# fxxJuses/MICFormer

Measured on AMD Instinct MI355X. Metric: train volumes/sec (128^3 CT+MRI pair), higher is better.
Workload: dtype bf16; 1 GPU; MicFormer base Head(embed_dim=48, depths 2-2-6-2, heads 3-6-12-24, window 2^3, 8 classes) full train step (fwd + MDiceLoss + bwd + Adam/cosine) on 128^3 CT+MR pairs, DropPath on; local_batch=2, global_batch=2, parallelism=dp1, launch=hipGraph replay (one graph)

## Files before the change

### include/micformer_hip.h

```cpp
#ifndef MICFORMER_HIP_H
#define MICFORMER_HIP_H

#include <stddef.h>
#include <stdint.h>

#ifdef __cplusplus
extern "C" {
#endif

typedef void* micf_stream_t;

#define MICF_OK 0
#define MICF_EINVAL (-1)
#define MICF_EUNSUPPORTED (-2)
#define MICF_ELAUNCH (-3)

#define MICF_ABI_VERSION 1

#define MICF_DTYPE_F32 0
#define MICF_DTYPE_BF16 1
#define MICF_DTYPE_BF16_ATTN_FP8 2

int micf_abi_version(void);
const char* micf_strerror(int code);
// ... 137 lines not shown
                            micf_stream_t stream);
int micf_conv_down_bwd_weight(const float* dy, const float* x, float* dw, float* dbias, int B, int D, int H, int W,
                              int C, int N, micf_stream_t stream);
int micf_space_to_depth(const float* x, float* a, int B, int D, int H, int W, int C, int k, int64_t batch_stride,
                        micf_stream_t stream);
int micf_depth_to_space(const float* a, const float* bias, float* y, int B, int D, int H, int W, int C, int k,
                        micf_stream_t stream);
int micf_depth_to_space_add(const float* a, const float* bias, const float* add, float* y, int B, int D, int H, int W, int C,
                            int k, micf_stream_t stream);
int micf_colsum(const float* x, float* out, int64_t M, int N, micf_stream_t stream);
int micf_conv_up_fwd(const float* x, const float* w, const float* bias, float* y, int B, int D, int H, int W, int C,
                     int N, int k, micf_stream_t stream);
int micf_conv_up_bwd_data(const float* dy, const float* w, float* dx, int B, int D, int H, int W, int C, int N, int k,
                          micf_stream_t stream);
int micf_conv_up_bwd_weight(const float* dy, const float* x, float* dw, float* dbias, int B, int D, int H, int W,
                            int C, int N, int k, micf_stream_t stream);

int micf_sw_window(const float* vol, float* win, int C, int D, int H, int W, int rd, int rh, int rw, int z0, int y0, int x0,
                   micf_stream_t stream);
int micf_sw_accumulate(const float* pred, float* out, float* count, int K, int D, int H, int W, int rd, int rh, int rw, int z0,
                       int y0, int x0, micf_stream_t stream);
int micf_sw_normalize(float* out, const float* count, int K, int64_t V, micf_stream_t stream);
int micf_sw_window_batch(const float* vol, float* win, const int32_t* coords, int n, int B, int C, int D, int H, int W, int rd,
                         int rh, int rw, micf_stream_t stream);
int micf_sw_accumulate_batch(const float* pred, float* out, float* count, const int32_t* coords, int n, int B, int K, int D, int H,
                             int W, int rd, int rh, int rw, micf_stream_t stream);

int micf_intensity_stats(const void* vol, int is_half, double* sums, int B, int Cm, int64_t V, micf_stream_t stream);
int micf_patch_rows_prepared(const void* vol, int is_half, const double* sums, const float* params, float* rows0, float* rows1, int B,
                             int Cm, int D, int H, int W, int k, micf_stream_t stream);
int micf_input_prepare(const void* vol, int is_half, const double* sums, const float* params, float* out, const uint8_t* label_in,
                       uint8_t* label_out, int B, int Cm, int D, int H, int W, micf_stream_t stream);

int micf_pad3d(const float* src, float* dst, int B, int D, int H, int W, int Dp, int Hp, int Wp, int C,
               micf_stream_t stream);
int micf_crop3d(const float* src, float* dst, int B, int D, int H, int W, int Dp, int Hp, int Wp, int C,
                int accumulate, micf_stream_t stream);
int micf_resize_trilinear_fwd(const float* src, float* dst, int B, int D, int H, int W, int Do, int Ho, int Wo, int C,
                              micf_stream_t stream);
int micf_resize_trilinear_bwd(const float* ddst, float* dsrc, int B, int D, int H, int W, int Do, int Ho, int Wo,
                              int C, micf_stream_t stream);

int micf_dice_bce_fwd(const float* logits, const float* target, double* sums, float* loss, int B, int K, int64_t V,
                      micf_stream_t stream);
int micf_dice_bce_bwd(const float* logits, const float* target, const double* sums, const float* grad_out,
                      float* dlogits, int B, int K, int64_t V, micf_stream_t stream);
int micf_dice_bce_label_fwd(const float* logits, const uint8_t* label, double* sums, float* loss, int B, int K, int64_t V,
                            micf_stream_t stream);
int micf_dice_bce_label_bwd(const float* logits, const uint8_t* label, const double* sums, const float* grad_out,
                            float* dlogits, int B, int K, int64_t V, micf_stream_t stream);
int micf_argmax_meandice(const float* logits, const uint8_t* label, uint8_t* mask_out, int64_t* counts, double* out,
                         int B, int K, int64_t V, micf_stream_t stream);

int micf_dice_metric(const float* logits, const void* target, int target_is_label, double* sums, float* out, int B, int K,
                     int64_t V, micf_stream_t stream);

int micf_adam_tick(void* state, double base_lr, double eta_min, int64_t t_max, micf_stream_t stream);
int micf_adam_step(float* p, const float* g, float* m, float* v, int64_t n, const void* state, float beta1,
                   float beta2, float eps, float grad_scale, void* p_bf16, micf_stream_t stream);


typedef struct micf_ln_pair_item {
  const float *x, *gamma, *beta;
  float *y, *mean, *rstd;
} micf_ln_pair_item;
typedef struct micf_ln_bwd_pair_item {
  const float *dy, *x, *mean, *rstd, *gamma;
  float *dx, *dgamma, *dbeta;
  const float* add;
  float* partials;
} micf_ln_bwd_pair_item;
int micf_layernorm_fwd_pair(const micf_ln_pair_item* items, int n, int64_t rows, int C, float eps, float* zero,
                            int64_t zero_floats, micf_stream_t stream);
int micf_layernorm_bwd_pair(const micf_ln_bwd_pair_item* items, int n, int64_t rows, int C, micf_stream_t stream);

typedef struct micf_offset_head_group {
  const float* xn;
  const float* xa;
  const float *conv_w, *conv_b;
  float* conv_ws;
  const float *ln_g, *ln_b, *w1;
  float *hid, *flow, *xs;
} micf_offset_head_group;
typedef struct micf_offset_head_bwd_group {
  const float* dxs;
  const float *hid, *flow, *xa, *ln_g, *ln_b, *w1, *conv_w;
  float* conv_ws;
  float* dxa;
  float* dxn;
  float* dhid;
  float *dln_g, *dln_b, *dw1;
} micf_offset_head_bwd_group;
int micf_offset_head_needs_zero(int B, int D, int H, int W, int C);
int micf_offset_head_fwd(const micf_offset_head_group* groups, int ngroups, int B, int D, int H, int W, int C, float eps,
                         int prepared, int hid_zeroed, int dtype, micf_stream_t stream);
int64_t micf_offset_head_bwd_workspace(int ngroups, int B, int D, int H, int W);
int micf_offset_head_bwd(const micf_offset_head_bwd_group* groups, int ngroups, int B, int D, int H, int W, int C, float eps,
                         int prepared, float* workspace, int64_t workspace_floats, int dtype, int defer_finish, micf_stream_t stream);
int micf_offset_head_finish_deferrable(int B, int D, int H, int W);
int micf_offset_head_bwd_finish(const micf_offset_head_bwd_group* groups, int ngroups, int B, int D, int H, int W, int C,
                                float* workspace, int64_t workspace_floats, micf_stream_t stream);
typedef struct micf_offset_head_finish_call {
  const micf_offset_head_bwd_group* groups;
  int32_t ngroups, B, D, H, W, C;
  float* workspace;
  int64_t workspace_floats;
} micf_offset_head_finish_call;
int micf_offset_head_bwd_finish_grouped(const micf_offset_head_finish_call* calls, int ncalls, micf_stream_t stream);

typedef struct micf_block_fwd_group {
  const float* x;
  const float* kvsrc;
  const float *ln1_g, *ln1_b, *bq, *bkv, *bp, *ln2_g, *ln2_b, *b1, *b2;
  const void *wq, *wkv, *wp, *w1, *w2;
  const float *s1, *s2;
  float* y;
  float *xn, *q, *kv, *o, *x1, *xn2;
  void* h;
  float* g;
  float* stats;
  void* kvs16;
  const float* hid;
  const float* samp_src;
  const float *ln16_g, *ln16_b, *w1c;
  float* flow;
  float* xs32;
  const float *nln_g, *nln_b;
  float *nln_y, *nln_mean, *nln_rstd;
  float* zero16;
} micf_block_fwd_group;
int micf_block_fuses_sampler(int C, int heads);
int micf_block_saves_bf16(int C, int heads, int dtype);
typedef struct micf_block_bwd_group {
  const float* dy;
  const float *x, *x1, *stats, *q, *kv;
  const void* h;
  const float *ln1_g, *ln2_g;
  const void *wqt, *wkvt, *wpt, *w1t, *w2t;
  const float *s1, *s2;
  float* dx;
  float* dxs;
  float *dx1, *dh, *dq, *dkv;
  float *ln1_part, *ln2_part;
  float* dx1_copy;
  void* dy16;
  const float* xn2;
  const void* w1;
  const float* b1;
  const float* pre_d;
  const float* pre_x;
  const float *pre_mean, *pre_rstd;
  const float* pre_g;
  float* pre_part;
} micf_block_bwd_group;
int micf_block_recomputes_h(int C, int heads);
int micf_block_tile_tokens(int B, int D, int H, int W, int C, int heads, int hidden, int backward);
int micf_block_fwd_persistent_probe(const micf_block_fwd_group* groups, int ngroups, int B, int D, int H, int W, int C, int heads,
                                    int hidden, float eps, float scale, int dtype, int repeats, int* sync_ws, micf_stream_t stream);
int micf_probe_mfma_chain(const void* a, const void* b, const void* c, const void* d, float* out, int form, micf_stream_t stream);
typedef struct micf_weight_prep_item {
  const float* src;
  void* dst;
  void* dst_t;
  int32_t rows, cols, bf16 , reserved;
} micf_weight_prep_item;
int micf_weight_prep_grouped(const micf_weight_prep_item* items, int n, micf_stream_t stream);
int micf_block_fwd(const micf_block_fwd_group* groups, int ngroups, int B, int D, int H, int W, int C, int heads,
                   int hidden, float eps, float scale, int dtype, micf_stream_t stream);
int micf_block_bwd(const micf_block_bwd_group* groups, int ngroups, int B, int D, int H, int W, int C, int heads,
                   int hidden, float scale, int dtype, micf_stream_t stream);

int micf_zero(void* p, int64_t bytes, micf_stream_t stream);
int micf_drop_path_draw(void* rng, const float* keep, float* out, int n, int B, micf_stream_t stream);


int micf_grad_wire_pack(const float* src, int64_t n, void* dst, int64_t padded, micf_stream_t stream);
int micf_grad_wire_sum(const void* recv, int ranks, int64_t shard, void* out, micf_stream_t stream);
int micf_grad_wire_unpack(const void* src, float* dst, int64_t n, micf_stream_t stream);

#ifdef __cplusplus
}
#endif
#endif
```

### micformer_amd/_lib.py

```python
import ctypes
import os

_PKT = "DEBUG_CLR_GRAPH_PACKET_CAPTURE"
_pkt_before = os.environ.get(_PKT)
if os.environ.get("MICF_SEGMENTED", "0") == "1":
    os.environ.setdefault(_PKT, "0")

import torch

GRAPH_SEGMENTS_OK = os.environ.get(_PKT) == "0" and (_pkt_before == "0" or not torch.cuda.is_initialized())

_HERE = os.path.dirname(os.path.abspath(__file__))
LIB_PATH = os.environ.get("MICF_LIB") or os.path.join(_HERE, "libmicformer_hip.so")

_P, _I, _L, _F, _D = ctypes.c_void_p, ctypes.c_int, ctypes.c_int64, ctypes.c_float, ctypes.c_double
_T = {"p": _P, "i": _I, "l": _L, "f": _F, "d": _D}

SIGNATURES = {
    "micf_layernorm_fwd": "ppippppplifp",
    "micf_layernorm_bwd": "pppippppppplippp",
    "micf_layernorm_bwd_partial_rows": "lii",
    "micf_layernorm_bwd_finish": "pip",
    "micf_linear_fwd": "ppipppplppliiiip",
    "micf_linear_bwd_data": "pplppppiiliiip",
    "micf_linear_bwd_weight": "pplppiippliiplip",
    "micf_linear_bwd_weight_workspace": "lii",
    "micf_linear_bwd_weight_grouped": "piplip",
    "micf_linear_bwd_weight_grouped_workspace": "pi",
    "micf_head_tail_compose": "pppppiiiipp",
    "micf_head_tail_col2im": "pppiiiiiip",
    "micf_head_tail_im2col": "ppiiiiiip",
    "micf_head_tail_col2im_sw": "pppppiiiiiiiiiip",
    "micf_head_tail_decompose": "pppppppppiiiipp",
    "micf_head_tail_fused_supported": "iiiiiii",
    "micf_head_tail_pack_bytes": "ii",
    "micf_head_tail_pack": "pppppiiip",
    "micf_head_tail_fwd_fused": "pppiiiiiiip",
    "micf_head_tail_fwd_fused_sw": "pppppiiiiiiiiiiip",
    "micf_head_tail_loss_parts": "iiii",
    "micf_head_tail_fwd_loss_fused": "ppppipppiiiiiiip",
    "micf_head_tail_bwd_data_fused": "pppiiiiiiip",
    "micf_head_tail_bwd_weight_fused": "pppppliiiiiiip",
    "micf_head_tail_bwd_weight_fused_workspace": "iiiii",
    "micf_sw_window": "ppiiiiiiiiiip",
    "micf_sw_accumulate": "pppiiiiiiiiiip",
    "micf_sw_normalize": "ppilp",
    "micf_window_attn_fwd": "pippipiiiiiiiiiifp",
    "micf_window_attn_fwd_fp8": "pippipiiiiiiiiiifp",
    "micf_window_attn_bwd": "pippipipippiiiiiiiiiifp",
    "micf_conv3_fwd": "pipipppiiiiiipliip",
    "micf_conv3_fwd_workspace": "iii",
    "micf_conv3_bwd_data": "pippiipiiiiiiipliip",
    "micf_conv3_weight_prep_grouped": "pip",
    "micf_layernorm_fwd_pair": "pilifplp",
    "micf_layernorm_bwd_pair": "pilip",
    "micf_offset_head_needs_zero": "iiiii",
    "micf_offset_head_fwd": "piiiiiifiiip",
    "micf_offset_head_bwd_workspace": "iiiii",
    "micf_offset_head_bwd": "piiiiiifipliip",
    "micf_offset_head_finish_deferrable": "iiii",
    "micf_offset_head_bwd_finish": "piiiiiiplp",
    "micf_offset_head_bwd_finish_grouped": "pip",
    "micf_conv3_bwd_data_workspace": "iii",
    "micf_conv3_bwd_weight": "pipipippiiiiiplip",
    "micf_conv3_bwd_weight_workspace": "iiiiiii",
    "micf_conv3_bwd_weight_grouped": "piiiiiiiiplip",
    "micf_conv3_bwd_weight_grouped_workspace": "iiiiiiii",
    "micf_offset_sample_fwd": "pppppppiiiiifp",
    "micf_offset_sample_bwd": "ppppppppppppiiiiifplp",
    "micf_offset_sample_bwd_workspace": "iiii",
    "micf_stn_fwd": "pppiiiiip",
    "micf_stn_bwd": "pppppiiiiip",
    "micf_patch_embed_fwd": "piipppiiiiiip",
    "micf_patch_embed_bwd_weight": "ppiippiiiiiip",
    "micf_conv_down_fwd": "ppppiiiiiip",
    "micf_conv_down_bwd_data": "pppiiiiiip",
    "micf_conv_down_bwd_weight": "ppppiiiiiip",
    "micf_conv_up_fwd": "ppppiiiiiiip",
    "micf_conv_up_bwd_data": "pppiiiiiiip",
    "micf_conv_up_bwd_weight": "ppppiiiiiiip",
    "micf_space_to_depth": "ppiiiiiilp",
    "micf_depth_to_space": "pppiiiiiip",
    "micf_depth_to_space_add": "ppppiiiiiip",
    "micf_colsum": "pplip",
    "micf_pad3d": "ppiiiiiiiip",
    "micf_crop3d": "ppiiiiiiiiip",
    "micf_resize_trilinear_fwd": "ppiiiiiiiip",
    "micf_resize_trilinear_bwd": "ppiiiiiiiip",
    "micf_dice_bce_fwd": "ppppiilp",
    "micf_dice_bce_bwd": "pppppiilp",
    "micf_dice_bce_label_fwd": "ppppiilp",
    "micf_dice_bce_label_bwd": "pppppiilp",
    "micf_argmax_meandice": "pppppiilp",
    "micf_adam_tick": "pddlp",
    "micf_adam_step": "pppplpffffpp",
    "micf_block_tile_tokens": "iiiiiiii",
    "micf_block_saves_bf16": "iii",
    "micf_block_fuses_sampler": "ii",
    "micf_block_recomputes_h": "ii",
    "micf_weight_prep_grouped": "pip",
    "micf_grad_wire_pack": "plplp",
    "micf_grad_wire_sum": "pilpp",
    "micf_grad_wire_unpack": "pplp",
    "micf_block_fwd": "piiiiiiiiffip",
    "micf_block_bwd": "piiiiiiiifip",
    "micf_block_fwd_persistent_probe": "piiiiiiiiffiipp",
    "micf_probe_mfma_chain": "pppppip",
    "micf_dice_metric": "ppippiilp",
    "micf_sw_window_batch": "pppiiiiiiiiip",
    "micf_sw_accumulate_batch": "ppppiiiiiiiiip",
    "micf_intensity_stats": "pipiilp",
    "micf_input_prepare": "pipppppiiiiip",
    "micf_patch_rows_prepared": "pippppiiiiiip",
    "micf_zero": "plp",
    "micf_drop_path_draw": "pppiip",
}


class WgradItem(ctypes.Structure):
    _fields_ = [("a", ctypes.c_void_p), ("dy", ctypes.c_void_p), ("dp_scale", ctypes.c_void_p), ("dw", ctypes.c_void_p),
                ("dbias", ctypes.c_void_p), ("M", ctypes.c_int64), ("rows_per_sample", ctypes.c_int64),
                ("N", ctypes.c_int32), ("K", ctypes.c_int32), ("operand_dtype", ctypes.c_int32), ("ldw", ctypes.c_int32)]


class Conv3WgradItem(ctypes.Structure):
    _fields_ = [("dy", ctypes.c_void_p), ("x1", ctypes.c_void_p), ("x2", ctypes.c_void_p), ("dw", ctypes.c_void_p),
                ("dbias", ctypes.c_void_p)]


class LnFinishItem(ctypes.Structure):
    _fields_ = [("partials", ctypes.c_void_p), ("dgamma", ctypes.c_void_p), ("dbeta", ctypes.c_void_p),
                ("blocks", ctypes.c_int32), ("C", ctypes.c_int32)]


_VP = ctypes.c_void_p


class BlockFwdGroup(ctypes.Structure):
    FIELDS = ("x", "kvsrc", "ln1_g", "ln1_b", "bq", "bkv", "bp", "ln2_g", "ln2_b", "b1", "b2", "wq", "wkv", "wp", "w1", "w2",
              "s1", "s2", "y", "xn", "q", "kv", "o", "x1", "xn2", "h", "g", "stats", "kvs16", "hid", "samp_src", "ln16_g", "ln16_b", "w1c", "flow", "xs32",
              "nln_g", "nln_b", "nln_y", "nln_mean", "nln_rstd", "zero16")
    _fields_ = [(n, _VP) for n in FIELDS]


class BlockBwdGroup(ctypes.Structure):
    FIELDS = ("dy", "x", "x1", "stats", "q", "kv", "h", "ln1_g", "ln2_g", "wqt", "wkvt", "wpt", "w1t", "w2t", "s1", "s2",
              "dx", "dxs", "dx1", "dh", "dq", "dkv", "ln1_part", "ln2_part", "dx1_copy", "dy16", "xn2", "w1", "b1",
              "pre_d", "pre_x", "pre_mean", "pre_rstd", "pre_g", "pre_part")
    _fields_ = [(n, _VP) for n in FIELDS]


class WeightPrepItem(ctypes.Structure):
    _fields_ = [("src", _VP), ("dst", _VP), ("dst_t", _VP), ("rows", ctypes.c_int32), ("cols", ctypes.c_int32),
                ("bf16", ctypes.c_int32), ("reserved", ctypes.c_int32)]


class LnPairItem(ctypes.Structure):
    FIELDS = ("x", "gamma", "beta", "y", "mean", "rstd")
    _fields_ = [(n, _VP) for n in FIELDS]


class LnBwdPairItem(ctypes.Structure):
    FIELDS = ("dy", "x", "mean", "rstd", "gamma", "dx", "dgamma", "dbeta", "add", "partials")
    _fields_ = [(n, _VP) for n in FIELDS]


class OffsetHeadGroup(ctypes.Structure):
    FIELDS = ("xn", "xa", "conv_w", "conv_b", "conv_ws", "ln_g", "ln_b", "w1", "hid", "flow", "xs")
    _fields_ = [(n, _VP) for n in FIELDS]


class OffsetHeadBwdGroup(ctypes.Structure):
    FIELDS = ("dxs", "hid", "flow", "xa", "ln_g", "ln_b", "w1", "conv_w", "conv_ws", "dxa", "dxn", "dhid", "dln_g", "dln_b", "dw1")
    _fields_ = [(n, _VP) for n in FIELDS]


class OffsetHeadFinishCall(ctypes.Structure):
    _fields_ = [("groups", _VP), ("ngroups", ctypes.c_int32), ("B", ctypes.c_int32), ("D", ctypes.c_int32), ("H", ctypes.c_int32),
                ("W", ctypes.c_int32), ("C", ctypes.c_int32), ("workspace", _VP), ("workspace_floats", ctypes.c_int64)]


class Conv3PrepItem(ctypes.Structure):
    _fields_ = [("w", _VP), ("fwd", _VP), ("bwd", _VP), ("N", ctypes.c_int32), ("Cin", ctypes.c_int32)]


class MicfError(RuntimeError):
    pass


INT64_RETURNS = frozenset((
    "micf_linear_bwd_weight_workspace", "micf_linear_bwd_weight_grouped_workspace", "micf_conv3_bwd_data_workspace",
    "micf_offset_sample_bwd_workspace", "micf_conv3_bwd_weight_workspace", "micf_conv3_bwd_weight_grouped_workspace",
    "micf_head_tail_pack_bytes", "micf_head_tail_loss_parts", "micf_head_tail_bwd_weight_fused_workspace",
    "micf_conv3_fwd_workspace", "micf_offset_head_bwd_workspace"))


def bind(signatures, int64=(), feature=None, library=None):
    library = lib if library is None else library
    for name, sig in signatures.items():
        try:
            fn = getattr(library, name)
        except AttributeError:
            what = f"predates the {feature} ({name} is missing)" if feature else f"does not export {name}"
            raise ImportError(f"{LIB_PATH} {what}: rebuild it with "
                              "`python -c \"import __graft_entry__ as g; g.build()\"`") from None
        fn.argtypes = [_T[c] for c in sig]
        fn.restype = _L if name in int64 else _I
    return library


def _load():
    if not os.path.exists(LIB_PATH):
        raise ImportError(
            f"{LIB_PATH} not found: build it with `python micformer_amd/build.py` (hipcc, gfx950). "
            "micformer_amd has no CPU / PyTorch fallback path.")
    lib = bind(SIGNATURES, INT64_RETURNS, library=ctypes.CDLL(LIB_PATH))
    lib.micf_strerror.argtypes = [_I]
    lib.micf_strerror.restype = ctypes.c_char_p
    lib.micf_set_option.argtypes = [ctypes.c_char_p, _I]
    lib.micf_set_option.restype = _I
    lib.micf_get_option.argtypes = [ctypes.c_char_p, ctypes.POINTER(_I)]
    lib.micf_get_option.restype = _I
    lib.micf_abi_version.argtypes = []
    lib.micf_abi_version.restype = _I
    if lib.micf_abi_version() != 1:
        raise ImportError("libmicformer_hip.so ABI version mismatch")
    return lib


lib = _load()


def get_option(name):
    v = _I(0)
    if lib.micf_get_option(name.encode(), ctypes.byref(v)) != 0:
        raise KeyError(f"unknown micformer option {name!r}")
    return v.value


def set_option(name, value):
    prev = get_option(name)
    if lib.micf_set_option(name.encode(), int(value)) != 0:
        raise KeyError(f"unknown micformer option {name!r}")
    return prev


class option:

    def __init__(self, name, value):
        self.name, self.value = name, value

    def __enter__(self):
        self.prev = set_option(self.name, self.value)

    def __exit__(self, *exc):
        set_option(self.name, self.prev)
        return False


def ptr(t):
    if t is None:
        return None
    if not t.is_cuda:
        raise MicfError("micformer_amd ops need CUDA (ROCm) tensors: there is no CPU path")
    if not t.is_contiguous():
        raise MicfError("micformer_amd ops need contiguous tensors")
    return t.data_ptr()


_raw_stream = getattr(torch._C, "_cuda_getCurrentRawStream", None)
_cur_device = getattr(torch._C, "_cuda_getDevice", None)


def stream():
    if _raw_stream is not None and _cur_device is not None:
        return _raw_stream(_cur_device())
    return torch.cuda.current_stream().cuda_stream


PROFILE = None
BLOCK_DEPTH = 0
UNIT = None


def set_unit(kind, groups, tokens, channels):
    global UNIT
    if PROFILE is not None:
        UNIT = f"{kind}|{groups}x{tokens}x{channels}"


class block_region:

    def __enter__(self):
        global BLOCK_DEPTH
        BLOCK_DEPTH += 1

    def __exit__(self, *exc):
        global BLOCK_DEPTH, UNIT
        BLOCK_DEPTH -= 1
        if BLOCK_DEPTH == 0:
            UNIT = None
# ... 79 lines not shown
```

### micformer_amd/csrc/block_bwd.hip

```cpp
#include "block_fused.h"
#include "attn_fp8.h"

namespace micf {

struct BlkBwdArgs {
  micf_block_bwd_group g[2];
  TileGeo geo;
  int G, tiles, C, heads, hidden;
  float scale;
  int attn_mfma;
};

template <int TM, int NW, int X4>
struct RowRegs {
  static constexpr int RPP = 4 * NW, NPASS = (TM + RPP - 1) / RPP, K = (X4 + 15) / 16;
  float4 v[NPASS][K];
  template <class Addr>
  __device__ __forceinline__ void load(const int* tok, int tk0, const Addr addr) {
    const int lane = threadIdx.x & 63, wave = threadIdx.x >> 6, l16 = lane & 15, rg = lane >> 4;
#pragma unroll
    for (int pass = 0; pass < NPASS; ++pass) {
      const int row = pass * RPP + wave * 4 + rg;
      const int tk = row < TM ? tok[row] : -1;
#pragma unroll
// ... 417 lines not shown
          float sacc = 0.f, dacc = 0.f;
#pragma unroll
          for (int d = 0; d < HP; d += 4) {
            const float4 t = *reinterpret_cast<const float4*>(kp + d);
            sacc += qr[d] * t.x; sacc += qr[d + 1] * t.y; sacc += qr[d + 2] * t.z; sacc += qr[d + 3] * t.w;
            const float4 u = *reinterpret_cast<const float4*>(vp + d);
            dacc += dor[d] * u.x; dacc += dor[d + 1] * u.y; dacc += dor[d + 2] * u.z; dacc += dor[d + 3] * u.w;
          }
          if (SP >= 2) { sacc += __shfl_xor(sacc, 1, 64); dacc += __shfl_xor(dacc, 1, 64); }
          if (SP == 4) { sacc += __shfl_xor(sacc, 2, 64); dacc += __shfl_xor(dacc, 2, 64); }
          p[j] = sacc; dp[j] = dacc;
          mx = fmaxf(mx, sacc);
        }
        float den = 0.f;
#pragma unroll
        for (int j = 0; j < 8; ++j) { p[j] = expf(p[j] - mx); den += p[j]; }
        const float inv = 1.0f / den;
        float dot = 0.f;
#pragma unroll
        for (int j = 0; j < 8; ++j) { p[j] *= inv; dot += p[j] * dp[j]; }
#pragma unroll
        for (int d = 0; d < HP; ++d) dq[d] = 0.f;
#pragma unroll
        for (int j = 0; j < 8; ++j) {
          const float ds = p[j] * (dp[j] - dot);
          if (j / (8 / SP) == sub) {
            PS[pair * 16 + j] = p[j];
            PS[pair * 16 + 8 + j] = ds;
          }
          const float* kp = U + (r0 + j) * SU + C + hoff;
          const float dss = ds * a.scale;
#pragma unroll
          for (int d = 0; d < HP; d += 4) {
            const float4 t = *reinterpret_cast<const float4*>(kp + d);
            dq[d] += dss * t.x; dq[d + 1] += dss * t.y; dq[d + 2] += dss * t.z; dq[d + 3] += dss * t.w;
          }
        }
      }
      lds_barrier();
      if (active) {
#pragma unroll
        for (int d = 0; d < HP; ++d) { dk[d] = 0.f; dv[d] = 0.f; }
        const int base = pair - i * heads;
#pragma unroll
        for (int m = 0; m < 8; ++m) {
          const float pm = PS[(base + m * heads) * 16 + i];
          const float dsm = PS[(base + m * heads) * 16 + 8 + i] * a.scale;
          const float* qp = U + (r0 + m) * SU + hoff;
          const float* dop = A2 + (r0 + m) * S + hoff;
#pragma unroll
          for (int d = 0; d < HP; d += 4) {
            const float4 t = *reinterpret_cast<const float4*>(qp + d);
            dk[d] += dsm * t.x; dk[d + 1] += dsm * t.y; dk[d + 2] += dsm * t.z; dk[d + 3] += dsm * t.w;
            const float4 u = *reinterpret_cast<const float4*>(dop + d);
            dv[d] += pm * u.x; dv[d + 1] += pm * u.y; dv[d + 2] += pm * u.z; dv[d + 3] += pm * u.w;
          }
        }
      }
      lds_barrier();
      if (active) {
#pragma unroll
        for (int d = 0; d < HP; d += 4) {
          *reinterpret_cast<float4*>(U + row * SU + hoff + d) = make_float4(dq[d], dq[d + 1], dq[d + 2], dq[d + 3]);
          *reinterpret_cast<float4*>(U + row * SU + C + hoff + d) = make_float4(dk[d], dk[d + 1], dk[d + 2], dk[d + 3]);
          *reinterpret_cast<float4*>(U + row * SU + 2 * C + hoff + d) = make_float4(dv[d], dv[d + 1], dv[d + 2], dv[d + 3]);
        }
      }
      lds_barrier();
    }
  }

#pragma unroll 1
  for (int pass = 0; pass < NPASS; ++pass) {
    const int row = pass * RPP + wave * 4 + rg;
    if (row >= TM) continue;
    const int tk = tok[row];
    if (tk < 0) continue;
    const uint32_t rel = (uint32_t)(tk - tk0);
    for (int c4 = l16; c4 < 3 * C4; c4 += 16) {
      const float4 v = *reinterpret_cast<const float4*>(U + row * SU + 4 * c4);
      if (c4 < C4) st_h4_32<BF16>(dq0, rel * C + 4 * c4, v);
      else st_h4_32<BF16>(dkv0, rel * 2 * C + 4 * (c4 - C4), v);
    }
  }

  if (!g.dxs) {
    if (PARK) r_ln1.unpark(stash, g.ln1_g);
    gemm_phase<TJ, NSLK, NKK, C, NW, BF16>(wqt, C, U, nullptr, 0, nullptr, SU, A2, S, EpiStore{});
    gemm_phase<TJ, NSLK, 2 * NKK, 2 * C, NW, BF16>(wkvt, C, U + C, nullptr, 0, nullptr, SU, A2, S, EpiAcc{});
    ln_bwd_tile<TJ, VPL, NW, C>(A2, A1, S, r_ln1, tok, tk0, dx0, nullptr, U, g.ln1_part ? g.ln1_part + (int64_t)tile * 2 * C : nullptr);
  } else {
    gemm_phase<TJ, NSLK, NKK, C, NW, BF16>(wqt, C, U, nullptr, 0, nullptr, SU, A2, S, EpiStore{});
#pragma unroll 1
    for (int pass = 0; pass < NPASS; ++pass) {
      const int row = pass * RPP + wave * 4 + rg;
      if (row >= TM) continue;
      const int tk = tok[row];
      if (tk < 0) continue;
      for (int c4 = l16; c4 < C4; c4 += 16)
        st4g(at32(dx0, ((uint32_t)(tk - tk0) * C + 4 * c4) * 4u), *reinterpret_cast<const float4*>(A2 + row * S + 4 * c4));
    }
    lds_barrier();
    gemm_phase<TJ, NSLK, 2 * NKK, 2 * C, NW, BF16>(wkvt, C, U + C, nullptr, 0, nullptr, SU, A2, S, EpiStore{});
#pragma unroll 1
    for (int pass = 0; pass < NPASS; ++pass) {
      const int row = pass * RPP + wave * 4 + rg;
      if (row >= TM) continue;
      const int tk = tok[row];
      if (tk < 0) continue;
      for (int c4 = l16; c4 < C4; c4 += 16)
        st4g(at32(g.dxs + (int64_t)tk0 * C, ((uint32_t)(tk - tk0) * C + 4 * c4) * 4u), *reinterpret_cast<const float4*>(A2 + row * S + 4 * c4));
    }
  }
}

template <int C, int HD, int TJ>
static int launch_bwd(const BlkBwdArgs& a, int dtype, hipStream_t s) {
  constexpr int TM = 16 * TJ, NW = C >= 192 ? 8 : 4;
  const bool recomp = a.g[0].h == nullptr;
  const size_t lds = block_lds_floats(TM, C, block_bwd_scratch_floats(TM, C / HD, 64 * NW),
                                      block_bwd_park_floats(TM, C, 64 * NW) + (recomp ? 4 * C : 0)) * sizeof(float);
  if (lds > 160 * 1024) return MICF_EUNSUPPORTED;
  const unsigned grid = a.G == 2 ? (unsigned)((a.tiles + 3) / 4 * 8) : (unsigned)a.tiles;
  static std::once_flag once;
  std::call_once(once, [] {
    (void)hipFuncSetAttribute(reinterpret_cast<const void*>(&block_bwd_kernel<C, HD, TJ, NW, true, false>), hipFuncAttributeMaxDynamicSharedMemorySize, 160 * 1024);
    (void)hipFuncSetAttribute(reinterpret_cast<const void*>(&block_bwd_kernel<C, HD, TJ, NW, false, false>), hipFuncAttributeMaxDynamicSharedMemorySize, 160 * 1024);
    (void)hipFuncSetAttribute(reinterpret_cast<const void*>(&block_bwd_kernel<C, HD, TJ, NW, true, true>), hipFuncAttributeMaxDynamicSharedMemorySize, 160 * 1024);
    (void)hipFuncSetAttribute(reinterpret_cast<const void*>(&block_bwd_kernel<C, HD, TJ, NW, false, true>), hipFuncAttributeMaxDynamicSharedMemorySize, 160 * 1024);
  });
  if (dtype == MICF_DTYPE_BF16) {
    if (recomp) hipLaunchKernelGGL((block_bwd_kernel<C, HD, TJ, NW, true, true>), dim3(grid), dim3(64 * NW), lds, s, a);
    else hipLaunchKernelGGL((block_bwd_kernel<C, HD, TJ, NW, true, false>), dim3(grid), dim3(64 * NW), lds, s, a);
  } else {
    if (recomp) hipLaunchKernelGGL((block_bwd_kernel<C, HD, TJ, NW, false, true>), dim3(grid), dim3(64 * NW), lds, s, a);
    else hipLaunchKernelGGL((block_bwd_kernel<C, HD, TJ, NW, false, false>), dim3(grid), dim3(64 * NW), lds, s, a);
  }
  MICF_RETURN_LAUNCH();
}

}

#include "block_wave_bwd.h"

using namespace micf;

extern "C" int micf_block_bwd(const micf_block_bwd_group* groups, int ngroups, int B, int D, int H, int W, int C, int heads,
                              int hidden, float scale, int dtype, micf_stream_t stream) {
  if (!groups || ngroups < 1 || ngroups > 2) return MICF_EINVAL;
  const int TM = micf_block_tile_tokens(B, D, H, W, C, heads, hidden, 1);
  if (TM == 0) return MICF_EUNSUPPORTED;
  if (dtype != MICF_DTYPE_F32 && dtype != MICF_DTYPE_BF16) return MICF_EINVAL;
  BlkBwdArgs a;
  for (int i = 0; i < ngroups; ++i) {
    const micf_block_bwd_group& g = groups[i];
    const void* need[] = {g.dy, g.x1, g.stats, g.q, g.kv, g.ln2_g, g.wqt, g.wkvt, g.wpt, g.w1t, g.w2t, g.dx, g.dx1, g.dh, g.dq, g.dkv};
    for (const void* p : need)
      if (!p || (reinterpret_cast<uintptr_t>(p) & 15)) return MICF_EINVAL;
    if (g.h) {
      if (reinterpret_cast<uintptr_t>(g.h) & 15) return MICF_EINVAL;
    } else {
      const void* re[] = {g.xn2, g.w1, g.b1};
      for (const void* p : re)
        if (!p || (reinterpret_cast<uintptr_t>(p) & 15)) return MICF_EINVAL;
      if (!micf_block_recomputes_h(C, heads)) return MICF_EINVAL;
    }
    if (i > 0 && (g.h == nullptr) != (groups[0].h == nullptr)) return MICF_EINVAL;
    if (g.pre_d) {
      const void* pr[] = {g.pre_d, g.pre_x, g.pre_mean, g.pre_rstd, g.pre_g, g.pre_part, g.dy16};
      for (const void* p : pr)
        if (!p || (reinterpret_cast<uintptr_t>(p) & 15)) return MICF_EINVAL;
      if (g.dxs || dtype != MICF_DTYPE_BF16 || block_wide_tile_tokens(C, C / heads)) return MICF_EINVAL;
    }
    if (!g.dxs && (!g.x || !g.ln1_g)) return MICF_EINVAL;
    const void* opt[] = {g.x, g.ln1_g, g.dxs, g.ln1_part, g.ln2_part, g.dx1_copy, g.dy16};
    for (const void* p : opt)
      if (p && (reinterpret_cast<uintptr_t>(p) & 15)) return MICF_EINVAL;
    a.g[i] = g;
  }
  if (ngroups == 1) a.g[1] = a.g[0];
  a.geo = make_tile_geo(B, D, H, W);
  a.G = ngroups; a.C = C; a.heads = heads; a.hidden = hidden; a.scale = scale;
  a.tiles = (a.geo.nwin + TM / 8 - 1) / (TM / 8);
  a.attn_mfma = dtype == MICF_DTYPE_BF16 ? 1 : 0;
  hipStream_t s = (hipStream_t)stream;
  const int hd = C / heads, tj = TM / 16;
  if ((int64_t)2 * H * W * (TM / 8 + 1) * hidden * (int64_t)sizeof(float) >= (int64_t)1 << 32) return MICF_EUNSUPPORTED;
  if (block_wide_tile_tokens(C, hd)) return block_bwd_wide(groups, ngroups, B, D, H, W, C, heads, scale, dtype, s);
  {
    if (options().block_wave != 0 && C == 48 && hd == 16 && tj == 2 && dtype == MICF_DTYPE_BF16 && a.attn_mfma && a.g[0].h && a.g[1].h && (a.g[0].dxs != nullptr) == (a.g[1].dxs != nullptr) &&
        (a.g[0].pre_d != nullptr) == (a.g[1].pre_d != nullptr) && !(a.g[0].dxs && a.g[0].pre_d) &&
        a.geo.T * (int64_t)hidden * 2 < ((int64_t)1 << 31))
    {
      if (options().block_debug & 1) a.attn_mfma |= 2;
      return wave48::launch_bwd_wave48(a, s);
    }
  }
#define MICF_BB(C_, HD_, TJ_) if (C == C_ && hd == HD_ && tj == TJ_) return launch_bwd<C_, HD_, TJ_>(a, dtype, s)
  MICF_BB(48, 16, 2); MICF_BB(96, 16, 2); MICF_BB(192, 16, 1);
  MICF_BB(96, 32, 1); MICF_BB(192, 32, 1); MICF_BB(384, 32, 1);
#undef MICF_BB
  return MICF_EUNSUPPORTED;
}
```

### micformer_amd/csrc/block_fwd.hip

```cpp
#include <cstdlib>

#include "block_fused.h"
#include "attn_fp8.h"

namespace micf {

struct BlkFwdArgs {
  micf_block_fwd_group g[2];
  TileGeo geo;
  int G, tiles, C, heads, hidden, debug;
  int att8;
  float eps, scale;
};

template <int C, int HD, int TJ, int NW, bool BF16, bool SAMP>
__device__ __forceinline__ void block_fwd_tile(const BlkFwdArgs& a, const unsigned bid) {
  constexpr int TM = 16 * TJ, VPL = (C + 63) / 64, NSL = C / 16, NTHR = 64 * NW, RPP = 4 * NW, NPASS = (TM + RPP - 1) / RPP;
  constexpr int NSLK = C >= 384 ? NSL / 2 : NSL, NKK = C >= 384 ? 2 : 1;
  extern __shared__ __attribute__((aligned(1024))) float lds[];
  constexpr int C4 = C >> 2, S = C + 4, SU = block_u_cols(C, true, TM) + 4, Hd = 4 * C;
  float* A1 = lds;
  float* A2 = A1 + TM * S;
  float* U = A2 + TM * S;
  float* sc1 = U + TM * SU;
// ... 317 lines not shown
      const int row = pass * RPP + wave * 4 + rg;
      if (row >= TM) continue;
      const int tk = tok[row];
      for (int c4 = l16; c4 < X4; c4 += 16) {
        float* up = U + row * SU + 4 * c4;
        const float4 v = *reinterpret_cast<const float4*>(up);
        const float4 ge = do_gelu ? make_float4(gelu_t<BF16>(v.x), gelu_t<BF16>(v.y), gelu_t<BF16>(v.z), gelu_t<BF16>(v.w)) : v;
        *reinterpret_cast<float4*>(up) = ge;
        if (tk >= 0 && save) {
          if (g.h) st_h4<BF16>(g.h, (int64_t)tk * Hd + c0 + 4 * c4, v);
          st_h4<BF16>(g.g, (int64_t)tk * Hd + c0 + 4 * c4, ge);
        }
      }
    }
    lds_barrier();
    if (!(a.debug & 4)) gemm_phase<TJ, NSLK, NKK * HC / C, Hd, NW, BF16>(w2 + 16 * c0, C, U, nullptr, 0, nullptr, SU, A2, S, EpiAccScale{sc2});
  }

  const bool nln = g.nln_g != nullptr;
#pragma unroll 1
  for (int pass = 0; pass < NPASS; ++pass) {
    const int row = pass * RPP + wave * 4 + rg;
    if (row >= TM) continue;
    const int tk = tok[row];
    if (tk < 0) continue;
    const float s2v = sc2[row];
    float4 v[VPL];
#pragma unroll
    for (int k = 0; k < VPL; ++k) {
      const int c4 = l16 + 16 * k;
      v[k] = make_float4(0.f, 0.f, 0.f, 0.f);
      if (c4 < C4) {
        v[k] = *reinterpret_cast<const float4*>(A2 + row * S + 4 * c4);
        const float4 b = *reinterpret_cast<const float4*>(p_b2 + 4 * c4);
        v[k].x += s2v * b.x; v[k].y += s2v * b.y; v[k].z += s2v * b.z; v[k].w += s2v * b.w;
        st4g(g.y + (int64_t)tk * C + 4 * c4, v[k]);
      }
    }
    if (nln) {
      float s = 0.f;
#pragma unroll
      for (int k = 0; k < VPL; ++k) s += (v[k].x + v[k].y) + (v[k].z + v[k].w);
      const float mu = sum16(s) * invC;
      float qd = 0.f;
#pragma unroll
      for (int k = 0; k < VPL; ++k) {
        if (l16 + 16 * k < C4) {
          const float d0 = v[k].x - mu, d1 = v[k].y - mu, d2 = v[k].z - mu, d3 = v[k].w - mu;
          qd += (d0 * d0 + d1 * d1) + (d2 * d2 + d3 * d3);
        }
      }
      const float rs = 1.0f / sqrtf(sum16(qd) * invC + a.eps);
#pragma unroll
      for (int k = 0; k < VPL; ++k) {
        const int c4 = l16 + 16 * k;
        if (c4 < C4) {
          const float4 gm = *reinterpret_cast<const float4*>(p_ln1g + 4 * c4), bt = *reinterpret_cast<const float4*>(p_ln1b + 4 * c4);
          st4g(g.nln_y + (int64_t)tk * C + 4 * c4, make_float4((v[k].x - mu) * rs * gm.x + bt.x, (v[k].y - mu) * rs * gm.y + bt.y,
                                                                (v[k].z - mu) * rs * gm.z + bt.z, (v[k].w - mu) * rs * gm.w + bt.w));
        }
      }
      if (l16 == 0) { g.nln_mean[tk] = mu; g.nln_rstd[tk] = rs; }
      if (g.zero16) g.zero16[(int64_t)tk * 16 + l16] = 0.f;
    }
  }
}

template <int C, int HD, int TJ, int NW, bool BF16, bool SAMP>
__global__ void __launch_bounds__(64 * NW) block_fwd_kernel(const BlkFwdArgs a) {
  block_fwd_tile<C, HD, TJ, NW, BF16, SAMP>(a, blockIdx.x);
}

__device__ __forceinline__ void probe_grid_barrier(unsigned* bar, unsigned target, int* err) {
  __syncthreads();
  if (threadIdx.x == 0) {
    __threadfence();
    atomicAdd(bar, 1u);
    long spins = 0;
    while (__atomic_load_n(bar, __ATOMIC_ACQUIRE) < target) {
      if (++spins > 40000000) { *err = 1; break; }
    }
    __threadfence();
  }
  __syncthreads();
}
template <int C, int HD, int TJ, int NW, bool BF16, bool SAMP>
__global__ void __launch_bounds__(64 * NW) block_fwd_persist_probe_kernel(const BlkFwdArgs a, int repeats, unsigned* bar, int* err) {
  for (int k = 0; k < repeats; ++k) {
    block_fwd_tile<C, HD, TJ, NW, BF16, SAMP>(a, blockIdx.x);
    if (k + 1 < repeats) probe_grid_barrier(bar, (unsigned)(k + 1) * gridDim.x, err);
  }
}

template <int C, int HD, int TJ>
static int launch_fwd(const BlkFwdArgs& a, int dtype, hipStream_t s) {
  constexpr int TM = 16 * TJ, NW = C >= 192 ? (HD <= 16 ? 16 : 8) : 4;
  const size_t lds = block_lds_floats(TM, C, 0, 9 * C + 4 * C, true) * sizeof(float);
  if (lds > 160 * 1024) return MICF_EUNSUPPORTED;
  const unsigned grid = a.G == 2 ? (unsigned)((a.tiles + 3) / 4 * 8) : (unsigned)a.tiles;
  static std::once_flag once;
  std::call_once(once, [] {
    (void)hipFuncSetAttribute(reinterpret_cast<const void*>(&block_fwd_kernel<C, HD, TJ, NW, true, false>), hipFuncAttributeMaxDynamicSharedMemorySize, 160 * 1024);
    (void)hipFuncSetAttribute(reinterpret_cast<const void*>(&block_fwd_kernel<C, HD, TJ, NW, false, false>), hipFuncAttributeMaxDynamicSharedMemorySize, 160 * 1024);
    (void)hipFuncSetAttribute(reinterpret_cast<const void*>(&block_fwd_kernel<C, HD, TJ, NW, true, true>), hipFuncAttributeMaxDynamicSharedMemorySize, 160 * 1024);
    (void)hipFuncSetAttribute(reinterpret_cast<const void*>(&block_fwd_kernel<C, HD, TJ, NW, false, true>), hipFuncAttributeMaxDynamicSharedMemorySize, 160 * 1024);
  });
  const bool samp = a.g[0].hid != nullptr || a.g[1].hid != nullptr;
  if (dtype == MICF_DTYPE_BF16) {
    if (samp) hipLaunchKernelGGL((block_fwd_kernel<C, HD, TJ, NW, true, true>), dim3(grid), dim3(64 * NW), lds, s, a);
    else hipLaunchKernelGGL((block_fwd_kernel<C, HD, TJ, NW, true, false>), dim3(grid), dim3(64 * NW), lds, s, a);
  } else {
    if (samp) hipLaunchKernelGGL((block_fwd_kernel<C, HD, TJ, NW, false, true>), dim3(grid), dim3(64 * NW), lds, s, a);
    else hipLaunchKernelGGL((block_fwd_kernel<C, HD, TJ, NW, false, false>), dim3(grid), dim3(64 * NW), lds, s, a);
  }
  MICF_RETURN_LAUNCH();
}

}

#include "block_wave_fwd.h"

using namespace micf;

extern "C" int micf_block_tile_tokens(int B, int D, int H, int W, int C, int heads, int hidden, int backward) {
  if (B <= 0 || D <= 0 || H <= 0 || W <= 0 || C <= 0 || heads <= 0 || hidden <= 0) return 0;
  if ((D | H | W) & 1) return 0;
  if (C % heads || hidden != 4 * C) return 0;
  if ((int64_t)B * D * H * W >= (1LL << 31)) return 0;
  const int hd = C / heads;
  if (const int wt = block_wide_tile_tokens(C, hd)) return wt;
  int tj = 0;
  if (C == 48 && hd == 16) tj = 2;
  else if (C == 96 && hd == 16) tj = backward ? 2 : 1;
  else if ((C == 96 || C == 192) && (hd == 16 || hd == 32)) tj = 1;
  else if (C == 384 && hd == 32) tj = 1;
  return 16 * tj;
}

extern "C" int micf_block_fuses_sampler(int C, int heads) {
  if (C <= 0 || heads <= 0 || C % heads) return 0;
  return block_wide_tile_tokens(C, C / heads) ? 0 : 1;
}

extern "C" int micf_block_recomputes_h(int C, int heads) {
  if (C <= 0 || heads <= 0 || C % heads || block_wide_tile_tokens(C, C / heads)) return 0;
  return options().block_recompute_h != 0 ? 1 : 0;
}

extern "C" int micf_block_saves_bf16(int C, int heads, int dtype) {
  if (C <= 0 || heads <= 0 || C % heads) return 0;
  return block_saves_bf16(C, C / heads, dtype) ? 1 : 0;
}

extern "C" int micf_block_fwd(const micf_block_fwd_group* groups, int ngroups, int B, int D, int H, int W, int C, int heads,
                              int hidden, float eps, float scale, int dtype, micf_stream_t stream) {
  if (!groups || ngroups < 1 || ngroups > 2) return MICF_EINVAL;
  const int TM = micf_block_tile_tokens(B, D, H, W, C, heads, hidden, 0);
  if (TM == 0) return MICF_EUNSUPPORTED;
  const int att8 = dtype == MICF_DTYPE_BF16_ATTN_FP8;
  if (att8) dtype = MICF_DTYPE_BF16;
  if (dtype != MICF_DTYPE_F32 && dtype != MICF_DTYPE_BF16) return MICF_EINVAL;
  BlkFwdArgs a;
  a.att8 = att8 ? 2 : (dtype == MICF_DTYPE_BF16 ? 1 : 0);
  int nosave = -1;
  for (int i = 0; i < ngroups; ++i) {
    const micf_block_fwd_group& g = groups[i];
    const void* must[] = {g.x, g.ln1_g, g.ln1_b, g.wq, g.bq, g.wkv, g.bkv, g.wp, g.bp, g.ln2_g, g.ln2_b, g.w1, g.b1, g.w2, g.b2, g.y};
    for (const void* p : must)
      if (!p || (reinterpret_cast<uintptr_t>(p) & 15)) return MICF_EINVAL;
    const void* saves[] = {g.q, g.kv, g.o, g.x1, g.xn2, g.g, g.stats};
    int nnull = 0;
    for (const void* p : saves) nnull += p == nullptr;
    const bool ns = nnull == 7 && !g.h && !g.xn && !g.kvs16 && !g.flow && !g.xs32;
    if (nosave >= 0 && nosave != (int)ns) return MICF_EINVAL;
    nosave = ns;
    if (ns) {
      if (block_wide_tile_tokens(C, C / heads)) return MICF_EUNSUPPORTED;
    } else {
      for (const void* p : saves)
        if (!p || (reinterpret_cast<uintptr_t>(p) & 15)) return MICF_EINVAL;
      if (g.h ? (reinterpret_cast<uintptr_t>(g.h) & 15) != 0 : !micf_block_recomputes_h(C, heads)) return MICF_EINVAL;
    }
    if ((g.kvsrc && (reinterpret_cast<uintptr_t>(g.kvsrc) & 15)) || (g.xn && (reinterpret_cast<uintptr_t>(g.xn) & 15)) ||
        (g.kvs16 && (reinterpret_cast<uintptr_t>(g.kvs16) & 15))) return MICF_EINVAL;
    if (g.hid) {
      if (g.kvsrc || !g.samp_src || !g.ln16_g || !g.ln16_b || !g.w1c || (!g.flow && !ns) || (reinterpret_cast<uintptr_t>(g.samp_src) & 15) ||
          (g.xs32 && (reinterpret_cast<uintptr_t>(g.xs32) & 15)) || block_wide_tile_tokens(C, C / heads))
        return MICF_EINVAL;
    }
    if (g.nln_g) {
      const void* need[] = {g.nln_g, g.nln_b, g.nln_y, g.nln_mean, g.nln_rstd};
      for (const void* p : need)
        if (!p || (reinterpret_cast<uintptr_t>(p) & 15)) return MICF_EINVAL;
      if (g.zero16 && (reinterpret_cast<uintptr_t>(g.zero16) & 15)) return MICF_EINVAL;
      if (block_wide_tile_tokens(C, C / heads)) return MICF_EUNSUPPORTED;
    } else if (g.nln_b || g.nln_y || g.nln_mean || g.nln_rstd || g.zero16) {
      return MICF_EINVAL;
    }
    a.g[i] = g;
  }
  if (ngroups == 1) a.g[1] = a.g[0];
  a.geo = make_tile_geo(B, D, H, W);
  a.G = ngroups; a.C = C; a.heads = heads; a.hidden = hidden; a.eps = eps; a.scale = scale;
  a.tiles = (a.geo.nwin + TM / 8 - 1) / (TM / 8);
  a.debug = options().block_debug;
  if (nosave == 1) a.debug |= 1;
  hipStream_t s = (hipStream_t)stream;
  const int hd = C / heads, tj = TM / 16;
  if (block_wide_tile_tokens(C, hd)) return block_fwd_wide(groups, ngroups, B, D, H, W, C, heads, eps, scale, att8 ? MICF_DTYPE_BF16_ATTN_FP8 : dtype, s);
  if (options().block_wave != 0 && C == 48 && hd == 16 && dtype == MICF_DTYPE_BF16 && a.att8 == 1 && !(a.debug & ~17) &&
      a.geo.T * (int64_t)C * 4 < ((int64_t)1 << 32))
    return wave48::launch_fwd_wave48(a, s);
#define MICF_BF(C_, HD_, TJ_) if (C == C_ && hd == HD_ && tj == TJ_) return launch_fwd<C_, HD_, TJ_>(a, dtype, s)
  MICF_BF(48, 16, 2); MICF_BF(96, 16, 1); MICF_BF(192, 16, 1);
  MICF_BF(96, 32, 1); MICF_BF(192, 32, 1); MICF_BF(384, 32, 1);
#undef MICF_BF
  return MICF_EUNSUPPORTED;
}

namespace micf {
namespace wave48 {
__global__ void __launch_bounds__(64) mfma_chain_probe_kernel0(const bf16x8* a, const bf16x8* b, const bf16x4_t* c, const bf16x4_t* d, f32x4* out) {
  const int l = threadIdx.x;
  const f32x4 z = {0.f, 0.f, 0.f, 0.f};
  out[l] = mfma16(c[l], d[l], mfma32(a[l], b[l], z));
}
__global__ void __launch_bounds__(64) mfma_chain_probe_kernel1(const bf16x8* a, const bf16x8* b, const bf16x4_t* c, const bf16x4_t* d, f32x4* out) {
  const int l = threadIdx.x;
  out[l] = mfma48(a[l], c[l], b[l], d[l]);
}
template <int NOPS>
__global__ void __launch_bounds__(64) mfma_chain_probe_kernel2(const bf16x8* a, const bf16x8* b, const bf16x4_t* c, const bf16x4_t* d, f32x4* out) {
  const int l = threadIdx.x;
  const bf16x8 av = a[l], bv = b[l];
  const bf16x4_t cv = c[l], dv = d[l];
  f32x4 acc;
  if (NOPS == 0)
    asm volatile("s_nop 7\n\tv_mfma_f32_16x16x32_bf16 %0, %1, %2, 0\n\tv_mfma_f32_16x16x16_bf16 %0, %3, %4, %0\n\ts_nop 15\n\ts_nop 15"
                 : "=&v"(acc) : "v"(av), "v"(bv), "v"(cv), "v"(dv));
  else
    asm volatile("s_nop 7\n\tv_mfma_f32_16x16x32_bf16 %0, %1, %2, 0\n\ts_nop 15\n\tv_mfma_f32_16x16x16_bf16 %0, %3, %4, %0\n\ts_nop 15\n\ts_nop 15"
                 : "=&v"(acc) : "v"(av), "v"(bv), "v"(cv), "v"(dv));
  out[l] = acc;
}
}
}
extern "C" int micf_probe_mfma_chain(const void* a, const void* b, const void* c, const void* d, float* out, int form, micf_stream_t stream) {
  if (!a || !b || !c || !d || !out || form < 0 || form > 3) return MICF_EINVAL;
  hipStream_t s = (hipStream_t)stream;
  using namespace micf::wave48;
  if (form == 0) hipLaunchKernelGGL(mfma_chain_probe_kernel0, dim3(1), dim3(64), 0, s, static_cast<const bf16x8*>(a), static_cast<const bf16x8*>(b), static_cast<const bf16x4_t*>(c), static_cast<const bf16x4_t*>(d), reinterpret_cast<f32x4*>(out));
  else if (form == 3) hipLaunchKernelGGL(mfma_chain_probe_kernel2<16>, dim3(1), dim3(64), 0, s, static_cast<const bf16x8*>(a), static_cast<const bf16x8*>(b), static_cast<const bf16x4_t*>(c), static_cast<const bf16x4_t*>(d), reinterpret_cast<f32x4*>(out));
  else if (form == 2) hipLaunchKernelGGL(mfma_chain_probe_kernel2<0>, dim3(1), dim3(64), 0, s, static_cast<const bf16x8*>(a), static_cast<const bf16x8*>(b), static_cast<const bf16x4_t*>(c), static_cast<const bf16x4_t*>(d), reinterpret_cast<f32x4*>(out));
  else hipLaunchKernelGGL(mfma_chain_probe_kernel1, dim3(1), dim3(64), 0, s, static_cast<const bf16x8*>(a), static_cast<const bf16x8*>(b), static_cast<const bf16x4_t*>(c), static_cast<const bf16x4_t*>(d), reinterpret_cast<f32x4*>(out));
  MICF_RETURN_LAUNCH();
}

extern "C" int micf_block_fwd_persistent_probe(const micf_block_fwd_group* groups, int ngroups, int B, int D, int H, int W, int C,
                                               int heads, int hidden, float eps, float scale, int dtype, int repeats, int* sync_ws,
                                               micf_stream_t stream) {
  if (!groups || ngroups < 1 || ngroups > 2 || !sync_ws || repeats < 1 || repeats > 64) return MICF_EINVAL;
  if (C != 192 || heads != 12 || hidden != 4 * C || dtype != MICF_DTYPE_BF16) return MICF_EUNSUPPORTED;
  const int TM = micf_block_tile_tokens(B, D, H, W, C, heads, hidden, 0);
  if (TM != 16) return MICF_EUNSUPPORTED;
  BlkFwdArgs a;
  a.att8 = 1;
  for (int i = 0; i < 2; ++i) a.g[i] = groups[i < ngroups ? i : 0];
  a.geo = make_tile_geo(B, D, H, W);
  a.G = ngroups; a.C = C; a.heads = heads; a.hidden = hidden; a.eps = eps; a.scale = scale;
  a.tiles = (a.geo.nwin + TM / 8 - 1) / (TM / 8);
  a.debug = 0;
  const unsigned grid = a.G == 2 ? (unsigned)((a.tiles + 3) / 4 * 8) : (unsigned)a.tiles;
  if (grid > 256) return MICF_EUNSUPPORTED;
  constexpr int NW = 16;
  const size_t lds = block_lds_floats(TM, C, 0, 9 * C + 4 * C, true) * sizeof(float);
  hipStream_t s = (hipStream_t)stream;
  if (hipMemsetAsync(sync_ws, 0, 2 * sizeof(int), s) != hipSuccess) return MICF_ELAUNCH;
  const bool samp = a.g[0].hid != nullptr;
  static std::once_flag once;
  std::call_once(once, [] {
    (void)hipFuncSetAttribute(reinterpret_cast<const void*>(&block_fwd_persist_probe_kernel<192, 16, 1, NW, true, false>), hipFuncAttributeMaxDynamicSharedMemorySize, 160 * 1024);
    (void)hipFuncSetAttribute(reinterpret_cast<const void*>(&block_fwd_persist_probe_kernel<192, 16, 1, NW, true, true>), hipFuncAttributeMaxDynamicSharedMemorySize, 160 * 1024);
  });
  unsigned* bar = reinterpret_cast<unsigned*>(sync_ws);
  if (samp) hipLaunchKernelGGL((block_fwd_persist_probe_kernel<192, 16, 1, NW, true, true>), dim3(grid), dim3(64 * NW), lds, s, a, repeats, bar, sync_ws + 1);
  else hipLaunchKernelGGL((block_fwd_persist_probe_kernel<192, 16, 1, NW, true, false>), dim3(grid), dim3(64 * NW), lds, s, a, repeats, bar, sync_ws + 1);
  MICF_RETURN_LAUNCH();
}
```

### micformer_amd/csrc/block_wave.h

```cpp
#pragma once

namespace micf {
namespace wave48 {

constexpr int C = 48, HID = 192, NWAVE = 8, NTHR = 64 * NWAVE;

typedef unsigned u32x4v __attribute__((ext_vector_type(4)));
typedef unsigned u32x2v __attribute__((ext_vector_type(2)));

__device__ __forceinline__ int row_p48(int j, int r) { return j < 2 ? 8 * (r >> 2) + 4 * j + (r & 3) : 32 + r; }
__device__ __forceinline__ int row_p192(int j, int r) { return 32 * (j >> 1) + 8 * (r >> 2) + 4 * (j & 1) + (r & 3); }
__device__ __forceinline__ int k16(int row, int k, int KB) { return ((row >> 4) * KB + (k >> 4)) * 256 + (row & 15) * 16 + (k & 15); }

__device__ __forceinline__ bf16x8 frag32(const char* lds, int base, int f, int lane) {
  return *reinterpret_cast<const bf16x8*>(lds + base + (f * 64 + lane) * 16);
}
__device__ __forceinline__ bf16x4_t frag16(const char* lds, int base, int f, int lane) {
  return *reinterpret_cast<const bf16x4_t*>(lds + base + (f * 64 + lane) * 8);
}
__device__ __forceinline__ f32x4 mfma32(const bf16x8& a, const bf16x8& b, const f32x4& c) { return __builtin_amdgcn_mfma_f32_16x16x32_bf16(a, b, c, 0, 0, 0); }
__device__ __forceinline__ f32x4 mfma16(const bf16x4_t& a, const bf16x4_t& b, const f32x4& c) { return __builtin_amdgcn_mfma_f32_16x16x16bf16_1k(a, b, c, 0, 0, 0); }
__device__ __forceinline__ f32x4 mfma48(const bf16x8& a32, const bf16x4_t& a16, const bf16x8& b32, const bf16x4_t& b16) {
  const f32x4 z = {0.f, 0.f, 0.f, 0.f};
  const f32x4 p = mfma32(a32, b32, z), q = mfma16(a16, b16, z);
  return f32x4{p[0] + q[0], p[1] + q[1], p[2] + q[2], p[3] + q[3]};
}
__device__ __forceinline__ float sum4(float v) {
  v += __shfl_xor(v, 16, 64);
  return v + __shfl_xor(v, 32, 64);
}
__device__ __forceinline__ void st4u(void* p, const bf16x8& v) { *reinterpret_cast<u32x4v*>(p) = __builtin_bit_cast(u32x4v, v); }
__device__ __forceinline__ void st2u(void* p, const bf16x4_t& v) { *reinterpret_cast<u32x2v*>(p) = __builtin_bit_cast(u32x2v, v); }
__device__ __forceinline__ bf16x4_t pack4q(const f32x4& v) { return pack4_bf16v(v[0], v[1], v[2], v[3]); }

struct Row12 {
  float v[12];
  __device__ __forceinline__ void load(const float* row, int lr) {
    const float4 a = ld4g(row + 8 * lr), b = ld4g(row + 8 * lr + 4), c = ld4g(row + 32 + 4 * lr);
    v[0] = a.x; v[1] = a.y; v[2] = a.z; v[3] = a.w; v[4] = b.x; v[5] = b.y; v[6] = b.z; v[7] = b.w; v[8] = c.x; v[9] = c.y; v[10] = c.z; v[11] = c.w;
  }
  __device__ __forceinline__ void zero() {
#pragma unroll
    for (int e = 0; e < 12; ++e) v[e] = 0.f;
  }
  __device__ __forceinline__ void store(float* row, int lr) const {
    *reinterpret_cast<float4*>(row + 8 * lr) = make_float4(v[0], v[1], v[2], v[3]);
    *reinterpret_cast<float4*>(row + 8 * lr + 4) = make_float4(v[4], v[5], v[6], v[7]);
    *reinterpret_cast<float4*>(row + 32 + 4 * lr) = make_float4(v[8], v[9], v[10], v[11]);
  }
  __device__ __forceinline__ bf16x8 lo() const { return to_bf16x8(make_float4(v[0], v[1], v[2], v[3]), make_float4(v[4], v[5], v[6], v[7])); }
  __device__ __forceinline__ bf16x4_t hi() const { return pack4_bf16v(v[8], v[9], v[10], v[11]); }
};
__device__ __forceinline__ void vec12(const float* p, int lr, float (&o)[12]) {
  const float4 a = *reinterpret_cast<const float4*>(p + 8 * lr), b = *reinterpret_cast<const float4*>(p + 8 * lr + 4),
               c = *reinterpret_cast<const float4*>(p + 32 + 4 * lr);
  o[0] = a.x; o[1] = a.y; o[2] = a.z; o[3] = a.w; o[4] = b.x; o[5] = b.y; o[6] = b.z; o[7] = b.w; o[8] = c.x; o[9] = c.y; o[10] = c.z; o[11] = c.w;
}
__device__ __forceinline__ void layernorm12(const Row12& x, const float* gam, const float* bet, int lr, float eps, Row12& y, float& mu, float& rs) {
  float s = 0.f;
#pragma unroll
  for (int e = 0; e < 12; e += 4) s += (x.v[e] + x.v[e + 1]) + (x.v[e + 2] + x.v[e + 3]);
  mu = sum4(s) * (1.0f / C);
  float qd = 0.f;
#pragma unroll
  for (int e = 0; e < 12; e += 4) {
    const float d0 = x.v[e] - mu, d1 = x.v[e + 1] - mu, d2 = x.v[e + 2] - mu, d3 = x.v[e + 3] - mu;
    qd += (d0 * d0 + d1 * d1) + (d2 * d2 + d3 * d3);
  }
  rs = 1.0f / sqrtf(sum4(qd) * (1.0f / C) + eps);
  float gm[12], bt[12];
  vec12(gam, lr, gm);
  vec12(bet, lr, bt);
#pragma unroll
  for (int e = 0; e < 12; ++e) y.v[e] = (x.v[e] - mu) * rs * gm[e] + bt[e];
}

}
}
```

### micformer_amd/csrc/block_wave_bwd.h

```cpp
#pragma once

#include "block_wave.h"

namespace micf {
namespace wave48 {

constexpr int kB2 = 0;
constexpr int kB2h = kB2 + 12 * 1024;
constexpr int kB1 = kB2h + 12 * 512;
constexpr int kBP = kB1 + 18 * 1024;
constexpr int kBPh = kBP + 3 * 1024;
constexpr int kBQ = kBPh + 3 * 512;
constexpr int kBKV = kBQ + 9 * 512;
constexpr int kBVec = kBKV + 18 * 512;
constexpr int kBPark = kBVec + 3 * C * 4;
constexpr int kParkFloats = 4 * (16 * 12 + 8);
constexpr int kBwdLdsBytes = kBPark + NWAVE * kParkFloats * 4;

__device__ __forceinline__ void stage_weights_bwd(char* lds, const micf_block_bwd_group& g) {
  const uint16_t* wqt = static_cast<const uint16_t*>(g.wqt), *wkvt = static_cast<const uint16_t*>(g.wkvt), *wpt = static_cast<const uint16_t*>(g.wpt),
                 *w1t = static_cast<const uint16_t*>(g.w1t), *w2t = static_cast<const uint16_t*>(g.w2t);
  const int tid = threadIdx.x;
  for (int s = tid; s < 12 * 64; s += NTHR) {
    const int j = s >> 6, li = s & 15, lr = (s >> 4) & 3, row = row_p192(j, li);
    *reinterpret_cast<u32x4v*>(lds + kB2 + s * 16) = *reinterpret_cast<const u32x4v*>(w2t + k16(row, 8 * lr, 3));
    *reinterpret_cast<u32x2v*>(lds + kB2h + s * 8) = *reinterpret_cast<const u32x2v*>(w2t + k16(row, 32 + 4 * lr, 3));
  }
  for (int s = tid; s < 18 * 64; s += NTHR) {
    const int f = s >> 6, j = f / 6, kc = f - 6 * j, li = s & 15, lr = (s >> 4) & 3;
    *reinterpret_cast<u32x4v*>(lds + kB1 + s * 16) = *reinterpret_cast<const u32x4v*>(w1t + k16(row_p48(j, li), 32 * kc + 8 * lr, 12));
  }
  for (int s = tid; s < 3 * 64; s += NTHR) {
    const int j = s >> 6, li = s & 15, lr = (s >> 4) & 3, row = 16 * j + li;
    *reinterpret_cast<u32x4v*>(lds + kBP + s * 16) = *reinterpret_cast<const u32x4v*>(wpt + k16(row, 8 * lr, 3));
    *reinterpret_cast<u32x2v*>(lds + kBPh + s * 8) = *reinterpret_cast<const u32x2v*>(wpt + k16(row, 32 + 4 * lr, 3));
  }
  for (int s = tid; s < 9 * 64; s += NTHR) {
    const int f = s >> 6, j = f / 3, h = f - 3 * j, li = s & 15, lr = (s >> 4) & 3;
    *reinterpret_cast<u32x2v*>(lds + kBQ + s * 8) = *reinterpret_cast<const u32x2v*>(wqt + k16(row_p48(j, li), 16 * h + 4 * lr, 3));
  }
  for (int s = tid; s < 18 * 64; s += NTHR) {
    const int f = s >> 6, j = f / 6, h = f - 6 * j, li = s & 15, lr = (s >> 4) & 3;
    *reinterpret_cast<u32x2v*>(lds + kBKV + s * 8) = *reinterpret_cast<const u32x2v*>(wkvt + k16(row_p48(j, li), 16 * h + 4 * lr, 6));
  }
  float* PV = reinterpret_cast<float*>(lds + kBVec);
  for (int e = tid; e < 3 * C; e += NTHR) {
    const float* src = e < C ? g.ln1_g : (e < 2 * C ? g.ln2_g : g.pre_g);
    PV[e] = src ? src[e % C] : 0.f;
  }
}

__device__ __forceinline__ void park12(float* tile, int lr, int li, const float (&v)[12]) {
  float* p = tile + lr * 200 + li * 12;
  *reinterpret_cast<float4*>(p) = make_float4(v[0], v[1], v[2], v[3]);
  *reinterpret_cast<float4*>(p + 4) = make_float4(v[4], v[5], v[6], v[7]);
  *reinterpret_cast<float4*>(p + 8) = make_float4(v[8], v[9], v[10], v[11]);
}
__device__ __forceinline__ void unpark12(const float* tile, int lr, int li, float (&v)[12]) {
  const float* p = tile + lr * 200 + li * 12;
  const float4 a = *reinterpret_cast<const float4*>(p), b = *reinterpret_cast<const float4*>(p + 4), c = *reinterpret_cast<const float4*>(p + 8);
  v[0] = a.x; v[1] = a.y; v[2] = a.z; v[3] = a.w; v[4] = b.x; v[5] = b.y; v[6] = b.z; v[7] = b.w; v[8] = c.x; v[9] = c.y; v[10] = c.z; v[11] = c.w;
}
__device__ __forceinline__ float colsum16(const float* tile, int lane) {
  const int c = lane < 48 ? lane : 0;
  const float* p = tile + (c < 32 ? (c >> 3) * 200 + (c & 7) : ((c - 32) >> 2) * 200 + 8 + (c & 3));
  float s0 = 0.f, s1 = 0.f;
#pragma unroll
  for (int t = 0; t < 16; t += 2) { s0 += p[12 * t]; s1 += p[12 * t + 12]; }
  return s0 + s1;
}

__device__ __forceinline__ void ln_bwd12(const float (&d)[12], const Row12& xin, float mu, float rs, const float* gam, int lr, int li,
                                         int lane, float* tile, const Row12& add, Row12& out, float& pg, float& pb) {
  float gm[12], dxh[12];
  vec12(gam, lr, gm);
  float sa = 0.f, sb = 0.f;
#pragma unroll
  for (int e = 0; e < 12; e += 4) {
    float g4[4], xh[4];
#pragma unroll
    for (int r = 0; r < 4; ++r) { xh[r] = (xin.v[e + r] - mu) * rs; g4[r] = gm[e + r] * d[e + r]; dxh[e + r] = d[e + r] * xh[r]; }
    sa += (g4[0] + g4[1]) + (g4[2] + g4[3]);
    sb += (g4[0] * xh[0] + g4[1] * xh[1]) + (g4[2] * xh[2] + g4[3] * xh[3]);
  }
  const float Am = sum4(sa) * (1.0f / C), Bm = sum4(sb) * (1.0f / C);
  park12(tile, lr, li, dxh);
#pragma unroll
  for (int e = 0; e < 12; ++e) out.v[e] = add.v[e] + rs * (gm[e] * d[e] - Am - ((xin.v[e] - mu) * rs) * Bm);
  pg += colsum16(tile, lane);
  asm volatile("" : "+v"(pg));
  park12(tile, lr, li, d);
  pb += colsum16(tile, lane);
  asm volatile("" : "+v"(pb));
}

__device__ __forceinline__ void unpack8(const u32x4v& u, float (&o)[8]) {
#pragma unroll
  for (int w = 0; w < 4; ++w) { o[2 * w] = __uint_as_float(u[w] << 16); o[2 * w + 1] = __uint_as_float(u[w] & 0xFFFF0000u); }
}

template <bool CROSS, bool PRE>
__global__ void __launch_bounds__(NTHR) __attribute__((amdgpu_waves_per_eu(4, 4))) block_bwd_wave48_kernel(const BlkBwdArgs a) {
  extern __shared__ __attribute__((aligned(1024))) char wlds[];
  const unsigned bid = blockIdx.x;
  int grp, wg, nwg;
  if (a.G == 2) { const int xcd = bid & 7; grp = xcd >> 2; wg = (int)(bid >> 3) * 4 + (xcd & 3); nwg = (int)(gridDim.x >> 3) * 4; }
  else { grp = 0; wg = bid; nwg = gridDim.x; }
  const micf_block_bwd_group& g = a.g[grp];
  stage_weights_bwd(wlds, g);
  const int tid = threadIdx.x, lane0 = tid & 63, wave = __builtin_amdgcn_readfirstlane(tid >> 6);
  const float* PV = reinterpret_cast<const float*>(wlds + kBVec);
  const float *p_ln1g = PV, *p_ln2g = PV + C, *p_preg = PV + 2 * C;
  const uint32_t T = (uint32_t)a.geo.T;
  const int ngroup16 = (a.geo.nwin + 1) >> 1;
  constexpr bool cross = CROSS, pre = PRE;
  const f32x4 z4 = {0.f, 0.f, 0.f, 0.f};
  lds_barrier();

  for (int unit = wg * NWAVE + wave; unit < a.tiles; unit += nwg * NWAVE) {
    float pg_pre = 0.f, pb_pre = 0.f, pg2 = 0.f, pb2 = 0.f, pg1 = 0.f, pb1 = 0.f;
#pragma unroll 1
    for (int sub = 0; sub < 2; ++sub) {
      const int gt = 2 * unit + sub;
      if (gt >= ngroup16) break;
      asm volatile("" ::: "memory");
      int lane = lane0;
      asm volatile("" : "+v"(lane));
      const int li = lane & 15, lr = lane >> 4;
      const bf16x4_t ident = pack4_bf16v(4 * lr == li ? 1.f : 0.f, 4 * lr + 1 == li ? 1.f : 0.f, 4 * lr + 2 == li ? 1.f : 0.f, 4 * lr + 3 == li ? 1.f : 0.f);
      const bool valid = (lr >> 1) == (li >> 3);
      float* tile = reinterpret_cast<float*>(wlds + kBPark) + wave * kParkFloats;
      const int win = 2 * gt + (li >> 3);
      const bool live0 = win < a.geo.nwin, live = live0 && !(a.attn_mfma & 2);
      int b = 0, d_ = 0, hh = 0, w = 0;
      a.geo.coords(live0 ? win : 0, li & 7, b, d_, hh, w);
      const uint32_t tk = (uint32_t)(((b * a.geo.D + d_) * a.geo.H + hh) * a.geo.W + w);
      const float s1v = g.s1 ? g.s1[b] : 1.f, s2v = g.s2 ? g.s2[b] : 1.f;
      const uint32_t rowC = tk * C;

      Row12 dy;
      dy.load(at32(g.dy, rowC * 4u), lr);
      if (!live) dy.zero();
      if (pre) {
        Row12 pd, px;
        pd.load(at32(g.pre_d, rowC * 4u), lr);
        px.load(at32(g.pre_x, rowC * 4u), lr);
        float pm = *at32(g.pre_mean, tk * 4u), pr = *at32(g.pre_rstd, tk * 4u);
        if (!live) { pd.zero(); px.zero(); pm = 0.f; pr = 0.f; }
        Row12 t;
        ln_bwd12(pd.v, px, pm, pr, p_preg, lr, li, lane, tile, dy, t, pg_pre, pb_pre);
        dy = t;
        if (!live) dy.zero();
      }
      const bf16x8 dyA = dy.lo();
      const bf16x4_t dyB = dy.hi();
      park12(tile, lr, li, dy.v);
      u32x4v hreg[6];
      {
        const uint16_t* hp = static_cast<const uint16_t*>(g.h);
#pragma unroll
        for (int c = 0; c < 6; ++c) {
          hreg[c] = *reinterpret_cast<const u32x4v*>(at32(hp, (tk * HID + 32 * c + 8 * lr) * 2u));
          if (!live) hreg[c] = u32x4v{0u, 0u, 0u, 0u};
        }
      }

      f32x4 dn2[3] = {z4, z4, z4};
      bf16x8 dhs[6];
      {
#pragma unroll
        for (int c = 0; c < 6; ++c) {
          float h8[8];
          unpack8(hreg[c], h8);
          float4 dv[2];
#pragma unroll
          for (int u = 0; u < 2; ++u) {
            const int j = 2 * c + u;
            const f32x4 acc = mfma48(frag32(wlds, kB2, j, lane), frag16(wlds, kB2h, j, lane), dyA, dyB);
            dv[u] = make_float4(s2v * acc[0] * gelu_grad_t<true>(h8[4 * u]), s2v * acc[1] * gelu_grad_t<true>(h8[4 * u + 1]),
                                s2v * acc[2] * gelu_grad_t<true>(h8[4 * u + 2]), s2v * acc[3] * gelu_grad_t<true>(h8[4 * u + 3]));
          }
          dhs[c] = to_bf16x8(dv[0], dv[1]);
#pragma unroll
          for (int j = 0; j < 3; ++j) dn2[j] = mfma32(frag32(wlds, kB1, 6 * j + c, lane), dhs[c], dn2[j]);
          __builtin_amdgcn_sched_barrier(0);
        }
      }
      const uint16_t* qp = reinterpret_cast<const uint16_t*>(g.q);
      const uint16_t* kp = reinterpret_cast<const uint16_t*>(g.kv);
      bf16x4_t qn, kn, vn;
      auto load_head = [&](int h) {
        qn = *reinterpret_cast<const bf16x4_t*>(at32(qp, (rowC + 16 * h + 4 * lr) * 2u));
        kn = *reinterpret_cast<const bf16x4_t*>(at32(kp, (2 * rowC + 16 * h + 4 * lr) * 2u));
        vn = *reinterpret_cast<const bf16x4_t*>(at32(kp, (2 * rowC + C + 16 * h + 4 * lr) * 2u));
        if (!live) { qn = bf16x4_t{0, 0, 0, 0}; kn = qn; vn = qn; }
      };
      load_head(0);
      Row12 x1;
      x1.load(at32(g.x1, rowC * 4u), lr);
      float mu2 = *at32(g.stats, (2 * T + tk) * 4u), rs2 = *at32(g.stats, (3 * T + tk) * 4u);
      if (!live) { x1.zero(); mu2 = 0.f; rs2 = 0.f; }
      Row12 x;
      float mu1 = 0.f, rs1 = 0.f;

      asm volatile("" ::: "memory");
      if (live) {
        if (g.dy16) {
          uint16_t* o = static_cast<uint16_t*>(g.dy16);
          st4u(at32(o, (rowC + 8 * lr) * 2u), dyA); st2u(at32(o, (rowC + 32 + 4 * lr) * 2u), dyB);
        }
        uint16_t* dho = reinterpret_cast<uint16_t*>(g.dh);
#pragma unroll
        for (int c = 0; c < 6; ++c) st4u(at32(dho, (tk * HID + 32 * c + 8 * lr) * 2u), dhs[c]);
      }

      __builtin_amdgcn_sched_barrier(0);
      Row12 dx1;
      {
        float d[12];
#pragma unroll
        for (int j = 0; j < 3; ++j)
#pragma unroll
          for (int r = 0; r < 4; ++r) d[4 * j + r] = dn2[j][r];
        Row12 dyp;
        unpark12(tile, lr, li, dyp.v);
        ln_bwd12(d, x1, mu2, rs2, p_ln2g, lr, li, lane, tile, dyp, dx1, pg2, pb2);
        if (!live) dx1.zero();
      }
      const bf16x8 d1A = dx1.lo();
      const bf16x4_t d1B = dx1.hi();
      if (live) {
        uint16_t* o = reinterpret_cast<uint16_t*>(g.dx1);
        st4u(at32(o, (rowC + 8 * lr) * 2u), d1A); st2u(at32(o, (rowC + 32 + 4 * lr) * 2u), d1B);
        if (g.dx1_copy) dx1.store(at32(g.dx1_copy, rowC * 4u), lr);
      }

      bf16x4_t dqf[3], dkf[3], dvf[3];
      {
        uint16_t* dqo = reinterpret_cast<uint16_t*>(g.dq);
        uint16_t* dko = reinterpret_cast<uint16_t*>(g.dkv);
#pragma unroll
        for (int h = 0; h < 3; ++h) {
          const bf16x4_t qcur = qn, kf = kn, vf = vn;
          if (h < 2) load_head(h + 1);
          else if (!cross) {
            x.load(at32(g.x, rowC * 4u), lr);
            mu1 = *at32(g.stats, tk * 4u); rs1 = *at32(g.stats, (T + tk) * 4u);
            if (!live) { x.zero(); mu1 = 0.f; rs1 = 0.f; }
          }
          const f32x4 dacc = mfma48(frag32(wlds, kBP, h, lane), frag16(wlds, kBPh, h, lane), d1A, d1B);
          const bf16x4_t of = pack4_bf16v(s1v * dacc[0], s1v * dacc[1], s1v * dacc[2], s1v * dacc[3]);
          const uint2 qu = __builtin_bit_cast(uint2, qcur);
          const bf16x4_t qf = pack4_bf16v(__uint_as_float(qu.x << 16) * a.scale, __uint_as_float(qu.x & 0xFFFF0000u) * a.scale,
                                          __uint_as_float(qu.y << 16) * a.scale, __uint_as_float(qu.y & 0xFFFF0000u) * a.scale);
          const f32x4 s1 = mfma16(kf, qf, z4);
          const f32x4 p1 = mfma16(vf, of, z4);
          const f32x4 s2 = mfma16(qf, kf, z4);
          const f32x4 p2 = mfma16(of, vf, z4);
          float m = valid ? fmaxf(fmaxf(s1[0], s1[1]), fmaxf(s1[2], s1[3])) : -INFINITY;
          m = fmaxf(m, __shfl_xor(m, 16, 64));
          float e[4];
#pragma unroll
          for (int r = 0; r < 4; ++r) e[r] = valid ? expf(s1[r] - m) : 0.f;
          float sum = (e[0] + e[1]) + (e[2] + e[3]);
          sum += __shfl_xor(sum, 16, 64);
          const float inv = valid ? 1.0f / sum : 0.f;
          float dot = 0.f;
#pragma unroll
          for (int r = 0; r < 4; ++r) { e[r] *= inv; dot += valid ? e[r] * p1[r] : 0.f; }
          dot += __shfl_xor(dot, 16, 64);
          float ds1[4];
#pragma unroll
          for (int r = 0; r < 4; ++r) ds1[r] = valid ? e[r] * (p1[r] - dot) : 0.f;
          const bf16x4_t dsf1 = pack4_bf16v(ds1[0], ds1[1], ds1[2], ds1[3]);
          float e2[4], ds2[4];
#pragma unroll
          for (int r = 0; r < 4; ++r) {
            const int qi = 4 * lr + r, src = qi + 16 * (2 * (qi >> 3));
            const float mq = __shfl(m, src, 64), iq = __shfl(inv, src, 64), dq_ = __shfl(dot, src, 64);
            e2[r] = valid ? expf(s2[r] - mq) * iq : 0.f;
            ds2[r] = valid ? e2[r] * (p2[r] - dq_) : 0.f;
          }
          const bf16x4_t pf2 = pack4_bf16v(e2[0], e2[1], e2[2], e2[3]);
          const bf16x4_t dsf2 = pack4_bf16v(ds2[0], ds2[1], ds2[2], ds2[3]);
          const bf16x4_t kt = pack4q(mfma16(kf, ident, z4)), qt = pack4q(mfma16(qf, ident, z4)), ot = pack4q(mfma16(of, ident, z4));
          const f32x4 ga = mfma16(kt, dsf1, z4);
          const f32x4 gb = mfma16(qt, dsf2, z4);
          const f32x4 gc = mfma16(ot, pf2, z4);
          dqf[h] = pack4_bf16v(ga[0] * a.scale, ga[1] * a.scale, ga[2] * a.scale, ga[3] * a.scale);
          dkf[h] = pack4q(gb);
          dvf[h] = pack4q(gc);
          if (live) {
            st2u(at32(dqo, (rowC + 16 * h + 4 * lr) * 2u), dqf[h]);
            st2u(at32(dko, (2 * rowC + 16 * h + 4 * lr) * 2u), dkf[h]);
            st2u(at32(dko, (2 * rowC + C + 16 * h + 4 * lr) * 2u), dvf[h]);
          }
          __builtin_amdgcn_sched_barrier(0);
        }
      }

      __builtin_amdgcn_sched_barrier(0);
      if (!cross) {
        float d[12];
#pragma unroll
        for (int j = 0; j < 3; ++j) {
          f32x4 acc = z4;
#pragma unroll
          for (int h = 0; h < 3; ++h) acc = mfma16(frag16(wlds, kBQ, 3 * j + h, lane), dqf[h], acc);
#pragma unroll
          for (int h = 0; h < 6; ++h) acc = mfma16(frag16(wlds, kBKV, 6 * j + h, lane), h < 3 ? dkf[h] : dvf[h - 3], acc);
#pragma unroll
          for (int r = 0; r < 4; ++r) d[4 * j + r] = acc[r];
        }
        Row12 dx;
        ln_bwd12(d, x, mu1, rs1, p_ln1g, lr, li, lane, tile, dx1, dx, pg1, pb1);
        if (live) dx.store(at32(g.dx, rowC * 4u), lr);
      } else {
        Row12 dxq, dxs;
#pragma unroll
        for (int j = 0; j < 3; ++j) {
          f32x4 acc = z4, acs = z4;
#pragma unroll
          for (int h = 0; h < 3; ++h) acc = mfma16(frag16(wlds, kBQ, 3 * j + h, lane), dqf[h], acc);
#pragma unroll
          for (int h = 0; h < 6; ++h) acs = mfma16(frag16(wlds, kBKV, 6 * j + h, lane), h < 3 ? dkf[h] : dvf[h - 3], acs);
#pragma unroll
          for (int r = 0; r < 4; ++r) { dxq.v[4 * j + r] = acc[r]; dxs.v[4 * j + r] = acs[r]; }
        }
        if (live) {
          dxq.store(at32(g.dx, rowC * 4u), lr);
          dxs.store(at32(g.dxs, rowC * 4u), lr);
        }
      }
    }
    if (lane0 < C) {
      const int64_t row = (int64_t)unit * 2 * C;
      if (g.ln2_part) { g.ln2_part[row + lane0] = pg2; g.ln2_part[row + C + lane0] = pb2; }
      if (!cross && g.ln1_part) { g.ln1_part[row + lane0] = pg1; g.ln1_part[row + C + lane0] = pb1; }
      if (pre) { g.pre_part[row + lane0] = pg_pre; g.pre_part[row + C + lane0] = pb_pre; }
    }
  }
}

static int launch_bwd_wave48(const BlkBwdArgs& a, hipStream_t s) {
  int nwg = (a.tiles + NWAVE - 1) / NWAVE;
  if (nwg > 256) nwg = 256;
  const unsigned grid = a.G == 2 ? (unsigned)((nwg + 3) / 4 * 8) : (unsigned)nwg;
  static std::once_flag once;
  std::call_once(once, [] {
    (void)hipFuncSetAttribute(reinterpret_cast<const void*>(&block_bwd_wave48_kernel<true, false>), hipFuncAttributeMaxDynamicSharedMemorySize, 160 * 1024);
    (void)hipFuncSetAttribute(reinterpret_cast<const void*>(&block_bwd_wave48_kernel<false, true>), hipFuncAttributeMaxDynamicSharedMemorySize, 160 * 1024);
    (void)hipFuncSetAttribute(reinterpret_cast<const void*>(&block_bwd_wave48_kernel<false, false>), hipFuncAttributeMaxDynamicSharedMemorySize, 160 * 1024);
  });
  const bool cross = a.g[0].dxs != nullptr, pre = a.g[0].pre_d != nullptr;
  if (cross) hipLaunchKernelGGL((block_bwd_wave48_kernel<true, false>), dim3(grid), dim3(NTHR), kBwdLdsBytes, s, a);
  else if (pre) hipLaunchKernelGGL((block_bwd_wave48_kernel<false, true>), dim3(grid), dim3(NTHR), kBwdLdsBytes, s, a);
  else hipLaunchKernelGGL((block_bwd_wave48_kernel<false, false>), dim3(grid), dim3(NTHR), kBwdLdsBytes, s, a);
  MICF_RETURN_LAUNCH();
}

}
}
```

### micformer_amd/csrc/block_wave_fwd.h

```cpp
#pragma once

#include "block_wave.h"

namespace micf {
namespace wave48 {

constexpr int kTapBatch = 8;

constexpr int kQ32 = 0;
constexpr int kQ16 = kQ32 + 9 * 1024;
constexpr int kP16 = kQ16 + 9 * 512;
constexpr int kF32 = kP16 + 9 * 512;
constexpr int kF16 = kF32 + 12 * 1024;
constexpr int kG32 = kF16 + 12 * 512;
constexpr int kVec = kG32 + 18 * 1024;
constexpr int kLdsBytes = kVec + (9 * C + HID + 2 * C) * 4;


__device__ __forceinline__ void stage_weights(char* lds, const micf_block_fwd_group& g) {
  const uint16_t* wq = static_cast<const uint16_t*>(g.wq), *wkv = static_cast<const uint16_t*>(g.wkv), *wp = static_cast<const uint16_t*>(g.wp),
                 *w1 = static_cast<const uint16_t*>(g.w1), *w2 = static_cast<const uint16_t*>(g.w2);
  const int tid = threadIdx.x;
  for (int s = tid; s < 9 * 64; s += NTHR) {
    const int j = s >> 6, li = s & 15, lr = (s >> 4) & 3;
    const uint16_t* W = j < 3 ? wq : wkv;
    const int row = 16 * (j < 3 ? j : j - 3) + li;
    *reinterpret_cast<u32x4v*>(lds + kQ32 + s * 16) = *reinterpret_cast<const u32x4v*>(W + k16(row, 8 * lr, 3));
    *reinterpret_cast<u32x2v*>(lds + kQ16 + s * 8) = *reinterpret_cast<const u32x2v*>(W + k16(row, 32 + 4 * lr, 3));
  }
  for (int s = tid; s < 9 * 64; s += NTHR) {
    const int f = s >> 6, j = f / 3, h = f - 3 * j, li = s & 15, lr = (s >> 4) & 3;
    *reinterpret_cast<u32x2v*>(lds + kP16 + s * 8) = *reinterpret_cast<const u32x2v*>(wp + k16(row_p48(j, li), 16 * h + 4 * lr, 3));
  }
  for (int s = tid; s < 12 * 64; s += NTHR) {
    const int j = s >> 6, li = s & 15, lr = (s >> 4) & 3, row = row_p192(j, li);
    *reinterpret_cast<u32x4v*>(lds + kF32 + s * 16) = *reinterpret_cast<const u32x4v*>(w1 + k16(row, 8 * lr, 3));
    *reinterpret_cast<u32x2v*>(lds + kF16 + s * 8) = *reinterpret_cast<const u32x2v*>(w1 + k16(row, 32 + 4 * lr, 3));
  }
  for (int s = tid; s < 18 * 64; s += NTHR) {
    const int f = s >> 6, j = f / 6, kc = f - 6 * j, li = s & 15, lr = (s >> 4) & 3;
    *reinterpret_cast<u32x4v*>(lds + kG32 + s * 16) = *reinterpret_cast<const u32x4v*>(w2 + k16(row_p48(j, li), 32 * kc + 8 * lr, 12));
  }
  float* PV = reinterpret_cast<float*>(lds + kVec);
  const float* const srcs[9] = {g.ln1_g, g.ln1_b, g.bq, g.bkv, g.bp, g.ln2_g, g.ln2_b, g.b2, g.b1};
  const int offs[10] = {0, C, 2 * C, 3 * C, 5 * C, 6 * C, 7 * C, 8 * C, 9 * C, 9 * C + HID};
  for (int e4 = tid; e4 < (9 * C + HID) >> 2; e4 += NTHR) {
    const int e = e4 << 2;
    int k = 0;
#pragma unroll
    for (int j = 1; j < 9; ++j) k += (e >= offs[j]) ? 1 : 0;
    const float* sp = srcs[0];
    int so = offs[0];
#pragma unroll
    for (int j = 1; j < 9; ++j) if (k == j) { sp = srcs[j]; so = offs[j]; }
    *reinterpret_cast<float4*>(PV + e) = ld4g(sp + (e - so));
  }
  if (g.nln_g && tid < 2 * C / 4)
    *reinterpret_cast<float4*>(PV + 9 * C + HID + 4 * tid) = tid < C / 4 ? ld4g(g.nln_g + 4 * tid) : ld4g(g.nln_b + 4 * (tid - C / 4));
}


template <bool SAMP>
__global__ void __launch_bounds__(NTHR) __attribute__((amdgpu_waves_per_eu(4, 4))) block_fwd_wave48_kernel(const BlkFwdArgs a) {
  extern __shared__ __attribute__((aligned(1024))) char wlds[];
  const unsigned bid = blockIdx.x;
  int grp, wg, nwg;
  if (a.G == 2) { const int xcd = bid & 7; grp = xcd >> 2; wg = (int)(bid >> 3) * 4 + (xcd & 3); nwg = (int)(gridDim.x >> 3) * 4; }
  else { grp = 0; wg = bid; nwg = gridDim.x; }
  const micf_block_fwd_group& g = a.g[grp];
  stage_weights(wlds, g);
  const int tid = threadIdx.x, lane = tid & 63, wave = __builtin_amdgcn_readfirstlane(tid >> 6), li = lane & 15, lr = lane >> 4;
  const float* PV = reinterpret_cast<const float*>(wlds + kVec);
  const float *p_ln1g = PV, *p_ln1b = PV + C, *p_bq = PV + 2 * C, *p_bkv = PV + 3 * C, *p_bp = PV + 5 * C, *p_ln2g = PV + 6 * C,
              *p_ln2b = PV + 7 * C, *p_b2 = PV + 8 * C, *p_b1 = PV + 9 * C;
  const int64_t T = a.geo.T;
  const int ngroup16 = (a.geo.nwin + 1) >> 1;
  const bool cross = g.kvsrc != nullptr || (SAMP && g.hid != nullptr);
  const bool save = !(a.debug & 1), save_hg = !(a.debug & 17);
  lds_barrier();

  struct In { Row12 x, kvr; int64_t tk; float s1v, s2v; bool live0; };
  auto fetch = [&](int gt, In& in) {
    const int win = 2 * gt + (li >> 3);
    const bool live0 = win < a.geo.nwin, live = live0 && save;
    int b = 0, d = 0, hh = 0, w = 0;
    a.geo.coords(live0 ? win : 0, li & 7, b, d, hh, w);
    const int64_t tk = ((int64_t)(b * a.geo.D + d) * a.geo.H + hh) * a.geo.W + w;
    in.tk = tk; in.live0 = live0;
    in.s1v = g.s1 ? g.s1[b] : 1.f; in.s2v = g.s2 ? g.s2[b] : 1.f;
    Row12& x = in.x; Row12& kvr = in.kvr;
    x.load(g.x + tk * C, lr);
    if (!live0) x.zero();
    if (g.kvsrc) {
      kvr.load(g.kvsrc + tk * C, lr);
      if (!live0) kvr.zero();
    }
    if (SAMP && g.hid) {
      const float4 hv = ld4g(g.hid + tk * kHid + 4 * lr);
      const float mu = sum4((hv.x + hv.y) + (hv.z + hv.w)) * (1.f / kHid);
      const float d0 = hv.x - mu, d1 = hv.y - mu, d2 = hv.z - mu, d3 = hv.w - mu;
      const float rs = 1.0f / sqrtf(sum4((d0 * d0 + d1 * d1) + (d2 * d2 + d3 * d3)) * (1.f / kHid) + a.eps);
      const float4 lg = ld4g(g.ln16_g + 4 * lr), lb = ld4g(g.ln16_b + 4 * lr);
      const float g0 = gelu_f(d0 * rs * lg.x + lb.x), g1 = gelu_f(d1 * rs * lg.y + lb.y), g2 = gelu_f(d2 * rs * lg.z + lb.z),
                  g3 = gelu_f(d3 * rs * lg.w + lb.w);
      float fl[3];
#pragma unroll
      for (int ax = 0; ax < 3; ++ax) {
        const float4 wv = ld4g(g.w1c + ax * kHid + 4 * lr);
        fl[ax] = sum4((wv.x * g0 + wv.y * g1) + (wv.z * g2 + wv.w * g3));
      }
      fl[0] += ((float)d + 0.5f) / (float)a.geo.H * 2.f - 1.f;
      fl[1] += ((float)hh + 0.5f) / (float)a.geo.W * 2.f - 1.f;
      fl[2] += ((float)w + 0.5f) / (float)a.geo.D * 2.f - 1.f;
      if (live && lr < 3) g.flow[tk * 3 + lr] = lr == 0 ? fl[0] : (lr == 1 ? fl[1] : fl[2]);
      const Taps tp = make_taps(d, hh, w, fl, a.geo.D, a.geo.H, a.geo.W);
      uint32_t row0 = (uint32_t)b * (uint32_t)(a.geo.D * a.geo.H * a.geo.W);
      int lin[8]; float wgt[8]; bool okq[8];
#pragma unroll
      for (int q = 0; q < 8; ++q) {
        const int dz = q >> 2, dy = (q >> 1) & 1, dx = q & 1;
        lin[q] = 0;
        okq[q] = live0 && tp.finite && corner(tp, dz, dy, dx, a.geo.D, a.geo.H, a.geo.W, lin[q]);
        const float wx = dx ? tp.cx - tp.x0 : (tp.x0 + 1.f) - tp.cx;
        const float wy = dy ? tp.cy - tp.y0 : (tp.y0 + 1.f) - tp.cy;
        const float wz = dz ? tp.cz - tp.z0 : (tp.z0 + 1.f) - tp.cz;
        wgt[q] = okq[q] ? wx * wy * wz : 0.f;
      }
#pragma unroll
      for (int pc = 0; pc < 3; ++pc) {
        const int co = pc < 2 ? 8 * lr + 4 * pc : 32 + 4 * lr;
        float4 acc = make_float4(0.f, 0.f, 0.f, 0.f);
#pragma unroll
        for (int q0 = 0; q0 < 8; q0 += kTapBatch) {
          float4 tv[kTapBatch];
#pragma unroll
          for (int q = 0; q < kTapBatch; ++q) tv[q] = ld4g(at32(g.samp_src, ((row0 + (uint32_t)lin[q0 + q]) * C + co) * 4u));
#pragma unroll
          for (int q = 0; q < kTapBatch; ++q) {
            const bool ok = okq[q0 + q];
            const float wq = wgt[q0 + q];
            acc.x += (ok ? tv[q].x : 0.f) * wq; acc.y += (ok ? tv[q].y : 0.f) * wq; acc.z += (ok ? tv[q].z : 0.f) * wq; acc.w += (ok ? tv[q].w : 0.f) * wq;
          }
          asm volatile("" : "+v"(row0), "+v"(acc.x), "+v"(acc.y), "+v"(acc.z), "+v"(acc.w));
        }
        kvr.v[4 * pc] = acc.x; kvr.v[4 * pc + 1] = acc.y; kvr.v[4 * pc + 2] = acc.z; kvr.v[4 * pc + 3] = acc.w;
      }
    }
  };
  const int gstride = nwg * NWAVE;
  In cur, nxt;
  int gt = wg * NWAVE + wave;
  if (gt < ngroup16) fetch(gt, cur);
  for (; gt < ngroup16; gt += gstride) {
    asm volatile("" ::: "memory");
    if (gt + gstride < ngroup16) fetch(gt + gstride, nxt);
    asm volatile("" ::: "memory");
    const Row12& x = cur.x; const Row12& kvr = cur.kvr;
    const int64_t tk = cur.tk;
    const float s1v = cur.s1v, s2v = cur.s2v;
    const bool live0 = cur.live0, live = live0 && save;
    bf16x8 xnA, kvA; bf16x4_t xnB, kvB;
    {
      Row12 xn;
      float mu, rs;
      layernorm12(x, p_ln1g, p_ln1b, lr, a.eps, xn, mu, rs);
      xnA = xn.lo(); xnB = xn.hi();
      if (live) {
        if (g.xn) {
          uint16_t* o = reinterpret_cast<uint16_t*>(g.xn) + tk * C;
          st4u(o + 8 * lr, xnA); st2u(o + 32 + 4 * lr, xnB);
        }
        if (lr == 0) { g.stats[tk] = mu; g.stats[T + tk] = rs; }
      }
    }
    if (cross) {
      kvA = kvr.lo(); kvB = kvr.hi();
      if (live && g.kvs16) {
        uint16_t* o = static_cast<uint16_t*>(g.kvs16) + tk * C;
        st4u(o + 8 * lr, kvA); st2u(o + 32 + 4 * lr, kvB);
      }
    } else { kvA = xnA; kvB = xnB; }

    const f32x4 z4 = {0.f, 0.f, 0.f, 0.f};
    bf16x4_t of[3];
    {
      const bool valid = (lr >> 1) == (li >> 3);
      uint16_t* qo = reinterpret_cast<uint16_t*>(g.q) + tk * C + 4 * lr;
      uint16_t* ko = reinterpret_cast<uint16_t*>(g.kv) + tk * 2 * C + 4 * lr;
      uint16_t* oo = reinterpret_cast<uint16_t*>(g.o) + tk * C + 4 * lr;
#pragma unroll
      for (int h = 0; h < 3; ++h) {
        f32x4 qkv[3], vsw;
#pragma unroll
        for (int t = 0; t < 3; ++t) {
          const int j = 3 * t + h;
          const bf16x8 wa = frag32(wlds, kQ32, j, lane);
          const bf16x4_t wb = frag16(wlds, kQ16, j, lane);
          const f32x4 acc = mfma48(wa, wb, t == 0 ? xnA : kvA, t == 0 ? xnB : kvB);
          const float4 bs = *reinterpret_cast<const float4*>(p_bq + 16 * j + 4 * lr);
          qkv[t] = f32x4{acc[0] + bs.x, acc[1] + bs.y, acc[2] + bs.z, acc[3] + bs.w};
          if (t == 2) {
            const f32x4 u = mfma48(kvA, kvB, wa, wb);
            const float bv = p_bkv[C + 16 * h + li];
            vsw = f32x4{u[0] + bv, u[1] + bv, u[2] + bv, u[3] + bv};
          }
        }
        const bf16x4_t kf = pack4q(qkv[1]);
        if (live) {
          st2u(qo + 16 * h, pack4q(qkv[0]));
          st2u(ko + 16 * h, kf);
          st2u(ko + C + 16 * h, pack4q(qkv[2]));
        }
        const bf16x4_t qf = pack4_bf16v(qkv[0][0] * a.scale, qkv[0][1] * a.scale, qkv[0][2] * a.scale, qkv[0][3] * a.scale);
        const f32x4 st = mfma16(kf, qf, z4);
        float m = valid ? fmaxf(fmaxf(st[0], st[1]), fmaxf(st[2], st[3])) : -INFINITY;
        m = fmaxf(m, __shfl_xor(m, 16, 64));
        float e[4];
#pragma unroll
        for (int r = 0; r < 4; ++r) e[r] = valid ? expf(st[r] - m) : 0.f;
        float sum = (e[0] + e[1]) + (e[2] + e[3]);
        sum += __shfl_xor(sum, 16, 64);
        const float inv = valid ? 1.0f / sum : 0.f;
        const bf16x4_t pf = pack4_bf16v(e[0] * inv, e[1] * inv, e[2] * inv, e[3] * inv);
        of[h] = pack4q(mfma16(pack4q(vsw), pf, z4));
        if (live) st2u(oo + 16 * h, of[h]);
      }
    }

    Row12 x1;
    {
      float bp[12];
      vec12(p_bp, lr, bp);
#pragma unroll
      for (int j = 0; j < 3; ++j) {
        f32x4 acc = z4;
#pragma unroll
        for (int h = 0; h < 3; ++h) acc = mfma16(frag16(wlds, kP16, 3 * j + h, lane), of[h], acc);
#pragma unroll
        for (int r = 0; r < 4; ++r) x1.v[4 * j + r] = x.v[4 * j + r] + s1v * (acc[r] + bp[4 * j + r]);
      }
      if (!live0) x1.zero();
    }
    bf16x8 n2A; bf16x4_t n2B;
    {
      Row12 xn2;
      float mu, rs;
      layernorm12(x1, p_ln2g, p_ln2b, lr, a.eps, xn2, mu, rs);
      n2A = xn2.lo(); n2B = xn2.hi();
      if (live) {
        x1.store(g.x1 + tk * C, lr);
        uint16_t* o = reinterpret_cast<uint16_t*>(g.xn2) + tk * C;
        st4u(o + 8 * lr, n2A); st2u(o + 32 + 4 * lr, n2B);
        if (lr == 0) { g.stats[2 * T + tk] = mu; g.stats[3 * T + tk] = rs; }
      }
    }

    {
      uint16_t* ho = g.h ? static_cast<uint16_t*>(g.h) + tk * HID + 8 * lr : nullptr;
      uint16_t* go = reinterpret_cast<uint16_t*>(g.g) + tk * HID + 8 * lr;
      f32x4 y3[3] = {z4, z4, z4};
#pragma unroll
      for (int c = 0; c < 6; ++c) {
        float4 hv[2], gv[2];
#pragma unroll
        for (int u = 0; u < 2; ++u) {
          const int j = 2 * c + u;
          const f32x4 acc = mfma48(frag32(wlds, kF32, j, lane), frag16(wlds, kF16, j, lane), n2A, n2B);
          const float4 bs = *reinterpret_cast<const float4*>(p_b1 + 32 * c + 8 * lr + 4 * u);
          hv[u] = make_float4(acc[0] + bs.x, acc[1] + bs.y, acc[2] + bs.z, acc[3] + bs.w);
          gv[u] = make_float4(gelu_t<true>(hv[u].x), gelu_t<true>(hv[u].y), gelu_t<true>(hv[u].z), gelu_t<true>(hv[u].w));
        }
        const bf16x8 gf = to_bf16x8(gv[0], gv[1]);
        if (live && save_hg) {
          if (ho) st4u(ho + 32 * c, to_bf16x8(hv[0], hv[1]));
          st4u(go + 32 * c, gf);
        }
#pragma unroll
        for (int j = 0; j < 3; ++j) y3[j] = mfma32(frag32(wlds, kG32, 6 * j + c, lane), gf, y3[j]);
      }
      float b2[12];
      vec12(p_b2, lr, b2);
      Row12 y;
#pragma unroll
      for (int j = 0; j < 3; ++j)
#pragma unroll
        for (int r = 0; r < 4; ++r) y.v[4 * j + r] = x1.v[4 * j + r] + s2v * (y3[j][r] + b2[4 * j + r]);
      if (live0) y.store(g.y + tk * C, lr);
      if (g.nln_g) {
        Row12 z;
        float mu, rs;
        layernorm12(y, PV + 9 * C + HID, PV + 10 * C + HID, lr, a.eps, z, mu, rs);
        if (live0) {
          z.store(g.nln_y + tk * C, lr);
          if (lr == 0) { g.nln_mean[tk] = mu; g.nln_rstd[tk] = rs; }
          if (g.zero16) *reinterpret_cast<float4*>(g.zero16 + tk * 16 + 4 * lr) = make_float4(0.f, 0.f, 0.f, 0.f);
        }
      }
    }
    cur = nxt;
  }
}

static int launch_fwd_wave48(const BlkFwdArgs& a, hipStream_t s) {
  const int ngroup16 = (a.geo.nwin + 1) / 2;
  int nwg = (ngroup16 + NWAVE - 1) / NWAVE;
  if (nwg > 256) nwg = 256;
  const unsigned grid = a.G == 2 ? (unsigned)((nwg + 3) / 4 * 8) : (unsigned)nwg;
  static std::once_flag once;
  std::call_once(once, [] {
    (void)hipFuncSetAttribute(reinterpret_cast<const void*>(&block_fwd_wave48_kernel<false>), hipFuncAttributeMaxDynamicSharedMemorySize, 160 * 1024);
    (void)hipFuncSetAttribute(reinterpret_cast<const void*>(&block_fwd_wave48_kernel<true>), hipFuncAttributeMaxDynamicSharedMemorySize, 160 * 1024);
  });
  const bool samp = a.g[0].hid != nullptr || a.g[1].hid != nullptr;
  if (samp) hipLaunchKernelGGL((block_fwd_wave48_kernel<true>), dim3(grid), dim3(NTHR), kLdsBytes, s, a);
  else hipLaunchKernelGGL((block_fwd_wave48_kernel<false>), dim3(grid), dim3(NTHR), kLdsBytes, s, a);
  MICF_RETURN_LAUNCH();
}

}
}
```

### micformer_amd/functional.py

```python
import torch

from . import ops
from . import _lib
from ._lib import block_region

_zl = torch.zeros_like


def _in_block(fn):
    import functools

    @functools.wraps(fn)
    def wrapped(*a, **k):
        with block_region():
            return fn(*a, **k)
    return wrapped


def effective_window(dims, window):
    return tuple(d if d <= w else w for d, w in zip(dims, window))


def _padded(dims, ws):
    return tuple(d + (-d) % w for d, w in zip(dims, ws))
# ... 755 lines not shown
            dxn = ops.linear_bwd_data(dq, P["self_attn.q.weight"])
            ops.linear_bwd_data(dkv, P["self_attn.kv.weight"], out=dxn, accumulate=True)
        if padded:
            dxn = ops.crop3d(dxn, dims, pd)
        dx = ops.layernorm_bwd(dxn, xf, m1, r1, P["norm1.weight"], G["norm1.weight"], G["norm1.bias"], add=dx1, defer=_ln_defer(side))
        return (dx.reshape(B, D, H, W, C), None, None, None, None, None) + \
            tuple(_ret(t, G[k]) for k, t in zip(SELF_KEYS, ctx.tg))


class CrossBlockFn(torch.autograd.Function):
    @staticmethod
    @_in_block
    def forward(ctx, x, xa, s1, s2, heads, window, eps, *params):
        P = dict(zip(CROSS_KEYS, params))
        x, xa = _c(x), _c(xa)
        B, D, H, W, C = x.shape
        dims = (B, D, H, W)
        ws = effective_window((D, H, W), window)
        pd = _padded((D, H, W), ws)
        padded = pd != (D, H, W)
        pdims = (B,) + pd
        rps = D * H * W
        scale = (C // heads) ** -0.5
        xf, xaf = x.reshape(-1, C), xa.reshape(-1, C)
        if not padded and _fusable(dims, C, heads, ws, P):
            hd = _cross_head_fwd(xf, xaf, P, dims, eps)
            sv = ops.block_fwd([{"x": xf, "kvsrc": hd[5], "P": P, "attn": "cross_attn", "s1": s1, "s2": s2, "want_xn": False}], dims, C,
                               heads, eps, scale)[0]
            ctx.save_for_backward(xf, xaf, *hd, *[sv[k] for k in _CSV_KEYS], s1, s2, *params)
            ctx.meta = (dims, heads, eps)
            ctx.tg = _targets(params)
            ctx.fused = True
            return sv["y"].reshape(x.shape)
        ctx.fused = False
        xn, m1, r1 = ops.layernorm_fwd(xf, P["norm1.weight"], P["norm1.bias"], eps)
        xnp = ops.pad3d(xn, dims, pd) if padded else xn
        xap = ops.pad3d(xaf, dims, pd) if padded else xaf
        hid = ops.conv3_fwd(xnp, P["conv_offset.0.weight"], P["conv_offset.0.bias"], pdims, x2=xap)
        w1 = P["conv_offset.3.weight"]
        flow, xs = ops.offset_sample_fwd(hid, P["conv_offset.1.norm.weight"], P["conv_offset.1.norm.bias"], w1, xap,
                                         pdims, eps)
        q = ops.linear_fwd(xnp, P["cross_attn.q.weight"], P["cross_attn.q.bias"])
        kv = ops.linear_fwd(xs, P["cross_attn.kv.weight"], P["cross_attn.kv.bias"])
        o = ops.window_attn_fwd(q, kv, pdims, heads, ws, scale)
        if padded:
            o = ops.crop3d(o, dims, pd)
        x1 = ops.linear_fwd(o, P["cross_attn.proj.weight"], P["cross_attn.proj.bias"], resid=xf, dp_scale=s1,
                            rows_per_sample=rps)
        y, mlp_saved = _mlp_fwd(x1, dims, P, s2, eps)
        ctx.save_for_backward(xf, m1, r1, xnp, xap, hid, flow, xs, q, kv, o, x1, s1, s2, *mlp_saved, *params)
        ctx.meta = (dims, ws, pd, padded, heads, scale, eps)
        ctx.tg = _targets(params)
        return y.reshape(x.shape)

    @staticmethod
    @_in_block
    def backward(ctx, dy):
        sv = ctx.saved_tensors
        if ctx.fused:
            m = len(_CSV_KEYS)
            xf, xaf, hd = sv[0], sv[1], sv[2:8]
            svd, (s1, s2), params = dict(zip(_CSV_KEYS, sv[8:8 + m])), sv[8 + m:10 + m], sv[10 + m:]
            P = dict(zip(CROSS_KEYS, params))
            G = {k: _grad_buf(t, v) for (k, v), t in zip(P.items(), ctx.tg)}
            dims, heads, eps = ctx.meta
            C = xf.shape[1]
            rps = dims[1] * dims[2] * dims[3]
            side = all(t is not None for t in ctx.tg)
            dyf = _c(dy).reshape(-1, C)
            bo = ops.block_bwd([{"dy": dyf, "x": None, "x1": svd["x1"], "stats": svd["stats"], "q": svd["q"], "kv": svd["kv"],
                                 "h": svd["h"], "xn2": svd["xn2"], "P": P, "attn": "cross_attn", "s1": s1, "s2": s2, "cross": True,
                                 "want_copy": True}], dims, C, heads, (C // heads) ** -0.5)[0]
            xn, m1, r1, hid, flow, xsamp = hd
            _queue_block_wgrads(side, P, G, "cross_attn", svd, bo, dyf, xn, xsamp, s1, s2, rps)
            _ln_partials(side, bo["ln2_part"], bo["tiles"], C, G["norm2.weight"], G["norm2.bias"])
            dxa = ops.zero_(torch.empty_like(xaf))
            dx = _cross_head_bwd(side, P, G, dims, eps, xf, xaf, xn, m1, r1, hid, flow, bo["dx"], bo["dxs"], dxa, bo["dx1_copy"])
            shape = dims + (C,)
            return (dx.reshape(shape), dxa.reshape(shape), None, None, None, None, None) + \
                tuple(_ret(t, G[k]) for k, t in zip(CROSS_KEYS, ctx.tg))
        xf, m1, r1, xnp, xap, hid, flow, xs, q, kv, o, x1, s1, s2 = sv[:14]
        mlp_saved = sv[14:19]
        params = sv[19:]
        P = dict(zip(CROSS_KEYS, params))
        G = {k: _grad_buf(t, v) for (k, v), t in zip(P.items(), ctx.tg)}
        dims, ws, pd, padded, heads, scale, eps = ctx.meta
        B, D, H, W = dims
        pdims = (B,) + pd
        rps = D * H * W
        C = xf.shape[1]
        dy = _c(dy).reshape(-1, C)
        side = all(t is not None for t in ctx.tg)
        dx1 = _mlp_bwd(dy, x1, mlp_saved, dims, P, G, s2, side)
        _lin_wgrad(side, dx1, o, G["cross_attn.proj.weight"], G["cross_attn.proj.bias"], s1, rps)
        do = ops.linear_bwd_data(dx1, P["cross_attn.proj.weight"], dp_scale=s1, rows_per_sample=rps)
        if padded:
            do = ops.pad3d(do, dims, pd)
        dq, dkv = ops.window_attn_bwd(q, kv, do, pdims, heads, ws, scale)
        _lin_wgrad(side, dq, xnp, G["cross_attn.q.weight"], G["cross_attn.q.bias"])
        _lin_wgrad(side, dkv, xs, G["cross_attn.kv.weight"], G["cross_attn.kv.bias"])
        dxnp = ops.linear_bwd_data(dq, P["cross_attn.q.weight"])
        dxs = ops.linear_bwd_data(dkv, P["cross_attn.kv.weight"])
        dxap = ops.zero_(torch.empty_like(xap))
        dhid = ops.offset_sample_bwd(dxs, hid, P["conv_offset.1.norm.weight"], P["conv_offset.1.norm.bias"],
                                     P["conv_offset.3.weight"], xap, flow, dxap, G["conv_offset.1.norm.weight"],
                                     G["conv_offset.1.norm.bias"], G["conv_offset.3.weight"], pdims, eps)
        _defer_conv_wgrad(side, dhid, xnp, xap, G["conv_offset.0.weight"], G["conv_offset.0.bias"], pdims)
        ops.conv3_bwd_data(dhid, P["conv_offset.0.weight"], pdims, C, C, dx1=dxnp, dx2=dxap, acc1=True, acc2=True)
        if padded:
            dxn = ops.crop3d(dxnp, dims, pd)
            dxa = ops.crop3d(dxap, dims, pd)
        else:
            dxn, dxa = dxnp, dxap
        dx = ops.layernorm_bwd(dxn, xf, m1, r1, P["norm1.weight"], G["norm1.weight"], G["norm1.bias"], add=dx1, defer=_ln_defer(side))
        return (dx.reshape(B, D, H, W, C), dxa.reshape(B, D, H, W, C), None, None, None, None, None) + \
            tuple(_ret(t, G[k]) for k, t in zip(CROSS_KEYS, ctx.tg))


def _fusable(dims, C, heads, window, P):
    if tuple(window) != (2, 2, 2) or not FUSE_BLOCKS:
        return 0
    return ops.block_tile_tokens(dims, C, heads, P["mlp.fc1.weight"].shape[0])


import os as _os
FUSE_BLOCKS = True


def _queue_block_wgrads(side, P, G, attn, sv, bo, dy, xn, kv_in, s1, s2, rps):
    if bo.get("dy16") is not None:
        dy, xn = bo["dy16"], sv["xn"]
        kv_in = sv["kvs16"] if sv.get("kvs16") is not None else sv["xn"]
    _lin_wgrad(side, dy, sv["g"], G["mlp.fc2.weight"], G["mlp.fc2.bias"], s2, rps)
    _lin_wgrad(side, bo["dh"], sv["xn2"], G["mlp.fc1.weight"], G["mlp.fc1.bias"])
    _lin_wgrad(side, bo["dx1"], sv["o"], G[f"{attn}.proj.weight"], G[f"{attn}.proj.bias"], s1, rps)
    _lin_wgrad(side, bo["dq"], xn, G[f"{attn}.q.weight"], G[f"{attn}.q.bias"])
    _lin_wgrad(side, bo["dkv"], kv_in, G[f"{attn}.kv.weight"], G[f"{attn}.kv.bias"])


def _ln_partials(side, part, tiles, C, dg, db):
    item = (part, tiles, C, dg, db)
    lst = _ln_defer(side)
    if lst is not None:
        lst.append(item)
    elif _LOCAL is not None:
        _LOCAL[1].append(item)
    else:
        ops.layernorm_bwd_finish([item])


FUSE_NEXT_LN = True


def _self_fwd_fused(xs, Ps, scales, dims, heads, eps, save=True, next_ln=None):
    C = xs[0].shape[1]
    groups = [{"x": x, "kvsrc": None, "P": P, "attn": "self_attn", "s1": s[0], "s2": s[1]} for x, P, s in zip(xs, Ps, scales)]
    if next_ln is None:
        return ops.block_fwd(groups, dims, C, heads, eps, (C // heads) ** -0.5, save=save)
    hid = None
    if ops.offset_head_needs_zero(dims, C):
        hid = torch.empty((len(xs), xs[0].shape[0], 16), dtype=torch.float32, device=xs[0].device)
    for i, gd in enumerate(groups):
        gd["next_ln"] = (next_ln[i][0], next_ln[i][1], hid[i] if hid is not None else None)
    return ops.block_fwd(groups, dims, C, heads, eps, (C // heads) ** -0.5, save=save), hid


LAZY_LN_DEFAULT = True


def lazy_ln_pending():
    return len(CTX.lazy_ln)


def _self_bwd_fused(dys, xs, svs, Ps, Gs, scales, dims, heads, sides):
    C = xs[0].shape[1]
    rps = dims[1] * dims[2] * dims[3]
    groups = [{"dy": dy, "x": x, "x1": sv["x1"], "stats": sv["stats"], "q": sv["q"], "kv": sv["kv"], "h": sv["h"], "xn2": sv["xn2"], "P": P,
               "attn": "self_attn", "s1": s[0], "s2": s[1], "cross": False} for dy, x, sv, P, s in zip(dys, xs, svs, Ps, scales)]
    pres = [CTX.lazy_ln.pop(dy.data_ptr(), None) for dy in dys]
    for gd, pre in zip(groups, pres):
        if pre is not None:
            if tuple(pre["d"].shape) != tuple(gd["dy"].shape):
                raise RuntimeError("parked LayerNorm backward does not match the gradient it was parked for")
            gd["pre"] = pre
    bos = ops.block_bwd(groups, dims, C, heads, (C // heads) ** -0.5)
    for bo, pre in zip(bos, pres):
        if pre is not None:
            _ln_partials(pre["side"], bo["pre_part"], bo["tiles"], C, pre["dgamma"], pre["dbeta"])
    for dy, sv, bo, P, G, s, side in zip(dys, svs, bos, Ps, Gs, scales, sides):
        _queue_block_wgrads(side, P, G, "self_attn", sv, bo, dy, sv["xn"], sv["xn"], s[0], s[1], rps)
        _ln_partials(side, bo["ln2_part"], bo["tiles"], C, G["norm2.weight"], G["norm2.bias"])
        _ln_partials(side, bo["ln1_part"], bo["tiles"], C, G["norm1.weight"], G["norm1.bias"])
    return [bo["dx"] for bo in bos]


_SV_KEYS = ("xn", "q", "kv", "o", "x1", "xn2", "h", "g", "stats")


class SelfPairFn(torch.autograd.Function):

    @staticmethod
    @_in_block
    def forward(ctx, x, xa, sa1, sa2, sb1, sb2, heads, eps, grad_mode, *params):
        n = len(SELF_KEYS)
        Ps = [dict(zip(SELF_KEYS, params[:n])), dict(zip(SELF_KEYS, params[n:]))]
        x, xa = _c(x), _c(xa)
        B, D, H, W, C = x.shape
        dims = (B, D, H, W)
        xs = [x.reshape(-1, C), xa.reshape(-1, C)]
        _lib.set_unit("self_fwd", 2, xs[0].shape[0], C)
        scales = [(sa1, sa2), (sb1, sb2)]
        save = bool(grad_mode) and any(ctx.needs_input_grad)
        nl, CTX.next_ln, CTX.next_ln_out = CTX.next_ln, None, None
        if nl is not None and FUSE_NEXT_LN and GROUP_CROSS_HEADS and ops.block_fuses_sampler(C, heads) \
                and all(t.numel() == C and t.device == x.device for pr in nl for t in pr):
            svs, hid = _self_fwd_fused(xs, Ps, scales, dims, heads, eps, save=save, next_ln=nl)
            CTX.next_ln_out = ((svs[0]["y"].data_ptr(), svs[1]["y"].data_ptr()), [svs[0]["nln"], svs[1]["nln"]], hid)
        else:
            svs = _self_fwd_fused(xs, Ps, scales, dims, heads, eps, save=save)
        if save:
            ctx.save_for_backward(*xs, *[sv[k] for sv in svs for k in _SV_KEYS], sa1, sa2, sb1, sb2, *params)
            ctx.meta = (dims, heads)
            ctx.tg = _targets(params)
        return svs[0]["y"].reshape(x.shape), svs[1]["y"].reshape(x.shape)

    @staticmethod
    @_in_block
    def backward(ctx, dy, dya):
        sv = ctx.saved_tensors
        dims, heads = ctx.meta
        n, m = len(SELF_KEYS), len(_SV_KEYS)
        xs = list(sv[:2])
        svs = [dict(zip(_SV_KEYS, sv[2:2 + m])), dict(zip(_SV_KEYS, sv[2 + m:2 + 2 * m]))]
        sa1, sa2, sb1, sb2 = sv[2 + 2 * m:6 + 2 * m]
        params = sv[6 + 2 * m:]
        Ps = [dict(zip(SELF_KEYS, params[:n])), dict(zip(SELF_KEYS, params[n:]))]
        tgs = [ctx.tg[:n], ctx.tg[n:]]
        Gs = [_grad_bufs(P, tg) for P, tg in zip(Ps, tgs)]
        sides = [all(t is not None for t in tg) for tg in tgs]
        C = xs[0].shape[1]
        _lib.set_unit("self_bwd", 2, xs[0].shape[0], C)
        dys = [_c(dy).reshape(-1, C), _c(dya).reshape(-1, C)]
        with _local_batch():
            dxs = _self_bwd_fused(dys, xs, svs, Ps, Gs, [(sa1, sa2), (sb1, sb2)], dims, heads, sides)
        shape = dims + (C,)
        grads = tuple(_ret(t, G[k]) for G, tg in zip(Gs, tgs) for k, t in zip(SELF_KEYS, tg))
        return (dxs[0].reshape(shape), dxs[1].reshape(shape), None, None, None, None, None, None, None) + grads


def _cross_head_fwd(xf, xaf, P, dims, eps):
    xn, m1, r1 = ops.layernorm_fwd(xf, P["norm1.weight"], P["norm1.bias"], eps)
    hid = ops.conv3_fwd(xn, P["conv_offset.0.weight"], P["conv_offset.0.bias"], dims, x2=xaf)
    flow, xs = ops.offset_sample_fwd(hid, P["conv_offset.1.norm.weight"], P["conv_offset.1.norm.bias"], P["conv_offset.3.weight"], xaf,
                                     dims, eps)
    return xn, m1, r1, hid, flow, xs


def _cross_head_bwd(side, P, G, dims, eps, xf, xaf, xn, m1, r1, hid, flow, dxq, dxs, dxa_acc, add, out=None):
    C = xf.shape[1]
    dhid = ops.offset_sample_bwd(dxs, hid, P["conv_offset.1.norm.weight"], P["conv_offset.1.norm.bias"], P["conv_offset.3.weight"],
                                 xaf, flow, dxa_acc, G["conv_offset.1.norm.weight"], G["conv_offset.1.norm.bias"],
                                 G["conv_offset.3.weight"], dims, eps)
    _defer_conv_wgrad(side, dhid, xn, xaf, G["conv_offset.0.weight"], G["conv_offset.0.bias"], dims)
    ops.conv3_bwd_data(dhid, P["conv_offset.0.weight"], dims, C, C, dx1=dxq, dx2=dxa_acc, acc1=True, acc2=True)
    return ops.layernorm_bwd(dxq, xf, m1, r1, P["norm1.weight"], G["norm1.weight"], G["norm1.bias"], add=add, defer=_ln_defer(side),
                             out=out)


_CSV_KEYS = ("q", "kv", "o", "x1", "xn2", "h", "g", "stats", "xn", "kvs16")

OVERLAP_CROSS_HEADS = True
GROUP_CROSS_HEADS = True
FUSE_SAMPLER = True


def _conv_offset_wgrad(side, dhid, xn, xa, G, dims):
    _defer_conv_wgrad(side, dhid, xn, xa, G["conv_offset.0.weight"], G["conv_offset.0.bias"], dims)
_SIDE = {}


def _side_stream(device):
    st = _SIDE.get(device)
    if st is None:
        st = _SIDE[device] = torch.cuda.Stream(device=device)
    return st


def _cross_head_adjoint(i, hds, bos, Ps, Gs, xs, acc, dims, eps, C, sides):
    xn, m1, r1, hid, flow, xsamp = hds[i]
    dhid = ops.offset_sample_bwd(bos[i]["dxs"], hid, Ps[i]["conv_offset.1.norm.weight"], Ps[i]["conv_offset.1.norm.bias"],
                                 Ps[i]["conv_offset.3.weight"], xs[1 - i], flow, acc[1 - i], Gs[i]["conv_offset.1.norm.weight"],
                                 Gs[i]["conv_offset.1.norm.bias"], Gs[i]["conv_offset.3.weight"], dims, eps)
    _defer_conv_wgrad(sides[i], dhid, xn, xs[1 - i], Gs[i]["conv_offset.0.weight"], Gs[i]["conv_offset.0.bias"], dims)
    ops.conv3_bwd_data(dhid, Ps[i]["conv_offset.0.weight"], dims, C, C, dx1=bos[i]["dx"], dx2=acc[1 - i], acc1=True, acc2=True)


class CrossPairFn(torch.autograd.Function):

    @staticmethod
    @_in_block
    def forward(ctx, x, xa, sa1, sa2, sb1, sb2, heads, eps, grad_mode, *params):
        n = len(CROSS_KEYS)
        Ps = [dict(zip(CROSS_KEYS, params[:n])), dict(zip(CROSS_KEYS, params[n:]))]
        x, xa = _c(x), _c(xa)
        ctx.lazy_ln = CTX.cross_after_self == (x.data_ptr(), xa.data_ptr())
        CTX.cross_after_self = None
        B, D, H, W, C = x.shape
        dims = (B, D, H, W)
        xs = [x.reshape(-1, C), xa.reshape(-1, C)]
        _lib.set_unit("cross_fwd", 2, xs[0].shape[0], C)
        fuse_sampler = GROUP_CROSS_HEADS and FUSE_SAMPLER and ops.block_fuses_sampler(C, heads)
        if GROUP_CROSS_HEADS:
            pre, CTX.next_ln_out = CTX.next_ln_out, None
            if pre is not None and pre[0] == (xs[0].data_ptr(), xs[1].data_ptr()):
                lns, hid = pre[1], pre[2]
            else:
                hid = None
                if ops.offset_head_needs_zero(dims, C):
                    hid = torch.empty((2, xs[0].shape[0], 16), dtype=torch.float32, device=x.device)
                lns = ops.layernorm_fwd_pair(xs, [P["norm1.weight"] for P in Ps], [P["norm1.bias"] for P in Ps], eps, zero=hid)
            outs = ops.offset_head_fwd([{"xn": lns[i][0], "xa": xs[1 - i], "P": Ps[i]} for i in (0, 1)], dims, eps, hid,
                                       sample=not fuse_sampler)
            heads_ = [lns[i] + outs[i] for i in (0, 1)]
        elif OVERLAP_CROSS_HEADS:
            main, side = torch.cuda.current_stream(), _side_stream(x.device)
            side.wait_stream(main)
            h0 = _cross_head_fwd(xs[0], xs[1], Ps[0], dims, eps)
            with torch.cuda.stream(side):
                h1 = _cross_head_fwd(xs[1], xs[0], Ps[1], dims, eps)
            main.wait_stream(side)
            for t in h1:
                t.record_stream(main)
            heads_ = [h0, h1]
        else:
            heads_ = [_cross_head_fwd(xs[i], xs[1 - i], Ps[i], dims, eps) for i in (0, 1)]
        scales = [(sa1, sa2), (sb1, sb2)]
        groups = [{"x": xs[i], "kvsrc": heads_[i][5], "P": Ps[i], "attn": "cross_attn", "s1": scales[i][0], "s2": scales[i][1],
                   "want_xn": False} for i in (0, 1)]
        if fuse_sampler:
            for i in (0, 1):
                groups[i].update(kvsrc=None, hid=heads_[i][3], samp_src=xs[1 - i])
        save = bool(grad_mode) and any(ctx.needs_input_grad)
        svs = ops.block_fwd(groups, dims, C, heads, eps, (C // heads) ** -0.5, save=save)
        if not save:
            return svs[0]["y"].reshape(x.shape), svs[1]["y"].reshape(x.shape)
        if fuse_sampler:
            heads_ = [heads_[i][:4] + (svs[i]["flow"], svs[i]["xs32"]) for i in (0, 1)]
        ctx.save_for_backward(*xs, *[t for hd in heads_ for t in hd], *[sv[k] for sv in svs for k in _CSV_KEYS], sa1, sa2, sb1, sb2,
                              *params)
        ctx.meta = (dims, heads, eps)
        ctx.tg = _targets(params)
        return svs[0]["y"].reshape(x.shape), svs[1]["y"].reshape(x.shape)

    @staticmethod
    @_in_block
    @_batched
    def backward(ctx, dy, dya):
        sv = ctx.saved_tensors
        dims, heads, eps = ctx.meta
        n, m = len(CROSS_KEYS), len(_CSV_KEYS)
        xs = list(sv[:2])
        hds = [sv[2:8], sv[8:14]]
        svs = [dict(zip(_CSV_KEYS, sv[14:14 + m])), dict(zip(_CSV_KEYS, sv[14 + m:14 + 2 * m]))]
        sa1, sa2, sb1, sb2 = sv[14 + 2 * m:18 + 2 * m]
        scales = [(sa1, sa2), (sb1, sb2)]
        params = sv[18 + 2 * m:]
        Ps = [dict(zip(CROSS_KEYS, params[:n])), dict(zip(CROSS_KEYS, params[n:]))]
        tgs = [ctx.tg[:n], ctx.tg[n:]]
        Gs = [_grad_bufs(P, tg) for P, tg in zip(Ps, tgs)]
        sides = [all(t is not None for t in tg) for tg in tgs]
        C = xs[0].shape[1]
        _lib.set_unit("cross_bwd", 2, xs[0].shape[0], C)
        rps = dims[1] * dims[2] * dims[3]
        dys = [_c(dy).reshape(-1, C), _c(dya).reshape(-1, C)]
        groups = [{"dy": dys[i], "x": None, "x1": svs[i]["x1"], "stats": svs[i]["stats"], "q": svs[i]["q"], "kv": svs[i]["kv"],
                   "h": svs[i]["h"], "xn2": svs[i]["xn2"], "P": Ps[i], "attn": "cross_attn", "s1": scales[i][0], "s2": scales[i][1], "cross": True,
                   "want_copy": True} for i in (0, 1)]
        bos = ops.block_bwd(groups, dims, C, heads, (C // heads) ** -0.5)
        acc = [bos[0]["dx1_copy"], bos[1]["dx1_copy"]]
        for i in (0, 1):
            xn, m1, r1, hid, flow, xsamp = hds[i]
            _queue_block_wgrads(sides[i], Ps[i], Gs[i], "cross_attn", svs[i], bos[i], dys[i], xn, xsamp, scales[i][0], scales[i][1], rps)
            _ln_partials(sides[i], bos[i]["ln2_part"], bos[i]["tiles"], C, Gs[i]["norm2.weight"], Gs[i]["norm2.bias"])
        if GROUP_CROSS_HEADS:
            hgroups = [{"dxs": bos[i]["dxs"], "hid": hds[i][3], "flow": hds[i][4], "xa": xs[1 - i], "P": Ps[i],
                        "G": Gs[i], "dxa": acc[1 - i], "dxn": bos[i]["dx"]} for i in (0, 1)]
            defer_ws = None
            if all(sides) and CTX.defer_calls and CTX.defer_wgrad and ops.offset_head_finish_deferrable(dims):
                defer_ws = torch.empty(ops.offset_head_bwd_workspace(2, dims), dtype=torch.float32, device=xs[0].device)
            dhids = ops.offset_head_bwd(hgroups, dims, eps, defer_ws=defer_ws)
            if defer_ws is not None:
                def fin():
                    ops.offset_head_bwd_finish(hgroups, dhids, dims, defer_ws)
                fin.finish = (hgroups, dhids, tuple(dims), defer_ws)
                _defer(True, fin, defer_ws, *dhids)
            for i in (0, 1):
                _conv_offset_wgrad(sides[i], dhids[i], hds[i][0], xs[1 - i], Gs[i], dims)
        else:
            main = torch.cuda.current_stream()
            side = _side_stream(dys[0].device) if OVERLAP_CROSS_HEADS else None
            if side is not None:
                side.wait_stream(main)
            for i in (0, 1):
                with torch.cuda.stream(side if (i == 1 and side is not None) else main):
                    _cross_head_adjoint(i, hds, bos, Ps, Gs, xs, acc, dims, eps, C, sides)
            if side is not None:
                main.wait_stream(side)
        lazy = (ctx.lazy_ln and CTX.lazy_ln_ok and GROUP_CROSS_HEADS and all(sides) and CTX.defer_wgrad and bos[0].get("dy16") is not None
                and ops.block_fuses_sampler(C, heads))
        if lazy:
            for i in (0, 1):
                CTX.lazy_ln[acc[i].data_ptr()] = {"d": bos[i]["dx"], "x": xs[i], "mean": hds[i][1], "rstd": hds[i][2],
                                               "gamma": Ps[i]["norm1.weight"], "dgamma": Gs[i]["norm1.weight"],
                                               "dbeta": Gs[i]["norm1.bias"], "side": sides[i]}
        elif GROUP_CROSS_HEADS:
            ops.layernorm_bwd_pair([{"dy": bos[i]["dx"], "x": xs[i], "mean": hds[i][1], "rstd": hds[i][2], "gamma": Ps[i]["norm1.weight"],
                                     "dgamma": Gs[i]["norm1.weight"], "dbeta": Gs[i]["norm1.bias"], "add": acc[i], "out": acc[i]}
                                    for i in (0, 1)], [_ln_defer(sides[i]) for i in (0, 1)])
        else:
            for i in (0, 1):
                xn, m1, r1 = hds[i][:3]
                ops.layernorm_bwd(bos[i]["dx"], xs[i], m1, r1, Ps[i]["norm1.weight"], Gs[i]["norm1.weight"], Gs[i]["norm1.bias"],
                                  add=acc[i], defer=_ln_defer(sides[i]), out=acc[i])
        shape = dims + (C,)
        grads = tuple(_ret(t, G[k]) for G, tg in zip(Gs, tgs) for k, t in zip(CROSS_KEYS, tg))
        return (acc[0].reshape(shape), acc[1].reshape(shape), None, None, None, None, None, None, None) + grads


PATCH_GEMM = True
class PatchEmbedFn(torch.autograd.Function):

    @staticmethod
    def forward(ctx, vol, mod, w, b, p):
        vol = _c(vol)
        B, nmod, D, H, W = vol.shape
        E = w.shape[0]
        if PATCH_GEMM and w.shape[1] == 1 and p in (2, 4):
            a = ops.space_to_depth(vol, (B, D, H, W), 1, p, batch_stride=nmod * D * H * W, offset=mod * D * H * W)
            y = ops.linear_fwd(a, w.reshape(E, p ** 3), b).reshape(B, -(-D // p), -(-H // p), -(-W // p), E)
            ctx.save_for_backward(a, w)
        else:
            y = ops.patch_embed_fwd(vol, mod, w, b, p)
            ctx.save_for_backward(vol, w)
        ctx.meta = (mod, p, PATCH_GEMM and w.shape[1] == 1 and p in (2, 4))
        ctx.tg = _targets((w, b))
        return y

    @staticmethod
    def backward(ctx, dy):
        vol, w = ctx.saved_tensors
        mod, p, gemm = ctx.meta
        dw = _grad_buf(ctx.tg[0], w)
        db = ctx.tg[1] if ctx.tg[1] is not None else torch.zeros(w.shape[0], dtype=w.dtype, device=w.device)
        dy = _c(dy)
        if gemm:
            _lin_wgrad(ctx.tg[0] is not None and ctx.tg[1] is not None, dy.reshape(-1, w.shape[0]), vol, dw.view(w.shape[0], -1), db)
        else:
            _defer(ctx.tg[0] is not None and ctx.tg[1] is not None, lambda: ops.patch_embed_bwd_weight(dy, vol, mod, dw, db, p), dy, vol)
        return None, None, _ret(ctx.tg[0], dw), _ret(ctx.tg[1], db), None


class PatchRowsEmbedFn(torch.autograd.Function):

    @staticmethod
    def forward(ctx, a, w, b):
        E = w.shape[0]
        ctx.save_for_backward(a, w)
        ctx.tg = _targets((w, b))
        return ops.linear_fwd(a, w.reshape(E, -1), b)

    @staticmethod
    def backward(ctx, dy):
        a, w = ctx.saved_tensors
        dw = _grad_buf(ctx.tg[0], w)
        db = ctx.tg[1] if ctx.tg[1] is not None else torch.zeros(w.shape[0], dtype=w.dtype, device=w.device)
        _lin_wgrad(ctx.tg[0] is not None and ctx.tg[1] is not None, _c(dy).reshape(-1, w.shape[0]), a, dw.view(w.shape[0], -1), db)
        return None, _ret(ctx.tg[0], dw), _ret(ctx.tg[1], db)


class PatchEmbedPairFn(torch.autograd.Function):

    @staticmethod
    def forward(ctx, vol, w, b, p):
        vol = _c(vol)
        B, nmod, D, H, W = vol.shape
        E = w.shape[0]
        rows = B * (-(-D // p)) * (-(-H // p)) * (-(-W // p))
        a = torch.empty((2 * rows, p ** 3), dtype=torch.float32, device=vol.device)
        for m in (0, 1):
            ops.space_to_depth(vol, (B, D, H, W), 1, p, batch_stride=nmod * D * H * W, offset=m * D * H * W, out=a[m * rows:(m + 1) * rows])
        ctx.save_for_backward(a, w)
        ctx.tg = _targets((w, b))
        return ops.linear_fwd(a, w.reshape(E, p ** 3), b).reshape(2 * B, -(-D // p), -(-H // p), -(-W // p), E)

    @staticmethod
    def backward(ctx, dy):
        a, w = ctx.saved_tensors
        dw = _grad_buf(ctx.tg[0], w)
        db = ctx.tg[1] if ctx.tg[1] is not None else torch.zeros(w.shape[0], dtype=w.dtype, device=w.device)
        _lin_wgrad(ctx.tg[0] is not None and ctx.tg[1] is not None, _c(dy).reshape(-1, w.shape[0]), a, dw.view(w.shape[0], -1), db)
        return None, _ret(ctx.tg[0], dw), _ret(ctx.tg[1], db), None


SKIP_MAIL = True


class _SkipToken:
    __slots__ = ("grad", "mailed", "received", "consumed")

    def __init__(self):
        self.grad = None
        self.mailed = self.received = 0
        self.consumed = False


def clear_skip_tokens():
    CTX.skip_tokens.clear()


def skip_token(t):
    return CTX.skip_tokens.get((t.data_ptr(), tuple(t.shape))) if SKIP_MAIL else None


class SkipMailFn(torch.autograd.Function):
    @staticmethod
    def forward(ctx, t, token):
        ctx.token = token
        token.mailed += 1
        return t.view_as(t)

# ... 220 lines not shown
```

### micformer_amd/ops.py

```python
import ctypes

import torch

from . import _lib
from ._lib import call, f32, ptr


DETAIL = False

_COMPUTE_DTYPE = "fp32"


def compute_dtype():
    return _COMPUTE_DTYPE


def _dt():
    return 1 if _COMPUTE_DTYPE == "bf16" else 0


def set_compute_dtype(name):
    global _COMPUTE_DTYPE, _ATTN_FP8
    if name not in ("fp32", "bf16", "bf16+fp8attn"):
        raise ValueError("compute dtype must be 'fp32', 'bf16' or 'bf16+fp8attn'")
# ... 836 lines not shown
         ("ln2_g", "norm2.weight"), ("ln2_b", "norm2.bias"), ("b1", "mlp.fc1.bias"), ("b2", "mlp.fc2.bias"))
FWD_WM = (("wq", "{a}.q.weight"), ("wkv", "{a}.kv.weight"), ("wp", "{a}.proj.weight"), ("w1", "mlp.fc1.weight"), ("w2", "mlp.fc2.weight"))
BWD_W = (("ln1_g", "norm1.weight"), ("ln2_g", "norm2.weight"))
BWD_WT = (("wqt", "{a}.q.weight"), ("wkvt", "{a}.kv.weight"), ("wpt", "{a}.proj.weight"), ("w1t", "mlp.fc1.weight"),
          ("w2t", "mlp.fc2.weight"))


def block_tile_tokens(dims, C, heads, hidden, backward=False):
    B, D, H, W = dims
    return int(_lib.lib.micf_block_tile_tokens(B, D, H, W, C, heads, hidden, 1 if backward else 0))


def blocked16(w):
    R, Cn = w.shape
    return w.reshape(R // 16, 16, Cn // 16, 16).permute(0, 2, 1, 3).contiguous().reshape(R, Cn)


class WeightPrepPlan:

    def __init__(self, triples, blocked=False):
        self.triples = list(triples)
        self.n = len(self.triples)
        self.arr = (_lib.WeightPrepItem * max(self.n, 1))()
        self.nbytes = 0
        for it, (src, dst, dst_t) in zip(self.arr, self.triples):
            outs = [t for t in (dst, dst_t) if t is not None]
            assert outs and len({t.dtype for t in outs}) == 1 and outs[0].dtype in (torch.float32, torch.bfloat16)
            it.src, it.dst, it.dst_t, it.rows, it.cols = f32(src), ptr(dst), ptr(dst_t), src.shape[0], src.shape[1]
            it.bf16 = (2 if blocked else 1) if outs[0].dtype == torch.bfloat16 else (3 if blocked else 0)
            self.nbytes += src.numel() * (4 + sum(t.element_size() for t in outs))

    def launch(self):
        if self.n:
            call("micf_weight_prep_grouped", ctypes.cast(self.arr, ctypes.c_void_p), self.n,
                 cost=(self.nbytes, 0) if _lib.PROFILE is not None else None)


class Conv3PrepPlan:

    def __init__(self, triples):
        self.triples = list(triples)
        self.n = len(self.triples)
        self.arr = (_lib.Conv3PrepItem * max(self.n, 1))()
        for it, (w, fwd, bwd) in zip(self.arr, self.triples):
            it.w, it.fwd, it.bwd, it.N, it.Cin = f32(w), f32(fwd), f32(bwd), w.shape[0], w.shape[1]

    def launch(self):
        if self.n:
            call("micf_conv3_weight_prep_grouped", ctypes.cast(self.arr, ctypes.c_void_p), self.n)


def conv3_prepared_like(w):
    N, Cin = w.shape[0], w.shape[1]
    nf, nb = _lib.lib.micf_conv3_fwd_workspace(N, Cin, 0), _lib.lib.micf_conv3_bwd_data_workspace(N, Cin, 0)
    mk = lambda n: torch.empty(n, dtype=torch.float32, device=w.device) if n > 0 else None
    return mk(nf), mk(nb)


_SHADOW = {("fp32", False): ("_micf_w32", False, torch.float32), ("fp32", True): ("_micf_wt", True, torch.float32),
           ("bf16", False): ("_micf_w16", False, torch.bfloat16),
           ("bf16", True): ("_micf_wt16", True, torch.bfloat16)}


ENGINE_SHADOWS = False


def shadow_spec(backward):
    return _SHADOW.get((compute_dtype(), bool(backward)))


def shadow_like(w, transposed, dtype):
    return torch.empty((w.shape[1], w.shape[0]) if transposed else tuple(w.shape), dtype=dtype, device=w.device)


PARAM_EPOCH = [0]


def _inference_cache(w, key, build):
    if torch.is_grad_enabled():
        return None
    cache = w.__dict__.setdefault("_micf_cache", {})
    ent = cache.get(key)
    stamp = (w._version, PARAM_EPOCH[0])
    if ent is None or ent[0] != stamp:
        ent = cache[key] = (stamp, build())
    return ent[1]


def _conv_layouts(w):
    f, b = (getattr(w, "_micf_c3f", None), getattr(w, "_micf_c3b", None)) if ENGINE_SHADOWS else (None, None)
    if f is None and b is None and w.dim() == 5 and w.shape[0] <= 16:
        def build():
            fb = conv3_prepared_like(w)
            if fb[0] is not None or fb[1] is not None:
                Conv3PrepPlan([(w, fb[0], fb[1])]).launch()
            return fb
        fb = _inference_cache(w, "conv3", build)
        if fb is not None:
            f, b = fb
    return f, b


def block_weights(P, attn, backward, only=None):
    fields = BWD_WT if backward else FWD_WM
    if only is not None:
        fields = tuple(f for f in fields if f[0] in only)
    spec = shadow_spec(backward)
    if spec is None:
        return {field: P[key.format(a=attn)] for field, key in fields}
    fspec, bspec = shadow_spec(False), shadow_spec(True)
    out, todo = {}, []
    for field, key in fields:
        w = P[key.format(a=attn)]
        sh = getattr(w, spec[0], None) if ENGINE_SHADOWS else None
        if sh is None:
            cache = w.__dict__.setdefault("_micf_cache", {})
            stamp = (w._version, PARAM_EPOCH[0], compute_dtype())
            ent = cache.get("shadows")
            if ent is None or ent[0] != stamp:
                fwd = shadow_like(w, fspec[1], fspec[2]) if fspec is not None else None
                bwd = shadow_like(w, bspec[1], bspec[2])
                ent = cache["shadows"] = (stamp, fwd, bwd)
                todo.append((w, fwd, bwd))
            sh = ent[2] if backward else ent[1]
        out[field] = sh
    if todo:
        WeightPrepPlan(todo, blocked=True).launch()
    return out


def _block_cost(nb, fl, groups, T, C, hidden, self_passes, cross_passes):
    if _lib.PROFILE is None:
        return None
    e = 2 if _dt() else 4
    s8d = 0
    for gd in groups:
        cross = gd.get("cross", gd.get("kvsrc") is not None or gd.get("hid") is not None)
        s8d += (cross_passes if cross else self_passes) * T * C * e + (4 * C * C + 2 * C * hidden) * e
    return (nb, fl, f"{len(groups)}x{T}x{C}" if DETAIL else None, s8d)


def block_fuses_sampler(C, heads):
    return bool(_lib.lib.micf_block_fuses_sampler(C, heads))


def block_saves_bf16(C, heads):
    return bool(_lib.lib.micf_block_saves_bf16(C, heads, _dt()))


def block_recomputes_h(C, heads):
    return bool(_lib.lib.micf_block_recomputes_h(C, heads))


def block_fwd(groups, dims, C, heads, eps, scale, persist_probe=None, save=True):
    B, D, H, W = dims
    T = B * D * H * W
    hidden = groups[0]["P"]["mlp.fc1.weight"].shape[0]
    arr = (_lib.BlockFwdGroup * 2)()
    outs = []
    h_dtype = torch.bfloat16 if _dt() else torch.float32
    st16 = block_saves_bf16(C, heads)
    sd = torch.bfloat16 if st16 else torch.float32
    no_h = block_recomputes_h(C, heads)
    keep = []
    nb = fl = 0
    y_all = _new(groups[0]["x"], len(groups) * T, C)
    for gi, (it, gd) in enumerate(zip(arr, groups)):
        x, P, a = gd["x"], gd["P"], gd["attn"]
        fused_sampler = gd.get("hid") is not None
        cross = gd.get("kvsrc") is not None or fused_sampler
        if not save and block_fuses_sampler(C, heads) and persist_probe is None:
            o = dict.fromkeys(("q", "kv", "o", "x1", "xn2", "h", "g", "stats", "xn", "kvs16", "flow", "xs32"))
            o["y"] = y_all[gi * T:(gi + 1) * T]
        else:
            o = {"y": y_all[gi * T:(gi + 1) * T], "q": _new(x, T, C, dtype=sd), "kv": _new(x, T, 2 * C, dtype=sd),
                 "o": _new(x, T, C, dtype=sd), "x1": _new(x, T, C), "xn2": _new(x, T, C, dtype=sd),
                 "h": None if no_h else _new(x, T, hidden, dtype=h_dtype), "g": _new(x, T, hidden, dtype=sd), "stats": _new(x, 4, T),
                 "xn": _new(x, T, C, dtype=sd) if (gd.get("want_xn", True) or st16) else None,
                 "kvs16": _new(x, T, C, dtype=sd) if (st16 and cross) else None,
                 "flow": _new(x, T, 3) if fused_sampler else None,
                 "xs32": _new(x, T, C) if (fused_sampler and not st16) else None}
        it.x, it.kvsrc, it.s1, it.s2 = f32(x), f32(gd.get("kvsrc")), f32(gd.get("s1")), f32(gd.get("s2"))
        if fused_sampler:
            it.hid, it.samp_src = f32(gd["hid"]), f32(gd["samp_src"])
            it.ln16_g, it.ln16_b, it.w1c = (f32(P[k]) for k in ("conv_offset.1.norm.weight", "conv_offset.1.norm.bias", "conv_offset.3.weight"))
        nl = gd.get("next_ln")
        if nl is not None:
            o["nln"] = (_new(x, T, C), _new(x, T), _new(x, T))
            it.nln_g, it.nln_b, it.zero16 = f32(nl[0]), f32(nl[1]), f32(nl[2])
            it.nln_y, it.nln_mean, it.nln_rstd = (f32(t) for t in o["nln"])
            nb += 4 * T * (C + 2)
        for field, key in FWD_W:
            setattr(it, field, f32(P[key.format(a=a)]))
        wts = block_weights(P, a, backward=False)
        keep.append(wts)
        for field, wt in wts.items():
            setattr(it, field, ptr(wt))
        for k, v in o.items():
            if k != "nln":
                setattr(it, k, ptr(v))
        outs.append(o)
        nb += 4 * T * C * (2 if cross else 1) + (64 * T if fused_sampler else 0) \
            + sum(v.numel() * v.element_size() for k, v in o.items() if v is not None and k != "nln") \
            + 12 * C * C * wt.element_size()
        fl += 2 * T * 12 * C * C + 4 * T * C * 8
    if persist_probe is not None:
        call("micf_block_fwd_persistent_probe", ctypes.cast(arr, ctypes.c_void_p), len(groups), B, D, H, W, C, heads, hidden, float(eps),
             float(scale), _dt(), int(persist_probe[0]), ptr(persist_probe[1]))
        return outs
    call("micf_block_fwd", ctypes.cast(arr, ctypes.c_void_p), len(groups), B, D, H, W, C, heads, hidden, float(eps), float(scale),
         _dt_attn(), cost=_block_cost(nb, fl, groups, T, C, hidden, 2, 3))
    return outs


def block_bwd(groups, dims, C, heads, scale):
    B, D, H, W = dims
    T = B * D * H * W
    hidden = groups[0]["P"]["mlp.fc1.weight"].shape[0]
    tm = block_tile_tokens(dims, C, heads, hidden, backward=True)
    tiles = (T + tm - 1) // tm
    arr = (_lib.BlockBwdGroup * 2)()
    outs = []
    keep = []
    nb = fl = 0
    st16 = block_saves_bf16(C, heads)
    sd = torch.bfloat16 if st16 else torch.float32
    dx_all = _new(groups[0]["dy"], len(groups) * T, C)
    copy_all = _new(groups[0]["dy"], len(groups) * T, C) if all(gd.get("want_copy") for gd in groups) else None
    for gi, (it, gd) in enumerate(zip(arr, groups)):
        dy, P, a, cross = gd["dy"], gd["P"], gd["attn"], gd["cross"]
        o = {"dx": dx_all[gi * T:(gi + 1) * T], "dxs": _new(dy, T, C) if cross else None, "dx1": _new(dy, T, C, dtype=sd),
             "dh": _new(dy, T, hidden, dtype=sd), "dq": _new(dy, T, C, dtype=sd), "dkv": _new(dy, T, 2 * C, dtype=sd),
             "ln2_part": _new(dy, tiles, 2 * C), "ln1_part": None if cross else _new(dy, tiles, 2 * C),
             "dx1_copy": (copy_all[gi * T:(gi + 1) * T] if copy_all is not None else _new(dy, T, C)) if gd.get("want_copy") else None,
             "dy16": _new(dy, T, C, dtype=sd) if st16 else None}
        for k in ("dy", "x", "x1", "stats", "s1", "s2"):
            setattr(it, k, f32(gd.get(k)))
        h = gd.get("h")
        if (h is not None and h.dtype != (torch.bfloat16 if _dt() else torch.float32)) or gd["q"].dtype != sd or gd["kv"].dtype != sd \
                or (h is None and gd["xn2"].dtype != sd):
            raise _lib.MicfError("block_bwd: the saved tensors were written in another arithmetic mode")
        it.h, it.q, it.kv = ptr(h), ptr(gd["q"]), ptr(gd["kv"])
        pre = gd.get("pre")
        if pre is not None:
            if not st16 or cross:
                raise _lib.MicfError("block_bwd: the LayerNorm-backward prologue needs a self block with bf16 storage")
            o["pre_part"] = _new(dy, tiles, 2 * C)
            it.pre_d, it.pre_x, it.pre_mean, it.pre_rstd, it.pre_g, it.pre_part = (f32(pre["d"]), f32(pre["x"]), f32(pre["mean"]),
                                                                                  f32(pre["rstd"]), f32(pre["gamma"]), f32(o["pre_part"]))
            nb += 4 * T * C * 2
        if h is None:
            w1 = block_weights(P, a, backward=False, only=("w1",))["w1"]
            keep.append(w1)
            it.xn2, it.w1, it.b1 = ptr(gd["xn2"]), ptr(w1), f32(P["mlp.fc1.bias"])
        for field, key in BWD_W:
            setattr(it, field, f32(P[key.format(a=a)]))
        wts = block_weights(P, a, backward=True)
        keep.append(wts)
        for field, wt in wts.items():
            setattr(it, field, ptr(wt))
        for k, v in o.items():
            setattr(it, k, ptr(v))
        nb += 4 * T * C * (2 if cross else 3) + sum(gd[k].numel() * gd[k].element_size() for k in ("q", "kv", "h" if h is not None else "xn2")) \
            + sum(v.numel() * v.element_size() for v in o.values() if v is not None) + 12 * C * C * wt.element_size()
        o["tiles"] = tiles
        outs.append(o)
        fl += 2 * T * 12 * C * C + 8 * T * C * 8
    call("micf_block_bwd", ctypes.cast(arr, ctypes.c_void_p), len(groups), B, D, H, W, C, heads, hidden, float(scale),
         _dt(), cost=_block_cost(nb, fl, groups, T, C, hidden, 3, 5))
    del keep
    return outs


def _coords(chunk):
    arr = (ctypes.c_int32 * (4 * len(chunk)))()
    for i, (b, z, y, x) in enumerate(chunk):
        arr[4 * i:4 * i + 4] = [b, z, y, x]
    return arr


def sw_window_batch(vol, chunk, roi):
    B, C, D, H, W = vol.shape
    rd, rh, rw = roi
    win = _new(vol, len(chunk), C, rd, rh, rw)
    arr = _coords(chunk)
    call("micf_sw_window_batch", f32(vol), f32(win), ctypes.cast(arr, ctypes.c_void_p), len(chunk), B, C, D, H, W, rd, rh, rw)
    return win


def sw_accumulate_batch(pred, out, count, chunk):
    B, K, D, H, W = out.shape
    rd, rh, rw = pred.shape[2:]
    arr = _coords(chunk)
    call("micf_sw_accumulate_batch", f32(pred), f32(out), f32(count), ctypes.cast(arr, ctypes.c_void_p), len(chunk), B, K, D, H, W,
         rd, rh, rw)


def intensity_stats(vol):
    B, Cm = vol.shape[:2]
    if vol.dtype not in (torch.float16, torch.float32):
        raise TypeError("raw volume must be float16 or float32")
    sums = torch.empty(B * Cm * 3, dtype=torch.float64, device=vol.device)
    call("micf_intensity_stats", ptr(vol), 1 if vol.dtype == torch.float16 else 0, ptr(sums), B, Cm, vol[0, 0].numel())
    return sums


def patch_rows_prepared(vol, sums, params, k):
    B, Cm, D, H, W = vol.shape
    rows = B * (-(-D // k)) * (-(-H // k)) * (-(-W // k))
    both = torch.empty((Cm * rows, k ** 3), dtype=torch.float32, device=vol.device)
    outs = [both[m * rows:(m + 1) * rows] for m in range(Cm)]
    call("micf_patch_rows_prepared", ptr(vol), 1 if vol.dtype == torch.float16 else 0, ptr(sums), f32(params), f32(outs[0]),
         f32(outs[1]) if Cm > 1 else None, B, Cm, D, H, W, k, cost=_cost(0, vol, *outs))
    return outs


def flip_labels(label_map, params):
    if params is None:
        return label_map
    B, D, H, W = label_map.shape
    out = torch.empty_like(label_map)
    dummy = torch.zeros(3 * B, dtype=torch.float64, device=label_map.device)
    call("micf_input_prepare", ptr(label_map), 0, ptr(dummy), f32(params), None, ptr(label_map), ptr(out), B, 1, D, H, W)
    return out


def input_prepare(vol, label_map=None, params=None):
    B, Cm, D, H, W = vol.shape
    if vol.dtype not in (torch.float16, torch.float32):
        raise TypeError("raw volume must be float16 or float32")
    half = 1 if vol.dtype == torch.float16 else 0
    sums = torch.empty(B * Cm * 3, dtype=torch.float64, device=vol.device)
    call("micf_intensity_stats", ptr(vol), half, ptr(sums), B, Cm, D * H * W)
    out = torch.empty((B, Cm, D, H, W), dtype=torch.float32, device=vol.device)
    lab_out = torch.empty_like(label_map) if label_map is not None else None
    if label_map is not None and label_map.dtype != torch.uint8:
        raise TypeError("label map must be uint8")
    call("micf_input_prepare", ptr(vol), half, ptr(sums), f32(params), f32(out), ptr(label_map), ptr(lab_out), B, Cm, D, H, W)
    return out, lab_out


def zero_(t):
    call("micf_zero", ptr(t), t.numel() * t.element_size())
    return t


def drop_path_rng(device, seed):
    return torch.tensor([int(seed) & 0x7FFFFFFFFFFFFFFF, 0], dtype=torch.int64, device=device)


def drop_path_draw(rng, keep, batch):
    n = keep.numel()
    out = _new(keep, n, batch)
    call("micf_drop_path_draw", ptr(rng), f32(keep), f32(out), n, batch)
    return out
```

Baseline: 233.0 pairs/s.

## Recompute MLP hidden and QKV in wave48 backward instead of saving them

The stage-1 (C=48) wave-private block kernels stop writing the MLP hidden activation and the q/kv projections in forward. Backward now rebuilds them from the saved bf16 LayerNorm outputs with MFMA, using fc1 and qkv weights staged in LDS. This removes large activation writes and reads, with hidden being 4C per token, at the cost of extra matmul work. The rebuild kernel uses 16 waves per workgroup and more LDS, which may lower occupancy. It is on by default through an environment toggle that can select none, h only, or full rebuild.

Result: faster. 242.4 pairs/s (median of 6 runs) (+4.0%).

```diff
diff --git a/include/micformer_hip.h b/include/micformer_hip.h
--- a/include/micformer_hip.h
+++ b/include/micformer_hip.h
@@ -313,6 +313,10 @@
   const float *pre_mean, *pre_rstd;
   const float* pre_g;
   float* pre_part;
+  const void* xn;
+  const void* kvs16;
+  const void *wq, *wkv;
+  const float *bq, *bkv;
 } micf_block_bwd_group;
 int micf_block_recomputes_h(int C, int heads);
 int micf_block_tile_tokens(int B, int D, int H, int W, int C, int heads, int hidden, int backward);
diff --git a/micformer_amd/_lib.py b/micformer_amd/_lib.py
--- a/micformer_amd/_lib.py
+++ b/micformer_amd/_lib.py
@@ -146,7 +146,7 @@
 class BlockBwdGroup(ctypes.Structure):
     FIELDS = ("dy", "x", "x1", "stats", "q", "kv", "h", "ln1_g", "ln2_g", "wqt", "wkvt", "wpt", "w1t", "w2t", "s1", "s2",
               "dx", "dxs", "dx1", "dh", "dq", "dkv", "ln1_part", "ln2_part", "dx1_copy", "dy16", "xn2", "w1", "b1",
-              "pre_d", "pre_x", "pre_mean", "pre_rstd", "pre_g", "pre_part")
+              "pre_d", "pre_x", "pre_mean", "pre_rstd", "pre_g", "pre_part", "xn", "kvs16", "wq", "wkv", "bq", "bkv")
     _fields_ = [(n, _VP) for n in FIELDS]
 
 
diff --git a/micformer_amd/csrc/block_bwd.hip b/micformer_amd/csrc/block_bwd.hip
--- a/micformer_amd/csrc/block_bwd.hip
+++ b/micformer_amd/csrc/block_bwd.hip
@@ -593,9 +593,13 @@
   if (TM == 0) return MICF_EUNSUPPORTED;
   if (dtype != MICF_DTYPE_F32 && dtype != MICF_DTYPE_BF16) return MICF_EINVAL;
   BlkBwdArgs a;
+  const micf_block_bwd_group& g0 = groups[0], &g1 = groups[ngroups - 1];
+  const bool wave = options().block_wave != 0 && C == 48 && C / heads == 16 && TM == 32 && dtype == MICF_DTYPE_BF16 &&
+                    (g0.dxs != nullptr) == (g1.dxs != nullptr) && (g0.pre_d != nullptr) == (g1.pre_d != nullptr) && !(g0.dxs && g0.pre_d) &&
+                    (int64_t)B * D * H * W * hidden * 2 < ((int64_t)1 << 31);
   for (int i = 0; i < ngroups; ++i) {
     const micf_block_bwd_group& g = groups[i];
-    const void* need[] = {g.dy, g.x1, g.stats, g.q, g.kv, g.ln2_g, g.wqt, g.wkvt, g.wpt, g.w1t, g.w2t, g.dx, g.dx1, g.dh, g.dq, g.dkv};
+    const void* need[] = {g.dy, g.x1, g.stats, g.ln2_g, g.wqt, g.wkvt, g.wpt, g.w1t, g.w2t, g.dx, g.dx1, g.dh, g.dq, g.dkv};
     for (const void* p : need)
       if (!p || (reinterpret_cast<uintptr_t>(p) & 15)) return MICF_EINVAL;
     if (g.h) {
@@ -604,9 +608,17 @@
       const void* re[] = {g.xn2, g.w1, g.b1};
       for (const void* p : re)
         if (!p || (reinterpret_cast<uintptr_t>(p) & 15)) return MICF_EINVAL;
-      if (!micf_block_recomputes_h(C, heads)) return MICF_EINVAL;
-    }
-    if (i > 0 && (g.h == nullptr) != (groups[0].h == nullptr)) return MICF_EINVAL;
+      if (!wave && !micf_block_recomputes_h(C, heads)) return MICF_EINVAL;
+    }
+    if (g.q) {
+      if (!g.kv || ((reinterpret_cast<uintptr_t>(g.q) | reinterpret_cast<uintptr_t>(g.kv)) & 15)) return MICF_EINVAL;
+    } else {
+      if (g.kv || g.h || !wave) return MICF_EINVAL;
+      const void* re[] = {g.xn, g.wq, g.wkv, g.bq, g.bkv, g.dxs ? g.kvs16 : g.xn};
+      for (const void* p : re)
+        if (!p || (reinterpret_cast<uintptr_t>(p) & 15)) return MICF_EINVAL;
+    }
+    if (i > 0 && ((g.h == nullptr) != (groups[0].h == nullptr) || (g.q == nullptr) != (groups[0].q == nullptr))) return MICF_EINVAL;
     if (g.pre_d) {
       const void* pr[] = {g.pre_d, g.pre_x, g.pre_mean, g.pre_rstd, g.pre_g, g.pre_part, g.dy16};
       for (const void* p : pr)
@@ -629,9 +641,7 @@
   if ((int64_t)2 * H * W * (TM / 8 + 1) * hidden * (int64_t)sizeof(float) >= (int64_t)1 << 32) return MICF_EUNSUPPORTED;
   if (block_wide_tile_tokens(C, hd)) return block_bwd_wide(groups, ngroups, B, D, H, W, C, heads, scale, dtype, s);
   {
-    if (options().block_wave != 0 && C == 48 && hd == 16 && tj == 2 && dtype == MICF_DTYPE_BF16 && a.attn_mfma && a.g[0].h && a.g[1].h && (a.g[0].dxs != nullptr) == (a.g[1].dxs != nullptr) &&
-        (a.g[0].pre_d != nullptr) == (a.g[1].pre_d != nullptr) && !(a.g[0].dxs && a.g[0].pre_d) &&
-        a.geo.T * (int64_t)hidden * 2 < ((int64_t)1 << 31))
+    if (wave)
     {
       if (options().block_debug & 1) a.attn_mfma |= 2;
       return wave48::launch_bwd_wave48(a, s);
diff --git a/micformer_amd/csrc/block_fwd.hip b/micformer_amd/csrc/block_fwd.hip
--- a/micformer_amd/csrc/block_fwd.hip
+++ b/micformer_amd/csrc/block_fwd.hip
@@ -493,6 +493,8 @@
   return block_saves_bf16(C, C / heads, dtype) ? 1 : 0;
 }
 
+static bool cross_group(const micf_block_fwd_group& g) { return g.kvsrc != nullptr || g.hid != nullptr; }
+
 extern "C" int micf_block_fwd(const micf_block_fwd_group* groups, int ngroups, int B, int D, int H, int W, int C, int heads,
                               int hidden, float eps, float scale, int dtype, micf_stream_t stream) {
   if (!groups || ngroups < 1 || ngroups > 2) return MICF_EINVAL;
@@ -504,6 +506,8 @@
   BlkFwdArgs a;
   a.att8 = att8 ? 2 : (dtype == MICF_DTYPE_BF16 ? 1 : 0);
   int nosave = -1;
+  const bool wave = options().block_wave != 0 && C == 48 && C / heads == 16 && dtype == MICF_DTYPE_BF16 && !att8 &&
+                    !(options().block_debug & ~17) && (int64_t)B * D * H * W * C * 4 < ((int64_t)1 << 32);
   for (int i = 0; i < ngroups; ++i) {
     const micf_block_fwd_group& g = groups[i];
     const void* must[] = {g.x, g.ln1_g, g.ln1_b, g.wq, g.bq, g.wkv, g.bkv, g.wp, g.bp, g.ln2_g, g.ln2_b, g.w1, g.b1, g.w2, g.b2, g.y};
@@ -518,9 +522,12 @@
     if (ns) {
       if (block_wide_tile_tokens(C, C / heads)) return MICF_EUNSUPPORTED;
     } else {
-      for (const void* p : saves)
-        if (!p || (reinterpret_cast<uintptr_t>(p) & 15)) return MICF_EINVAL;
-      if (g.h ? (reinterpret_cast<uintptr_t>(g.h) & 15) != 0 : !micf_block_recomputes_h(C, heads)) return MICF_EINVAL;
+      const bool noqkv = !g.q && !g.kv && !g.h && wave;
+      for (int k = 0; k < 7; ++k)
+        if ((!saves[k] && !(noqkv && k < 2)) || (reinterpret_cast<uintptr_t>(saves[k]) & 15)) return MICF_EINVAL;
+      if (noqkv && (!g.xn || (cross_group(g) && !g.kvs16))) return MICF_EINVAL;
+      if (i > 0 && (g.q == nullptr) != (groups[0].q == nullptr)) return MICF_EINVAL;
+      if (g.h ? (reinterpret_cast<uintptr_t>(g.h) & 15) != 0 : !(wave || micf_block_recomputes_h(C, heads))) return MICF_EINVAL;
     }
     if ((g.kvsrc && (reinterpret_cast<uintptr_t>(g.kvsrc) & 15)) || (g.xn && (reinterpret_cast<uintptr_t>(g.xn) & 15)) ||
         (g.kvs16 && (reinterpret_cast<uintptr_t>(g.kvs16) & 15))) return MICF_EINVAL;
@@ -549,8 +556,7 @@
   hipStream_t s = (hipStream_t)stream;
   const int hd = C / heads, tj = TM / 16;
   if (block_wide_tile_tokens(C, hd)) return block_fwd_wide(groups, ngroups, B, D, H, W, C, heads, eps, scale, att8 ? MICF_DTYPE_BF16_ATTN_FP8 : dtype, s);
-  if (options().block_wave != 0 && C == 48 && hd == 16 && dtype == MICF_DTYPE_BF16 && a.att8 == 1 && !(a.debug & ~17) &&
-      a.geo.T * (int64_t)C * 4 < ((int64_t)1 << 32))
+  if (wave)
     return wave48::launch_fwd_wave48(a, s);
 #define MICF_BF(C_, HD_, TJ_) if (C == C_ && hd == HD_ && tj == TJ_) return launch_fwd<C_, HD_, TJ_>(a, dtype, s)
   MICF_BF(48, 16, 2); MICF_BF(96, 16, 1); MICF_BF(192, 16, 1);
diff --git a/micformer_amd/csrc/block_wave.h b/micformer_amd/csrc/block_wave.h
--- a/micformer_amd/csrc/block_wave.h
+++ b/micformer_amd/csrc/block_wave.h
@@ -17,6 +17,22 @@
 }
 __device__ __forceinline__ bf16x4_t frag16(const char* lds, int base, int f, int lane) {
   return *reinterpret_cast<const bf16x4_t*>(lds + base + (f * 64 + lane) * 8);
+}
+__device__ __forceinline__ void stage_qkv_fwd(char* lds, int b32, int b16, const uint16_t* wq, const uint16_t* wkv, int tid, int nthr) {
+  for (int s = tid; s < 9 * 64; s += nthr) {
+    const int j = s >> 6, li = s & 15, lr = (s >> 4) & 3;
+    const uint16_t* W = j < 3 ? wq : wkv;
+    const int row = 16 * (j < 3 ? j : j - 3) + li;
+    *reinterpret_cast<u32x4v*>(lds + b32 + s * 16) = *reinterpret_cast<const u32x4v*>(W + k16(row, 8 * lr, 3));
+    *reinterpret_cast<u32x2v*>(lds + b16 + s * 8) = *reinterpret_cast<const u32x2v*>(W + k16(row, 32 + 4 * lr, 3));
+  }
+}
+__device__ __forceinline__ void stage_fc1_fwd(char* lds, int b32, int b16, const uint16_t* w1, int tid, int nthr) {
+  for (int s = tid; s < 12 * 64; s += nthr) {
+    const int j = s >> 6, li = s & 15, lr = (s >> 4) & 3, row = row_p192(j, li);
+    *reinterpret_cast<u32x4v*>(lds + b32 + s * 16) = *reinterpret_cast<const u32x4v*>(w1 + k16(row, 8 * lr, 3));
+    *reinterpret_cast<u32x2v*>(lds + b16 + s * 8) = *reinterpret_cast<const u32x2v*>(w1 + k16(row, 32 + 4 * lr, 3));
+  }
 }
 __device__ __forceinline__ f32x4 mfma32(const bf16x8& a, const bf16x8& b, const f32x4& c) { return __builtin_amdgcn_mfma_f32_16x16x32_bf16(a, b, c, 0, 0, 0); }
 __device__ __forceinline__ f32x4 mfma16(const bf16x4_t& a, const bf16x4_t& b, const f32x4& c) { return __builtin_amdgcn_mfma_f32_16x16x16bf16_1k(a, b, c, 0, 0, 0); }
diff --git a/micformer_amd/csrc/block_wave_bwd.h b/micformer_amd/csrc/block_wave_bwd.h
--- a/micformer_amd/csrc/block_wave_bwd.h
+++ b/micformer_amd/csrc/block_wave_bwd.h
@@ -13,11 +13,21 @@
 constexpr int kBQ = kBPh + 3 * 512;
 constexpr int kBKV = kBQ + 9 * 512;
 constexpr int kBVec = kBKV + 18 * 512;
-constexpr int kBPark = kBVec + 3 * C * 4;
+constexpr int kBRF32 = kBVec + 3 * C * 4;
+constexpr int kBRF16 = kBRF32 + 12 * 1024;
+constexpr int kBRB1 = kBRF16 + 12 * 512;
+constexpr int kBRQ32 = kBRB1 + HID * 4;
+constexpr int kBRQ16 = kBRQ32 + 9 * 1024;
+constexpr int kBRBq = kBRQ16 + 9 * 512;
+constexpr int bwd_waves(int rb) { return rb ? 16 : NWAVE; }
+constexpr int bwd_park(int rb) { return rb == 0 ? kBRF32 : (rb == 1 ? kBRQ32 : kBRBq + 3 * C * 4); }
 constexpr int kParkFloats = 4 * (16 * 12 + 8);
-constexpr int kBwdLdsBytes = kBPark + NWAVE * kParkFloats * 4;
-
+constexpr int bwd_lds_bytes(int rb) { return bwd_park(rb) + bwd_waves(rb) * kParkFloats * 4; }
+static_assert(bwd_lds_bytes(0) == 81472 && 2 * bwd_lds_bytes(0) <= 160 * 1024 && bwd_lds_bytes(2) <= 160 * 1024, "LDS budget of the wave-private backward");
+
+template <int RB>
 __device__ __forceinline__ void stage_weights_bwd(char* lds, const micf_block_bwd_group& g) {
+  constexpr int NTHR = 64 * bwd_waves(RB);
   const uint16_t* wqt = static_cast<const uint16_t*>(g.wqt), *wkvt = static_cast<const uint16_t*>(g.wkvt), *wpt = static_cast<const uint16_t*>(g.wpt),
                  *w1t = static_cast<const uint16_t*>(g.w1t), *w2t = static_cast<const uint16_t*>(g.w2t);
   const int tid = threadIdx.x;
@@ -48,6 +58,16 @@
     const float* src = e < C ? g.ln1_g : (e < 2 * C ? g.ln2_g : g.pre_g);
     PV[e] = src ? src[e % C] : 0.f;
   }
+  if (RB >= 1) {
+    stage_fc1_fwd(lds, kBRF32, kBRF16, static_cast<const uint16_t*>(g.w1), tid, NTHR);
+    float* b1 = reinterpret_cast<float*>(lds + kBRB1);
+    for (int e = tid; e < HID; e += NTHR) b1[e] = g.b1[e];
+  }
+  if (RB == 2) {
+    stage_qkv_fwd(lds, kBRQ32, kBRQ16, static_cast<const uint16_t*>(g.wq), static_cast<const uint16_t*>(g.wkv), tid, NTHR);
+    float* bq = reinterpret_cast<float*>(lds + kBRBq);
+    for (int e = tid; e < 3 * C; e += NTHR) bq[e] = e < C ? g.bq[e] : g.bkv[e - C];
+  }
 }
 
 __device__ __forceinline__ void park12(float* tile, int lr, int li, const float (&v)[12]) {
@@ -99,15 +119,16 @@
   for (int w = 0; w < 4; ++w) { o[2 * w] = __uint_as_float(u[w] << 16); o[2 * w + 1] = __uint_as_float(u[w] & 0xFFFF0000u); }
 }
 
-template <bool CROSS, bool PRE>
-__global__ void __launch_bounds__(NTHR) __attribute__((amdgpu_waves_per_eu(4, 4))) block_bwd_wave48_kernel(const BlkBwdArgs a) {
+template <bool CROSS, bool PRE, int RB>
+__global__ void __launch_bounds__(64 * bwd_waves(RB)) __attribute__((amdgpu_waves_per_eu(4, 4))) block_bwd_wave48_kernel(const BlkBwdArgs a) {
+  constexpr int NWAVE = bwd_waves(RB), kBPark = bwd_park(RB);
   extern __shared__ __attribute__((aligned(1024))) char wlds[];
   const unsigned bid = blockIdx.x;
   int grp, wg, nwg;
   if (a.G == 2) { const int xcd = bid & 7; grp = xcd >> 2; wg = (int)(bid >> 3) * 4 + (xcd & 3); nwg = (int)(gridDim.x >> 3) * 4; }
   else { grp = 0; wg = bid; nwg = gridDim.x; }
   const micf_block_bwd_group& g = a.g[grp];
-  stage_weights_bwd(wlds, g);
+  stage_weights_bwd<RB>(wlds, g);
   const int tid = threadIdx.x, lane0 = tid & 63, wave = __builtin_amdgcn_readfirstlane(tid >> 6);
   const float* PV = reinterpret_cast<const float*>(wlds + kBVec);
   const float *p_ln1g = PV, *p_ln2g = PV + C, *p_preg = PV + 2 * C;
@@ -156,13 +177,19 @@
       const bf16x4_t dyB = dy.hi();
       park12(tile, lr, li, dy.v);
       u32x4v hreg[6];
-      {
+      bf16x8 n2A = {};
+      bf16x4_t n2B = {};
+      if (RB == 0) {
         const uint16_t* hp = static_cast<const uint16_t*>(g.h);
 #pragma unroll
         for (int c = 0; c < 6; ++c) {
           hreg[c] = *reinterpret_cast<const u32x4v*>(at32(hp, (tk * HID + 32 * c + 8 * lr) * 2u));
           if (!live) hreg[c] = u32x4v{0u, 0u, 0u, 0u};
         }
+      } else {
+        const uint16_t* np = reinterpret_cast<const uint16_t*>(g.xn2);
+        n2A = *reinterpret_cast<const bf16x8*>(at32(np, (rowC + 8 * lr) * 2u));
+        n2B = *reinterpret_cast<const bf16x4_t*>(at32(np, (rowC + 32 + 4 * lr) * 2u));
       }
 
       f32x4 dn2[3] = {z4, z4, z4};
@@ -171,7 +198,21 @@
 #pragma unroll
         for (int c = 0; c < 6; ++c) {
           float h8[8];
-          unpack8(hreg[c], h8);
+          if (RB == 0) {
+            unpack8(hreg[c], h8);
+          } else {
+            float4 hv[2];
+#pragma unroll
+            for (int u = 0; u < 2; ++u) {
+              const int j = 2 * c + u;
+              const f32x4 acc = mfma48(frag32(wlds, kBRF32, j, lane), frag16(wlds, kBRF16, j, lane), n2A, n2B);
+              const float4 bs = *reinterpret_cast<const float4*>(reinterpret_cast<const float*>(wlds + kBRB1) + 32 * c + 8 * lr + 4 * u);
+              hv[u] = make_float4(acc[0] + bs.x, acc[1] + bs.y, acc[2] + bs.z, acc[3] + bs.w);
+            }
+            u32x4v hq = __builtin_bit_cast(u32x4v, to_bf16x8(hv[0], hv[1]));
+            if (!live) hq = u32x4v{0u, 0u, 0u, 0u};
+            unpack8(hq, h8);
+          }
           float4 dv[2];
 #pragma unroll
           for (int u = 0; u < 2; ++u) {
@@ -189,13 +230,40 @@
       const uint16_t* qp = reinterpret_cast<const uint16_t*>(g.q);
       const uint16_t* kp = reinterpret_cast<const uint16_t*>(g.kv);
       bf16x4_t qn, kn, vn;
+      bf16x8 xnA = {}, kvA = {};
+      bf16x4_t xnB = {}, kvB = {};
       auto load_head = [&](int h) {
+        if (RB == 2) {
+          bf16x4_t r[3];
+#pragma unroll
+          for (int t = 0; t < 3; ++t) {
+            const int j = 3 * t + h;
+            const bool own = t == 0 || !cross;
+            const f32x4 acc = mfma48(frag32(wlds, kBRQ32, j, lane), frag16(wlds, kBRQ16, j, lane), own ? xnA : kvA, own ? xnB : kvB);
+            const float4 bs = *reinterpret_cast<const float4*>(reinterpret_cast<const float*>(wlds + kBRBq) + 16 * j + 4 * lr);
+            r[t] = pack4q(f32x4{acc[0] + bs.x, acc[1] + bs.y, acc[2] + bs.z, acc[3] + bs.w});
+          }
+          qn = r[0]; kn = r[1]; vn = r[2];
+          if (!live) { qn = bf16x4_t{0, 0, 0, 0}; kn = qn; vn = qn; }
+          return;
+        }
         qn = *reinterpret_cast<const bf16x4_t*>(at32(qp, (rowC + 16 * h + 4 * lr) * 2u));
         kn = *reinterpret_cast<const bf16x4_t*>(at32(kp, (2 * rowC + 16 * h + 4 * lr) * 2u));
         vn = *reinterpret_cast<const bf16x4_t*>(at32(kp, (2 * rowC + C + 16 * h + 4 * lr) * 2u));
         if (!live) { qn = bf16x4_t{0, 0, 0, 0}; kn = qn; vn = qn; }
       };
-      load_head(0);
+      if (RB == 2) {
+        const uint16_t* xp = reinterpret_cast<const uint16_t*>(g.xn);
+        xnA = *reinterpret_cast<const bf16x8*>(at32(xp, (rowC + 8 * lr) * 2u));
+        xnB = *reinterpret_cast<const bf16x4_t*>(at32(xp, (rowC + 32 + 4 * lr) * 2u));
+        if (cross) {
+          const uint16_t* sp = static_cast<const uint16_t*>(g.kvs16);
+          kvA = *reinterpret_cast<const bf16x8*>(at32(sp, (rowC + 8 * lr) * 2u));
+          kvB = *reinterpret_cast<const bf16x4_t*>(at32(sp, (rowC + 32 + 4 * lr) * 2u));
+        }
+      } else {
+        load_head(0);
+      }
       Row12 x1;
       x1.load(at32(g.x1, rowC * 4u), lr);
       float mu2 = *at32(g.stats, (2 * T + tk) * 4u), rs2 = *at32(g.stats, (3 * T + tk) * 4u);
@@ -241,9 +309,10 @@
         uint16_t* dko = reinterpret_cast<uint16_t*>(g.dkv);
 #pragma unroll
         for (int h = 0; h < 3; ++h) {
+          if (RB == 2) load_head(h);
           const bf16x4_t qcur = qn, kf = kn, vf = vn;
-          if (h < 2) load_head(h + 1);
-          else if (!cross) {
+          if (RB != 2 && h < 2) load_head(h + 1);
+          if (h == 2 && !cross) {
             x.load(at32(g.x, rowC * 4u), lr);
             mu1 = *at32(g.stats, tk * 4u); rs1 = *at32(g.stats, (T + tk) * 4u);
             if (!live) { x.zero(); mu1 = 0.f; rs1 = 0.f; }
@@ -342,22 +411,33 @@
   }
 }
 
-static int launch_bwd_wave48(const BlkBwdArgs& a, hipStream_t s) {
-  int nwg = (a.tiles + NWAVE - 1) / NWAVE;
-  if (nwg > 256) nwg = 256;
+template <bool CROSS, bool PRE, int RB>
+static void launch_bwd_wave48_form(const BlkBwdArgs& a, hipStream_t s) {
+  constexpr int NW = bwd_waves(RB);
+  int nwg = (a.tiles + NW - 1) / NW;
+  if (nwg > 2048 / NW) nwg = 2048 / NW;
   const unsigned grid = a.G == 2 ? (unsigned)((nwg + 3) / 4 * 8) : (unsigned)nwg;
   static std::once_flag once;
   std::call_once(once, [] {
-    (void)hipFuncSetAttribute(reinterpret_cast<const void*>(&block_bwd_wave48_kernel<true, false>), hipFuncAttributeMaxDynamicSharedMemorySize, 160 * 1024);
-    (void)hipFuncSetAttribute(reinterpret_cast<const void*>(&block_bwd_wave48_kernel<false, true>), hipFuncAttributeMaxDynamicSharedMemorySize, 160 * 1024);
-    (void)hipFuncSetAttribute(reinterpret_cast<const void*>(&block_bwd_wave48_kernel<false, false>), hipFuncAttributeMaxDynamicSharedMemorySize, 160 * 1024);
+    (void)hipFuncSetAttribute(reinterpret_cast<const void*>(&block_bwd_wave48_kernel<CROSS, PRE, RB>), hipFuncAttributeMaxDynamicSharedMemorySize, 160 * 1024);
   });
+  hipLaunchKernelGGL((block_bwd_wave48_kernel<CROSS, PRE, RB>), dim3(grid), dim3(64 * NW), bwd_lds_bytes(RB), s, a);
+}
+
+template <int RB>
+static int launch_bwd_wave48_rb(const BlkBwdArgs& a, hipStream_t s) {
   const bool cross = a.g[0].dxs != nullptr, pre = a.g[0].pre_d != nullptr;
-  if (cross) hipLaunchKernelGGL((block_bwd_wave48_kernel<true, false>), dim3(grid), dim3(NTHR), kBwdLdsBytes, s, a);
-  else if (pre) hipLaunchKernelGGL((block_bwd_wave48_kernel<false, true>), dim3(grid), dim3(NTHR), kBwdLdsBytes, s, a);
-  else hipLaunchKernelGGL((block_bwd_wave48_kernel<false, false>), dim3(grid), dim3(NTHR), kBwdLdsBytes, s, a);
+  if (cross) launch_bwd_wave48_form<true, false, RB>(a, s);
+  else if (pre) launch_bwd_wave48_form<false, true, RB>(a, s);
+  else launch_bwd_wave48_form<false, false, RB>(a, s);
   MICF_RETURN_LAUNCH();
 }
 
-}
-}
+static int launch_bwd_wave48(const BlkBwdArgs& a, hipStream_t s) {
+  if (a.g[0].q == nullptr) return launch_bwd_wave48_rb<2>(a, s);
+  if (a.g[0].h == nullptr) return launch_bwd_wave48_rb<1>(a, s);
+  return launch_bwd_wave48_rb<0>(a, s);
+}
+
+}
+}
diff --git a/micformer_amd/csrc/block_wave_fwd.h b/micformer_amd/csrc/block_wave_fwd.h
--- a/micformer_amd/csrc/block_wave_fwd.h
+++ b/micformer_amd/csrc/block_wave_fwd.h
@@ -21,22 +21,12 @@
   const uint16_t* wq = static_cast<const uint16_t*>(g.wq), *wkv = static_cast<const uint16_t*>(g.wkv), *wp = static_cast<const uint16_t*>(g.wp),
                  *w1 = static_cast<const uint16_t*>(g.w1), *w2 = static_cast<const uint16_t*>(g.w2);
   const int tid = threadIdx.x;
-  for (int s = tid; s < 9 * 64; s += NTHR) {
-    const int j = s >> 6, li = s & 15, lr = (s >> 4) & 3;
-    const uint16_t* W = j < 3 ? wq : wkv;
-    const int row = 16 * (j < 3 ? j : j - 3) + li;
-    *reinterpret_cast<u32x4v*>(lds + kQ32 + s * 16) = *reinterpret_cast<const u32x4v*>(W + k16(row, 8 * lr, 3));
-    *reinterpret_cast<u32x2v*>(lds + kQ16 + s * 8) = *reinterpret_cast<const u32x2v*>(W + k16(row, 32 + 4 * lr, 3));
-  }
+  stage_qkv_fwd(lds, kQ32, kQ16, wq, wkv, tid, NTHR);
   for (int s = tid; s < 9 * 64; s += NTHR) {
     const int f = s >> 6, j = f / 3, h = f - 3 * j, li = s & 15, lr = (s >> 4) & 3;
     *reinterpret_cast<u32x2v*>(lds + kP16 + s * 8) = *reinterpret_cast<const u32x2v*>(wp + k16(row_p48(j, li), 16 * h + 4 * lr, 3));
   }
-  for (int s = tid; s < 12 * 64; s += NTHR) {
-    const int j = s >> 6, li = s & 15, lr = (s >> 4) & 3, row = row_p192(j, li);
-    *reinterpret_cast<u32x4v*>(lds + kF32 + s * 16) = *reinterpret_cast<const u32x4v*>(w1 + k16(row, 8 * lr, 3));
-    *reinterpret_cast<u32x2v*>(lds + kF16 + s * 8) = *reinterpret_cast<const u32x2v*>(w1 + k16(row, 32 + 4 * lr, 3));
-  }
+  stage_fc1_fwd(lds, kF32, kF16, w1, tid, NTHR);
   for (int s = tid; s < 18 * 64; s += NTHR) {
     const int f = s >> 6, j = f / 6, kc = f - 6 * j, li = s & 15, lr = (s >> 4) & 3;
     *reinterpret_cast<u32x4v*>(lds + kG32 + s * 16) = *reinterpret_cast<const u32x4v*>(w2 + k16(row_p48(j, li), 32 * kc + 8 * lr, 12));
@@ -206,7 +196,7 @@
           }
         }
         const bf16x4_t kf = pack4q(qkv[1]);
-        if (live) {
+        if (live && g.q) {
           st2u(qo + 16 * h, pack4q(qkv[0]));
           st2u(ko + 16 * h, kf);
           st2u(ko + C + 16 * h, pack4q(qkv[2]));
diff --git a/micformer_amd/functional.py b/micformer_amd/functional.py
--- a/micformer_amd/functional.py
+++ b/micformer_amd/functional.py
@@ -931,9 +931,18 @@
 FUSE_NEXT_LN = True
 
 
+BLOCK_REBUILD = {"0": False, "h": "h"}.get(_os.environ.get("MICF_BLOCK_REBUILD", ""), True)
+
+
+def _rebuild(dims, C, heads, P):
+    return BLOCK_REBUILD if BLOCK_REBUILD and ops.block_rebuilds(dims, C, heads, P["mlp.fc1.weight"].shape[0]) else False
+
+
 def _self_fwd_fused(xs, Ps, scales, dims, heads, eps, save=True, next_ln=None):
     C = xs[0].shape[1]
     groups = [{"x": x, "kvsrc": None, "P": P, "attn": "self_attn", "s1": s[0], "s2": s[1]} for x, P, s in zip(xs, Ps, scales)]
+    for gd in groups:
+        gd["rebuild"] = _rebuild(dims, C, heads, Ps[0])
     if next_ln is None:
         return ops.block_fwd(groups, dims, C, heads, eps, (C // heads) ** -0.5, save=save)
     hid = None
@@ -954,7 +963,7 @@
 def _self_bwd_fused(dys, xs, svs, Ps, Gs, scales, dims, heads, sides):
     C = xs[0].shape[1]
     rps = dims[1] * dims[2] * dims[3]
-    groups = [{"dy": dy, "x": x, "x1": sv["x1"], "stats": sv["stats"], "q": sv["q"], "kv": sv["kv"], "h": sv["h"], "xn2": sv["xn2"], "P": P,
+    groups = [{"dy": dy, "x": x, "x1": sv["x1"], "stats": sv["stats"], "q": sv["q"], "kv": sv["kv"], "h": sv["h"], "xn2": sv["xn2"], "xn": sv["xn"], "P": P,
                "attn": "self_attn", "s1": s[0], "s2": s[1], "cross": False} for dy, x, sv, P, s in zip(dys, xs, svs, Ps, scales)]
     pres = [CTX.lazy_ln.pop(dy.data_ptr(), None) for dy in dys]
     for gd, pre in zip(groups, pres):
@@ -1115,7 +1124,7 @@
             heads_ = [_cross_head_fwd(xs[i], xs[1 - i], Ps[i], dims, eps) for i in (0, 1)]
         scales = [(sa1, sa2), (sb1, sb2)]
         groups = [{"x": xs[i], "kvsrc": heads_[i][5], "P": Ps[i], "attn": "cross_attn", "s1": scales[i][0], "s2": scales[i][1],
-                   "want_xn": False} for i in (0, 1)]
+                   "want_xn": False, "rebuild": _rebuild(dims, C, heads, Ps[0])} for i in (0, 1)]
         if fuse_sampler:
             for i in (0, 1):
                 groups[i].update(kvsrc=None, hid=heads_[i][3], samp_src=xs[1 - i])
@@ -1153,8 +1162,8 @@
         rps = dims[1] * dims[2] * dims[3]
         dys = [_c(dy).reshape(-1, C), _c(dya).reshape(-1, C)]
         groups = [{"dy": dys[i], "x": None, "x1": svs[i]["x1"], "stats": svs[i]["stats"], "q": svs[i]["q"], "kv": svs[i]["kv"],
-                   "h": svs[i]["h"], "xn2": svs[i]["xn2"], "P": Ps[i], "attn": "cross_attn", "s1": scales[i][0], "s2": scales[i][1], "cross": True,
-                   "want_copy": True} for i in (0, 1)]
+                   "h": svs[i]["h"], "xn2": svs[i]["xn2"], "xn": svs[i]["xn"], "kvs16": svs[i]["kvs16"], "P": Ps[i], "attn": "cross_attn",
+                   "s1": scales[i][0], "s2": scales[i][1], "cross": True, "want_copy": True} for i in (0, 1)]
         bos = ops.block_bwd(groups, dims, C, heads, (C // heads) ** -0.5)
         acc = [bos[0]["dx1_copy"], bos[1]["dx1_copy"]]
         for i in (0, 1):
diff --git a/micformer_amd/ops.py b/micformer_amd/ops.py
--- a/micformer_amd/ops.py
+++ b/micformer_amd/ops.py
@@ -1012,7 +1012,17 @@
     return bool(_lib.lib.micf_block_recomputes_h(C, heads))
 
 
-def block_fwd(groups, dims, C, heads, eps, scale, persist_probe=None, save=True):
+def block_rebuilds(dims, C, heads, hidden):
+    B, D, H, W = dims
+    T = B * D * H * W
+    return (_lib.get_option("block_wave") != 0 and C == 48 and C % heads == 0 and C // heads == 16
+            and _dt() == 1 and _dt_attn() == 1 and not (_lib.get_option("block_debug") & ~17)
+            and block_tile_tokens(dims, C, heads, hidden, backward=True) == 32
+            and T * C * 4 < (1 << 32) and T * hidden * 2 < (1 << 31))
+
+
+def block_fwd(groups, dims, C, heads, eps, scale, persist_probe=None, save=True, rebuild=False):
+    rebuild = rebuild or groups[0].get("rebuild", False)
     B, D, H, W = dims
     T = B * D * H * W
     hidden = groups[0]["P"]["mlp.fc1.weight"].shape[0]
@@ -1040,6 +1050,10 @@
                  "kvs16": _new(x, T, C, dtype=sd) if (st16 and cross) else None,
                  "flow": _new(x, T, 3) if fused_sampler else None,
                  "xs32": _new(x, T, C) if (fused_sampler and not st16) else None}
+            if rebuild:
+                o["h"] = None
+                if rebuild != "h":
+                    o["q"] = o["kv"] = None
         it.x, it.kvsrc, it.s1, it.s2 = f32(x), f32(gd.get("kvsrc")), f32(gd.get("s1")), f32(gd.get("s2"))
         if fused_sampler:
             it.hid, it.samp_src = f32(gd["hid"]), f32(gd["samp_src"])
@@ -1097,10 +1111,17 @@
         for k in ("dy", "x", "x1", "stats", "s1", "s2"):
             setattr(it, k, f32(gd.get(k)))
         h = gd.get("h")
-        if (h is not None and h.dtype != (torch.bfloat16 if _dt() else torch.float32)) or gd["q"].dtype != sd or gd["kv"].dtype != sd \
-                or (h is None and gd["xn2"].dtype != sd):
+        reads = [gd[k] for k in ("q", "kv") if gd[k] is not None] + ([gd["xn2"]] if h is None else [])
+        if gd["q"] is None:
+            reads += [gd["xn"]] + ([gd["kvs16"]] if cross else [])
+        if (h is not None and h.dtype != (torch.bfloat16 if _dt() else torch.float32)) or any(t.dtype != sd for t in reads):
             raise _lib.MicfError("block_bwd: the saved tensors were written in another arithmetic mode")
         it.h, it.q, it.kv = ptr(h), ptr(gd["q"]), ptr(gd["kv"])
+        if gd["q"] is None:
+            wf = block_weights(P, a, backward=False, only=("wq", "wkv"))
+            keep.append(wf)
+            it.xn, it.kvs16, it.wq, it.wkv = ptr(gd["xn"]), ptr(gd["kvs16"]) if cross else None, ptr(wf["wq"]), ptr(wf["wkv"])
+            it.bq, it.bkv = f32(P[f"{a}.q.bias"]), f32(P[f"{a}.kv.bias"])
         pre = gd.get("pre")
         if pre is not None:
             if not st16 or cross:
@@ -1121,7 +1142,7 @@
             setattr(it, field, ptr(wt))
         for k, v in o.items():
             setattr(it, k, ptr(v))
-        nb += 4 * T * C * (2 if cross else 3) + sum(gd[k].numel() * gd[k].element_size() for k in ("q", "kv", "h" if h is not None else "xn2")) \
+        nb += 4 * T * C * (2 if cross else 3) + sum(t.numel() * t.element_size() for t in reads + ([h] if h is not None else [])) \
             + sum(v.numel() * v.element_size() for v in o.values() if v is not None) + 12 * C * C * wt.element_size()
         o["tiles"] = tiles
         outs.append(o)
```
